# kav-institute/SemanticLiDARUnc

Hardware: AMD Instinct MI355X
Metric: range-image scans/sec (64x2048, T=8 MC) (higher is better)
Workload: dtype f16 (fp16 activations/weights, fp32 accumulate + epilogue, fp32 logits); 1 GPU; SalsaNext MC-dropout T=8 + entropy/MI map + IoU/ECE accumulation, 8 scans of 64x2048x5 per step per GPU (BASELINE configs[2] shape); T=8, parallelism=scan-sharded x1, mc_schedule=every pass fully recomputed

## Files before the change

include/slu.h:

```cpp
#ifndef SLU_H_
#define SLU_H_

#include <stddef.h>
#include <stdint.h>

#ifdef __cplusplus
extern "C" {
#endif

#define SLU_ABI_VERSION 32

#define SLU_OK            0
#define SLU_EINVAL       -1
#define SLU_EUNSUPPORTED -2
#define SLU_ELAUNCH      -3

typedef void* slu_stream_t;

int slu_abi_version(void);
const char* slu_strerror(int code);

#define SLU_MAX_SRC 3

typedef struct slu_conv_src {
  const float* ptr;
  const float* scale;
  int32_t C;
  int32_t pixel_shuffle;
  int32_t nbatch;
  int32_t cuse;
} slu_conv_src;

typedef struct slu_conv_desc {
  slu_conv_src src[SLU_MAX_SRC];
  int32_t nsrc;
  int32_t N, H, W;
  int32_t Cin, Cout;
  int32_t ksize, dil, pad;
  int32_t ck;
  const float* wpack;
  const float* bias;
  int32_t has_act;
  float slope;
  const float* bn_a;
  const float* bn_b;
  const float* resid;
  float* out;
  int32_t precision;
  double* stats;
} slu_conv_desc;

#define SLU_CONV_FP32  0
#define SLU_CONV_F16X3 1

int slu_conv_ck(int ksize);
size_t slu_packed_weight_floats(int cout, int cin, int ksize, int ck);
int slu_pack_conv_weight(const float* w, int cout, int cin, int ksize, int ck, float* out, slu_stream_t stream);
typedef struct slu_pack_job {
  const float* w;
  float* out;
  int32_t cout, cin, ksize, ck;
  int32_t dgrad, reserved;
  uint64_t begin;
// ... 39 lines not shown
int slu_lovasz_fwd(const float* probs, const int64_t* labels, int B, int C, int HW, int64_t ignore_index, unsigned class_mask,
                   void* workspace, size_t workspace_bytes, float* loss, float* n_present, float* grad_probs,
                   slu_stream_t stream);

int slu_bn_stats(const float* y, int N, int C, int HW, double* sum, double* sumsq, slu_stream_t stream);
int slu_bn_bwd_reduce(const float* dz, const float* y, const float* mean, const float* invstd, int N, int C, int HW,
                      double* s1, double* s2, slu_stream_t stream);
int slu_bn_coeffs_fwd(const double* sum, const double* sumsq, double count, const float* gamma, const float* beta, float eps,
                      float momentum, int train, float* running_mean, float* running_var, int C, float* mean, float* invstd,
                      float* a, float* b, slu_stream_t stream);
int slu_bn_coeffs_bwd(const double* s1, const double* s2, double count, const float* gamma, const float* mean, const float* invstd,
                      int train, int C, float* k1, float* k2, float* k3, float* dgamma, float* dbeta, slu_stream_t stream);
int slu_affine_fwd(const float* y, const float* a, const float* b, const float* resid, float* z, int N, int C, int HW,
                   slu_stream_t stream);
int slu_act_affine_bwd(const float* dz, const float* y, const float* k1, const float* k2, const float* k3, float slope,
                       int has_act, int N, int C, int HW, float* da, double* dbias, slu_stream_t stream);
int slu_bn_apply_fwd(const float* y, const double* sum, const double* sumsq, double count, const float* gamma, const float* beta, float eps,
                     float momentum, int train, float* running_mean, float* running_var, const float* resid, float* z, int N, int C, int HW,
                     float* mean, float* invstd, slu_stream_t stream);
int slu_bn_act_bwd(const float* dz, const float* y, const double* s1, const double* s2, double count, const float* gamma, const float* mean,
                   const float* invstd, int has_bn, int train, float slope, int has_act, int N, int C, int HW, float* da, double* acc64,
                   unsigned* ticket, float* dbias, float* dgamma, float* dbeta, slu_stream_t stream);
int slu_nchw_to_nhwc(const float* src, int N, int C, int HW, float* dst, slu_stream_t stream);
int slu_gather_nhwc(const slu_conv_src* src, int nsrc, int N, int H, int W, float* dst, slu_stream_t stream);
int slu_split_grad(const float* dcat, int N, int Ccat, int cbeg, int H, int W, int Csrc, int pixel_shuffle, const float* scale,
                   float* dsrc, slu_stream_t stream);
int slu_avgpool3s2_bwd(const float* dy, const float* scale, float* dx, int N, int C, int H, int W, slu_stream_t stream);
int slu_dgrad_weight(const float* w, int cout, int cin, int ksize, float* wd, slu_stream_t stream);
size_t slu_wgrad_packed_floats(int cout, int cin, int ksize);
int slu_conv2d_wgrad(const float* da_t, const float* in_t, int N, int H, int W, int Cout, int Cin, int ksize, int dil, int pad,
                     float* dWp, float* dW, slu_stream_t stream);
int slu_conv1x1_wgrad_nchw(const float* da, const slu_conv_src* src, int nsrc, int N, int HW, int Cout, float* dW, int prezeroed, slu_stream_t stream);
int slu_conv2d_wgrad_nchw(const float* da, const slu_conv_src* src, int nsrc, int N, int H, int W, int Cout, int ksize, int dil, int pad,
                          float* dWp, float* dW, int prezeroed, slu_stream_t stream);

int slu_maxpool3s2_fwd(const float* x, float* y, int N, int C, int H, int W, slu_stream_t stream);
int slu_nearest_down(const float* x, float* y, int N, int C, int H, int W, int factor, slu_stream_t stream);
int slu_space_to_depth2(const float* x, float* y, int N, int C, int H, int W, slu_stream_t stream);
int slu_space_to_depth2_cat(const float* a, int Ca, int ca, const float* b, int Cb, float* y, int N, int H, int W, slu_stream_t stream);
int slu_depth_to_space(const float* x, float* y, int N, int Cout, int H, int W, int r, int elu_plus_one, int c_off, int Ctot,
                       slu_stream_t stream);
int slu_row_softmax_mul(const float* score, const float* value, float* out, int N, int C, int H, int W, slu_stream_t stream);

int slu_bilinear_upsample(const float* x, float* y, int N, int C, int H, int W, int scale, slu_stream_t stream);
int slu_groupnorm_fwd(const float* x, const float* gamma, const float* beta, int N, int C, int HW, int groups, float eps, int relu, float* mean,
                      float* rstd, float* y, slu_stream_t stream);
int slu_spatial_softmax_gate(const float* x, const float* score, float* stats, float* out, int N, int C, int HW, slu_stream_t stream);

typedef struct slu_h8_src {
  const void* ptr;
  const float* scale;
  int32_t G;
  int32_t nbatch;
} slu_h8_src;

typedef struct slu_conv_h8_desc {
  slu_h8_src src[SLU_MAX_SRC];
  int32_t nsrc;
  int32_t N, H, W, Cout, ksize, dil, pad;
  const void* wpack;
  const float* bias;
  int32_t has_act;
  float slope;
  const float* bn_a;
  const float* bn_b;
  const void* resid;
  void* out;
  int32_t out_f32_nchw;
} slu_conv_h8_desc;

size_t slu_packed_weight_bytes_h8(int cout, int cin, int ksize);
int slu_pack_conv_weight_h8(const float* w, int cout, int cin, int ksize, void* out, slu_stream_t stream);
int slu_conv2d_h8_fwd(const slu_conv_h8_desc* desc, slu_stream_t stream);
int slu_conv2d_h8_kernel_name(const slu_conv_h8_desc* desc, char* buf, size_t n);
int slu_nchw_to_h8(const float* x, const float* scale, void* y, int N, int C, int H, int W, slu_stream_t stream);
int slu_h8_to_nchw(const void* x, float* y, int N, int C, int H, int W, slu_stream_t stream);
int slu_avgpool3s2_h8(const void* x, const float* scale, void* y, int N, int in_batch, int G, int H, int W, slu_stream_t stream);
int slu_pixel_shuffle_h8(const void* x, const float* scale_in, const float* scale_out, void* y, int N, int Gin, int H, int W,
                         slu_stream_t stream);

typedef struct slu_conv_tail_h8_desc {
  const void *a1, *a2;
  int32_t N, H, W, C;
  const void *w2x2, *w1x1;
  const float *biasA, *bnA_a, *bnA_b;
  int32_t hasactA;
  float slopeA;
  const float *biasB, *bnB_a, *bnB_b;
  int32_t hasactB;
  float slopeB;
  const void* resid;
  void* out;
  const void *sc_x, *sc_w;
  const float* sc_bias;
  int32_t sc_cin, sc_hasact;
  float sc_slope;
} slu_conv_tail_h8_desc;
int slu_conv_tail_h8_supported(int C, int H, int W);
int slu_conv_tail_h8_shortcut_supported(int C, int sc_cin);
int slu_conv_tail_h8_fwd(const slu_conv_tail_h8_desc* desc, slu_stream_t stream);
int slu_conv_tail_h8_kernel_name(const slu_conv_tail_h8_desc* desc, char* buf, size_t n);

typedef struct slu_ctx_block_h8_desc {
  const void* x;
  int32_t N, H, W, Cin, C;
  const void *w1, *w2, *w3;
  const float* bias1;
  const float *bias2, *bn1_a, *bn1_b;
  const float *bias3, *bn2_a, *bn2_b;
  float slope;
  void* out;
} slu_ctx_block_h8_desc;
int slu_ctx_block_h8_supported(int Cin, int C, int H, int W);
int slu_ctx_block_h8_fwd(const slu_ctx_block_h8_desc* desc, slu_stream_t stream);

int slu_head_mc_h8(const void* x, int T, int B, int G, int HW, const void* wpack, const float* bias, int C, float eps, float* p_bar,
                   float* h_norm, float* mi_norm, int64_t* preds, slu_stream_t stream);

int slu_dirichlet_head(const float* shape_logits, long long shape_batch_stride, const float* scale_logits, long long scale_batch_stride,
                       int B, int C, int HW, float temperature, float eps, float* alpha, float* p_hat, float* entropy, float* aleatoric,
                       int64_t* preds, slu_stream_t stream);
int slu_dirichlet_uncertainty(const float* alpha, int B, int C, int HW, float eps, float* p_hat, float* entropy, float* aleatoric,
                              int64_t* preds, slu_stream_t stream);

int slu_auroc_scores(const float* preds, const int64_t* labels, const float* score_override, int B, int C, int HW, int mode, int score_kind,
                     int has_ignore, int64_t ignore_index, float eps, float* scores, uint8_t* flags, slu_stream_t stream);
size_t slu_auroc_workspace_bytes(long long n);
int slu_auroc_compute(const float* scores, const uint8_t* is_error, long long n, void* workspace, size_t workspace_bytes, double* out3,
                      float* sorted_scores, uint8_t* sorted_is_error, slu_stream_t stream);

int slu_ua_samples(const int64_t* labels, const int64_t* preds, const float* uncertainty, long long n, const int64_t* ignore_ids, int n_ignore,
                   float* u_out, uint8_t* flags, slu_stream_t stream);
int slu_binned_counts(const float* u, const uint8_t* correct, long long n, const float* edges, int n_bins, int64_t* count, int64_t* n_correct,
                      slu_stream_t stream);

int slu_ece_samples(const float* preds, const int64_t* labels, int B, int C, int HW, int mode, int has_ignore, int64_t ignore_index, float eps,
                    float* conf, uint8_t* flags, slu_stream_t stream);
int slu_binned_stats(const float* u, const uint8_t* correct, long long n, const float* edges, int n_bins, int64_t* count, int64_t* n_correct,
                     double* sum_u, slu_stream_t stream);

size_t slu_group_by_class_workspace_bytes(long long n);
int slu_group_by_class(const int64_t* labels, const float* values, long long n, int C, float* out_values, int64_t* counts, void* workspace,
                       size_t workspace_bytes, slu_stream_t stream);

int slu_tversky_fwd(const float* x, const int64_t* labels, int B, int C, int HW, int model_act, int has_ignore, int64_t ignore_index, float alpha,
                    float beta, float smooth, int reduction, double* sums, float* coef, float* loss, float* any_valid, slu_stream_t stream);
int slu_tversky_bwd(const float* x, const int64_t* labels, int B, int C, int HW, int model_act, int has_ignore, int64_t ignore_index, float alpha,
                    float beta, const float* coef, const float* grad_out, int grad_out_per_class, float* grad_x, slu_stream_t stream);

int slu_dirichlet_loss_fwd(const float* alpha, const int64_t* labels, int B, int C, int HW, int kind, float param, float eps, int has_ignore,
                           int64_t ignore_index, double* sum, int64_t* count, slu_stream_t stream);
int slu_dirichlet_loss_bwd(const float* alpha, const int64_t* labels, int B, int C, int HW, int kind, float param, float eps, int has_ignore,
                           int64_t ignore_index, const float* gscale, float* grad_alpha, slu_stream_t stream);

int slu_dirichlet_loss_fwd_ex(const float* alpha, const int64_t* labels, int B, int C, int HW, int kind, const float* params, int nparams, float eps,
                              int has_ignore, int64_t ignore_index, double* sums2, int64_t* count, slu_stream_t stream);
int slu_dirichlet_loss_bwd_ex(const float* alpha, const int64_t* labels, int B, int C, int HW, int kind, const float* params, int nparams, float eps,
                              int has_ignore, int64_t ignore_index, const float* gscale, float* grad_alpha, slu_stream_t stream);

size_t slu_spherical_projection_workspace_bytes(int N, int H, int W);
int slu_spherical_projection(const double* pc, int N, int C, int H, int W, int use_data_theta_range, double theta_min, double theta_max,
                             void* workspace, size_t workspace_bytes, float* img, double* theta_range_out, slu_stream_t stream);
int slu_spherical_projection_ex(const double* pc, int N, int C, int H, int W, int use_data_theta_range, double theta_min, double theta_max,
                                const double* bins_h, int bins_increasing, int keep_farthest, int flip, void* workspace, size_t workspace_bytes,
// ... 49 lines not shown
```

semanticlidarunc_amd/_lib.py:

```python
from __future__ import annotations

import ctypes as C
import os

ABI_VERSION = 32
MAX_SRC = 3
_HERE = os.path.dirname(os.path.abspath(__file__))
LIB_PATH = os.path.join(_HERE, "libslu_hip.so")

c_f32p = C.c_void_p
c_i64p = C.c_void_p
c_f64p = C.c_void_p
c_stream = C.c_void_p


class ConvSrc(C.Structure):
    _fields_ = [("ptr", C.c_void_p), ("scale", C.c_void_p), ("C", C.c_int32), ("pixel_shuffle", C.c_int32),
                ("nbatch", C.c_int32), ("cuse", C.c_int32)]


class ConvDesc(C.Structure):
    _fields_ = [
        ("src", ConvSrc * MAX_SRC),
        ("nsrc", C.c_int32),
        ("N", C.c_int32), ("H", C.c_int32), ("W", C.c_int32),
        ("Cin", C.c_int32), ("Cout", C.c_int32),
        ("ksize", C.c_int32), ("dil", C.c_int32), ("pad", C.c_int32),
        ("ck", C.c_int32),
        ("wpack", C.c_void_p), ("bias", C.c_void_p),
        ("has_act", C.c_int32), ("slope", C.c_float),
        ("bn_a", C.c_void_p), ("bn_b", C.c_void_p),
        ("resid", C.c_void_p), ("out", C.c_void_p),
        ("precision", C.c_int32),
        ("stats", C.c_void_p),
    ]


class H8Src(C.Structure):
    _fields_ = [("ptr", C.c_void_p), ("scale", C.c_void_p), ("G", C.c_int32), ("nbatch", C.c_int32)]


class ConvH8Desc(C.Structure):
    _fields_ = [
        ("src", H8Src * MAX_SRC),
        ("nsrc", C.c_int32),
        ("N", C.c_int32), ("H", C.c_int32), ("W", C.c_int32), ("Cout", C.c_int32),
        ("ksize", C.c_int32), ("dil", C.c_int32), ("pad", C.c_int32),
        ("wpack", C.c_void_p), ("bias", C.c_void_p),
        ("has_act", C.c_int32), ("slope", C.c_float),
        ("bn_a", C.c_void_p), ("bn_b", C.c_void_p),
        ("resid", C.c_void_p), ("out", C.c_void_p),
        ("out_f32_nchw", C.c_int32),
    ]


class PackJob(C.Structure):
    _fields_ = [("w", C.c_void_p), ("out", C.c_void_p), ("cout", C.c_int32), ("cin", C.c_int32), ("ksize", C.c_int32), ("ck", C.c_int32),
                ("dgrad", C.c_int32), ("reserved", C.c_int32), ("begin", C.c_uint64)]


class ConvTailH8Desc(C.Structure):
    _fields_ = [
        ("a1", C.c_void_p), ("a2", C.c_void_p),
        ("N", C.c_int32), ("H", C.c_int32), ("W", C.c_int32), ("C", C.c_int32),
        ("w2x2", C.c_void_p), ("w1x1", C.c_void_p),
        ("biasA", C.c_void_p), ("bnA_a", C.c_void_p), ("bnA_b", C.c_void_p),
        ("hasactA", C.c_int32), ("slopeA", C.c_float),
        ("biasB", C.c_void_p), ("bnB_a", C.c_void_p), ("bnB_b", C.c_void_p),
        ("hasactB", C.c_int32), ("slopeB", C.c_float),
        ("resid", C.c_void_p), ("out", C.c_void_p),
        ("sc_x", C.c_void_p), ("sc_w", C.c_void_p), ("sc_bias", C.c_void_p),
        ("sc_cin", C.c_int32), ("sc_hasact", C.c_int32), ("sc_slope", C.c_float),
    ]


class CtxBlockH8Desc(C.Structure):
    _fields_ = [
        ("x", C.c_void_p),
        ("N", C.c_int32), ("H", C.c_int32), ("W", C.c_int32), ("Cin", C.c_int32), ("C", C.c_int32),
        ("w1", C.c_void_p), ("w2", C.c_void_p), ("w3", C.c_void_p),
        ("bias1", C.c_void_p),
        ("bias2", C.c_void_p), ("bn1_a", C.c_void_p), ("bn1_b", C.c_void_p),
        ("bias3", C.c_void_p), ("bn2_a", C.c_void_p), ("bn2_b", C.c_void_p),
        ("slope", C.c_float),
        ("out", C.c_void_p),
    ]


SIGNATURES = {
    "slu_abi_version": (C.c_int, []),
    "slu_strerror": (C.c_char_p, [C.c_int]),
    "slu_conv_ck": (C.c_int, [C.c_int]),
    "slu_packed_weight_floats": (C.c_size_t, [C.c_int, C.c_int, C.c_int, C.c_int]),
    "slu_pack_conv_weight": (C.c_int, [c_f32p, C.c_int, C.c_int, C.c_int, C.c_int, c_f32p, c_stream]),
    "slu_pack_conv_weights_multi": (C.c_int, [C.c_void_p, C.c_int, C.c_size_t, c_stream]),
    "slu_conv2d_fwd": (C.c_int, [C.POINTER(ConvDesc), c_stream]),
    "slu_packed_weight_bytes_f16x3": (C.c_size_t, [C.c_int, C.c_int, C.c_int]),
    "slu_pack_conv_weight_f16x3": (C.c_int, [c_f32p, C.c_int, C.c_int, C.c_int, C.c_void_p, c_stream]),
    "slu_conv2d_kernel_name": (C.c_int, [C.POINTER(ConvDesc), C.c_char_p, C.c_size_t]),
    "slu_bn_fold": (C.c_int, [c_f32p, c_f32p, c_f32p, c_f32p, C.c_float, C.c_int, c_f32p, c_f32p, c_stream]),
    "slu_avgpool3s2_fwd": (C.c_int, [c_f32p, c_f32p, c_f32p, C.c_int, C.c_int, C.c_int, C.c_int, c_stream]),
    "slu_avgpool3s2_bcast_fwd": (C.c_int, [c_f32p, c_f32p, c_f32p, C.c_int, C.c_int, C.c_int, C.c_int, C.c_int, c_stream]),
    "slu_mc_reduce": (C.c_int, [c_f32p, C.c_int, C.c_int, C.c_int, C.c_int, C.c_float, c_f32p, c_f32p, c_f32p,
                                c_i64p, c_stream]),
    "slu_softmax_entropy": (C.c_int, [c_f32p, C.c_int, C.c_int, C.c_int, C.c_float, c_f32p, c_f32p, c_i64p,
                                      c_stream]),
    "slu_confusion_update": (C.c_int, [c_i64p, c_i64p, C.c_int64, C.c_int, c_i64p, c_stream]),
    "slu_ece_update": (C.c_int, [c_f32p, c_i64p, C.c_int, C.c_int, C.c_int, C.c_int64, C.c_int, c_i64p, c_f64p,
                                 c_f64p, c_stream]),
    "slu_softmax_nll_fwd": (C.c_int, [c_f32p, c_i64p, C.c_int, C.c_int, C.c_int, C.c_float, c_f32p, c_f64p,
                                      c_stream]),
    "slu_nll_fwd": (C.c_int, [c_f32p, c_i64p, C.c_int, C.c_int, C.c_int, C.c_int, C.c_float, C.c_int64, c_f64p, c_i64p,
                              c_stream]),
    "slu_nll_bwd": (C.c_int, [c_f32p, c_i64p, C.c_int, C.c_int, C.c_int, C.c_int, C.c_float, C.c_int64, c_f32p, c_f32p,
                              c_stream]),
    "slu_softmax_loss_bwd": (C.c_int, [c_f32p, c_i64p, c_f32p, C.c_float, C.c_float, C.c_float, c_f32p, C.c_int, C.c_int,
                                       C.c_int, c_f32p, c_stream]),
    "slu_bn_stats": (C.c_int, [c_f32p, C.c_int, C.c_int, C.c_int, c_f64p, c_f64p, c_stream]),
    "slu_bn_bwd_reduce": (C.c_int, [c_f32p, c_f32p, c_f32p, c_f32p, C.c_int, C.c_int, C.c_int, c_f64p, c_f64p, c_stream]),
    "slu_bn_coeffs_fwd": (C.c_int, [c_f64p, c_f64p, C.c_double, c_f32p, c_f32p, C.c_float, C.c_float, C.c_int, c_f32p, c_f32p, C.c_int,
                                    c_f32p, c_f32p, c_f32p, c_f32p, c_stream]),
    "slu_bn_coeffs_bwd": (C.c_int, [c_f64p, c_f64p, C.c_double, c_f32p, c_f32p, c_f32p, C.c_int, C.c_int, c_f32p, c_f32p, c_f32p,
                                    c_f32p, c_f32p, c_stream]),
    "slu_affine_fwd": (C.c_int, [c_f32p, c_f32p, c_f32p, c_f32p, c_f32p, C.c_int, C.c_int, C.c_int, c_stream]),
    "slu_bn_apply_fwd": (C.c_int, [c_f32p, c_f64p, c_f64p, C.c_double, c_f32p, c_f32p, C.c_float, C.c_float, C.c_int, c_f32p, c_f32p, c_f32p, c_f32p,
                                   C.c_int, C.c_int, C.c_int, c_f32p, c_f32p, c_stream]),
    "slu_bn_act_bwd": (C.c_int, [c_f32p, c_f32p, c_f64p, c_f64p, C.c_double, c_f32p, c_f32p, c_f32p, C.c_int, C.c_int, C.c_float, C.c_int, C.c_int,
                                 C.c_int, C.c_int, c_f32p, c_f64p, C.c_void_p, c_f32p, c_f32p, c_f32p, c_stream]),
    "slu_act_affine_bwd": (C.c_int, [c_f32p, c_f32p, c_f32p, c_f32p, c_f32p, C.c_float, C.c_int, C.c_int, C.c_int, C.c_int,
                                     c_f32p, c_f64p, c_stream]),
    "slu_nchw_to_nhwc": (C.c_int, [c_f32p, C.c_int, C.c_int, C.c_int, c_f32p, c_stream]),
    "slu_gather_nhwc": (C.c_int, [C.POINTER(ConvSrc), C.c_int, C.c_int, C.c_int, C.c_int, c_f32p, c_stream]),
    "slu_split_grad": (C.c_int, [c_f32p, C.c_int, C.c_int, C.c_int, C.c_int, C.c_int, C.c_int, C.c_int, c_f32p, c_f32p,
                                 c_stream]),
    "slu_avgpool3s2_bwd": (C.c_int, [c_f32p, c_f32p, c_f32p, C.c_int, C.c_int, C.c_int, C.c_int, c_stream]),
    "slu_dgrad_weight": (C.c_int, [c_f32p, C.c_int, C.c_int, C.c_int, c_f32p, c_stream]),
    "slu_wgrad_packed_floats": (C.c_size_t, [C.c_int, C.c_int, C.c_int]),
    "slu_conv2d_wgrad": (C.c_int, [c_f32p, c_f32p, C.c_int, C.c_int, C.c_int, C.c_int, C.c_int, C.c_int, C.c_int, C.c_int,
# ... 116 lines not shown
```

semanticlidarunc_amd/csrc/conv2d_h8.hip:

```cpp
#include <stdio.h>
#include "slu_common.h"
#include <cstdlib>
#include <utility>

typedef _Float16 half8 __attribute__((ext_vector_type(8)));
typedef _Float16 half2v __attribute__((ext_vector_type(2)));
typedef float f32x16 __attribute__((ext_vector_type(16)));
typedef float float2v __attribute__((ext_vector_type(2)));

#ifndef H8_M128_OPT_3X3
#define H8_M128_OPT_3X3 15
#endif
#ifndef H8_M128_OPT_2X2
#define H8_M128_OPT_2X2 15
#endif
#ifndef H8_M128_KPC2_DEFAULT
#define H8_M128_KPC2_DEFAULT 0
#endif

namespace {

struct H8Src {
  const uint4* ptr;
  const float* scale;
  int G;
  int gbeg;
  int nb;
};

struct H8Args {
  H8Src src[SLU_MAX_SRC];
  int nsrc;
  int N, H, W, Gin, Cout, Gout, nmblk, nks;
  const uint4* wpack;
  const float *bias, *bn_a, *bn_b;
  int has_act;
  float slope;
  int out_f32;
  int tiles_x, tiles_y;
  int order;
#ifdef SLU_H8_AB
  int dbg;
#endif
};

struct SrcSel {
  const uint4* ptr;
  const float* scale;
  int G, gl, ns;
};

__device__ __forceinline__ SrcSel select_src(const H8Args& a, const int (&img)[SLU_MAX_SRC], int g) {
  SrcSel p{a.src[0].ptr, a.src[0].scale, a.src[0].G, g, img[0]};
#pragma unroll
  for (int s = 1; s < SLU_MAX_SRC; ++s)
    if (s < a.nsrc && g >= a.src[s].gbeg) p = SrcSel{a.src[s].ptr, a.src[s].scale, a.src[s].G, g - a.src[s].gbeg, img[s]};
  return p;
}

__device__ __forceinline__ uint4 scale_record(uint4 v, const float* sp) {
  const float4 s0 = *reinterpret_cast<const float4*>(sp);
  const float4 s1 = *reinterpret_cast<const float4*>(sp + 4);
  half8 h = __builtin_bit_cast(half8, v);
  h[0] *= (_Float16)s0.x; h[1] *= (_Float16)s0.y; h[2] *= (_Float16)s0.z; h[3] *= (_Float16)s0.w;
  h[4] *= (_Float16)s1.x; h[5] *= (_Float16)s1.y; h[6] *= (_Float16)s1.z; h[7] *= (_Float16)s1.w;
  return __builtin_bit_cast(uint4, h);
}

__device__ __forceinline__ unsigned pack2(float x, float y) {
  half2v h;
  h[0] = (_Float16)x;
  h[1] = (_Float16)y;
  return __builtin_bit_cast(unsigned, h);
}

template <int STRIDE>
__device__ __forceinline__ void store_tile(const H8Args& a, const f32x16& acc, const float* se, int cl0, int co0, int hh, bool pix_ok,
                                           size_t n, size_t pix, size_t HW, const void* __restrict__ resid, void* __restrict__ out,
                                           float slope_pre) {
#pragma unroll
// ... 84 lines not shown
      if (resid) {
        const bool okq = pix_ok && go0 + q < a.Gout;
        const uint2 r = *(okq ? resid + (((n * a.Gout + go0 + q) * HW + pix) * 2 + hh) : reinterpret_cast<const uint2*>(zero_addr));
        t0 += __builtin_convertvector(__builtin_bit_cast(half2v, r.x), float2v);
        t1 += __builtin_convertvector(__builtin_bit_cast(half2v, r.y), float2v);
      }
      hw[2 * q2] = __builtin_bit_cast(unsigned, __builtin_convertvector(t0, half2v));
      hw[2 * q2 + 1] = __builtin_bit_cast(unsigned, __builtin_convertvector(t1, half2v));
    }
    const auto s0 = __builtin_amdgcn_permlane32_swap(hw[0], hw[2], false, false);
    const auto s1 = __builtin_amdgcn_permlane32_swap(hw[1], hw[3], false, false);
    const int go = go0 + 2 * pr + hh;
    uint4* dst = (pix_ok && go < a.Gout) ? out + ((n * a.Gout + go) * HW + pix) : reinterpret_cast<uint4*>(trash_addr);
    *dst = make_uint4(s0[0], s1[0], s0[1], s1[1]);
  }
}

#ifdef SLU_H8_PROF
__device__ unsigned long long g_h8_prof[8];
#define H8_PROF_MARK(i)                                         \
  {                                                             \
    const unsigned long long t_now = __builtin_amdgcn_s_memtime(); \
    asm volatile("" ::: "memory");                              \
    prof_acc[i] += t_now - prof_t;                              \
    prof_t = t_now;                                             \
  }
#else
#define H8_PROF_MARK(i)
#endif

#define SLU_GLDS16(gsrc, ldst_wave_base)                                                                  \
  __builtin_amdgcn_global_load_lds((const __attribute__((address_space(1))) void*)(gsrc),                 \
                                   (__attribute__((address_space(3))) void*)(ldst_wave_base), 16, 0, 0)

constexpr int h8_waves_per_simd(int mb, int nwave, int rpw) { return (mb * rpw >= 8) ? 1 : ((nwave >= 8 || mb >= 2 || rpw >= 2) ? 2 : 3); }

template <int KS, int DIL, int PAD, int MB, int WM, int WN, int RPW, bool SCALED, bool WRES, bool F32OUT, int KPC = 1, int OPT = 0, bool ONE = false>
__global__ __launch_bounds__(64 * WM * WN, h8_waves_per_simd(MB, WM * WN, RPW)) void conv_h8_kernel(const H8Args a, const void* __restrict__ resid,
                                                                                                       void* __restrict__ out) {
  constexpr int NWAVE = WM * WN;
  constexpr int T = KS * KS, TS = KPC * T;
  constexpr int TW = 64, TH = WN * RPW, NB = 2 * RPW;
  constexpr int LW = TW + 2 * PAD, LH = TH + 2 * PAD;
  constexpr int REC = LH * LW;
  constexpr int MBLK = WM * MB;
  constexpr int NREC_B = KPC * 2 * REC, NBLK_B = (NREC_B + 63) / 64;
  constexpr int NB_ALLOC = NBLK_B * 64;
  constexpr int NREC_A = MBLK * TS * 64, NBLK_A = MBLK * TS;
  constexpr int NIB = (NBLK_B + NWAVE - 1) / NWAVE, NIA = (NBLK_A + NWAVE - 1) / NWAVE;
  static_assert(KPC == 1 || (!WRES && !SCALED && MB == 2 && WM == 2 && WN == 4), "multi-K-step chunks: the 8-wave 128-channel configuration only");
  static_assert(OPT == 0 || (MB == 2 && WM == 2 && WN == 4 && !F32OUT), "OPT: the 8-wave 128-channel configuration only");
  static_assert(KPC <= 2, "pc_rc carries 2 bits of channel block");
  static_assert(KPC == 1 || ONE, "multi-K-step chunks: single-source layers only");

  extern __shared__ __attribute__((aligned(16))) char smem[];
  float* s_epi = reinterpret_cast<float*>(smem);
  uint4* s_scale = reinterpret_cast<uint4*>(s_epi + 3 * MBLK * 32);
  uint4* s_b = s_scale + (SCALED ? 128 : 0);
  uint4* s_a = s_b + 2 * NB_ALLOC;

  const int tid = threadIdx.x, lane = tid & 63, wave = __builtin_amdgcn_readfirstlane(tid >> 6);
  const int wm = wave / WN, wn = wave % WN;
  const bool late_half = wave >= NWAVE / 2;
  const int mblk0 = blockIdx.y * MBLK;
  int t_beg, t_end, t_step = 1;
  {
    const int nwg = gridDim.x, b = blockIdx.x, xcd = b & 7, qq = nwg >> 3, rr = nwg & 7;
    const int w = (xcd < rr ? xcd * (qq + 1) : rr * (qq + 1) + (xcd - rr) * qq) + (b >> 3);
    const long long nt = (long long)a.tiles_x * a.tiles_y * a.N;
    if (a.order) {
      t_step = nwg;
      t_beg = w;
      t_end = w < nt ? w + (int)((nt - w + nwg - 1) / nwg) * nwg : w;
    } else {
      t_beg = (int)(nt * w / nwg);
      t_end = (int)(nt * (w + 1) / nwg);
    }
  }
  t_beg = __builtin_amdgcn_readfirstlane(t_beg);
  t_end = __builtin_amdgcn_readfirstlane(t_end);
  t_step = __builtin_amdgcn_readfirstlane(t_step);
  if (t_beg >= t_end) return;

  if (tid < MBLK * 32) {
    const int co = mblk0 * 32 + tid;
    const bool ok = co < a.Cout;
    s_epi[tid] = (ok && a.bias) ? a.bias[co] : 0.0f;
    s_epi[MBLK * 32 + tid] = (ok && a.bn_a) ? a.bn_a[co] : 1.0f;
    s_epi[2 * MBLK * 32 + tid] = (ok && a.bn_a) ? a.bn_b[co] : 0.0f;
  }

  const int hh = lane >> 5, jj = lane & 31;
  const size_t HW = (size_t)a.H * a.W;
  const float slope_pre = (a.has_act & 3) == 1 ? a.slope : 1.0f;
  const int nks = a.nks;
  const int nchunk = (nks + KPC - 1) / KPC;
  const int a_stride = WRES ? nks * T * 64 : TS * 64;
  const int abase = (wm * MB) * a_stride + lane;
  const int bbase = hh * REC + (wn * RPW) * LW + jj;

  struct TilePos { int tx, ty, x0, y0, n, i0, i1, i2; };
  auto rfl = [](int v) __attribute__((always_inline)) { return __builtin_amdgcn_readfirstlane(v); };
  const int step_tx = rfl(t_step % a.tiles_x), step_ty = rfl((t_step / a.tiles_x) % a.tiles_y), step_n = rfl(t_step / (a.tiles_x * a.tiles_y));
  auto finish = [&](TilePos& p) __attribute__((always_inline)) {
    p.x0 = p.tx * TW;
    p.y0 = p.ty * TH;
    p.i0 = p.i1 = p.i2 = p.n;
    if constexpr (!ONE) {
      if (a.src[0].nb) p.i0 = rfl(p.n % a.src[0].nb);
      if (a.nsrc > 1 && a.src[1].nb) p.i1 = rfl(p.n % a.src[1].nb);
      if (a.nsrc > 2 && a.src[2].nb) p.i2 = rfl(p.n % a.src[2].nb);
    }
  };
  auto decode = [&](int t) __attribute__((always_inline)) {
    TilePos p;
    p.tx = rfl(t % a.tiles_x);
    t /= a.tiles_x;
    p.ty = rfl(t % a.tiles_y);
    p.n = rfl(t / a.tiles_y);
    finish(p);
    return p;
  };
  auto advance = [&](TilePos p) __attribute__((always_inline)) {
    p.tx += step_tx;
    if (p.tx >= a.tiles_x) p.tx -= a.tiles_x, p.ty += 1;
    p.ty += step_ty;
    if (p.ty >= a.tiles_y) p.ty -= a.tiles_y, p.n += 1;
    p.n += step_n;
    finish(p);
    return p;
  };
  static_assert(SLU_MAX_SRC == 3, "TilePos carries one image index per source");
  uintptr_t zero_addr = reinterpret_cast<uintptr_t>(&g_zero_rec);
  asm volatile("" : "+s"(zero_addr));
  uintptr_t trash_addr = reinterpret_cast<uintptr_t>(&g_trash_rec);
  asm volatile("" : "+s"(trash_addr));
  int pc_rc[NIB], pc_off[NIB];
#pragma unroll
  for (int i = 0; i < NIB; ++i) {
    const int e = (i * NWAVE + wave) * 64 + lane;
    const int g2 = e / REC;
    const int rem = e - g2 * REC;
    const int r = rem / LW;
    const int c = rem - r * LW;
    pc_rc[i] = r | (c << 8) | ((g2 & (2 * KPC - 1)) << 16) | ((e < NREC_B ? 1 : 0) << 20);
    pc_off[i] = r * a.W + c + (g2 & (2 * KPC - 1)) * (int)HW;
  }
  constexpr int NPIECE = NIB + (WRES ? 0 : NIA);
  constexpr int PPT = (NPIECE + TS - 1) / TS;
  uintptr_t st_b0 = 0, st_b1 = 0;
  int st_g0 = 0;
  bool st_on = false;
  int st_x0 = 0, st_y0 = 0, st_q = 0, st_wave = wave;
  uint4 *st_db = s_b, *st_da = s_a;
  auto stage_begin = [&](const TilePos& tp, int q, int buf) __attribute__((always_inline)) {
    const int img[SLU_MAX_SRC] = {tp.i0, tp.i1, tp.i2};
    const long long org = (long long)(tp.y0 - PAD) * a.W + (tp.x0 - PAD);
    st_g0 = 2 * KPC * q;
    if constexpr (ONE) {
      st_b0 = reinterpret_cast<uintptr_t>(a.src[0].ptr) + 16 * ((long long)(((size_t)tp.n * a.src[0].G + st_g0) * HW) + org);
      st_b1 = st_b0;
    } else {
      const SrcSel p0 = select_src(a, img, st_g0 < a.Gin ? st_g0 : 0), p1 = select_src(a, img, st_g0 + 1 < a.Gin ? st_g0 + 1 : 0);
      st_b0 = reinterpret_cast<uintptr_t>(p0.ptr) + 16 * ((long long)(((size_t)p0.ns * p0.G + p0.gl) * HW) + org);
      st_b1 = reinterpret_cast<uintptr_t>(p1.ptr) + 16 * ((long long)(((size_t)p1.ns * p1.G + p1.gl) * HW) + org - (long long)HW);
    }
    st_x0 = tp.x0 - PAD;
    st_y0 = tp.y0 - PAD;
    st_q = q;
    st_db = s_b + buf * NB_ALLOC;
    st_da = s_a + buf * NREC_A;
    st_on = true;
    st_wave = wave;
    asm volatile("" : "+s"(st_wave));
  };
  auto stage_piece = [&](int i) __attribute__((always_inline)) {
    if (i < NIB) {
      const int blk = i * NWAVE + st_wave;
      if (NBLK_B % NWAVE == 0 || blk < NBLK_B) {
        const int rc = pc_rc[i];
        const int gy = st_y0 + (rc & 255), gx = st_x0 + ((rc >> 8) & 255);
        const int gsel = (rc >> 16) & 3;
        const uintptr_t gb = (!ONE && gsel == 1) ? st_b1 : st_b0;
        const bool ok = (rc >> 20) && st_g0 + gsel < a.Gin && (unsigned)gy < (unsigned)a.H && (unsigned)gx < (unsigned)a.W;
        const uintptr_t src = ok ? gb + 16 * (long long)pc_off[i] : zero_addr;
        SLU_GLDS16(reinterpret_cast<const uint4*>(src), st_db + blk * 64);
      }
    } else if constexpr (!WRES) {
      const int blk = (i - NIB) * NWAVE + st_wave;
      if (NBLK_A % NWAVE == 0 || blk < NBLK_A) {
        const int m = blk / TS, r = blk - m * TS;
        const bool live = mblk0 + m < a.nmblk && (KPC == 1 || KPC * st_q + r / T < nks);
        const uint4* src = live ? a.wpack + (((size_t)(mblk0 + m) * nks + KPC * st_q) * T + r) * 64 + lane : reinterpret_cast<const uint4*>(zero_addr);
        SLU_GLDS16(src, st_da + blk * 64);
      }
    }
  };
  auto stage_after_tap = [&](int tap) __attribute__((always_inline)) {
    if (st_on) {
#pragma unroll
      for (int k = 0; k < PPT; ++k)
        if (tap * PPT + k < NPIECE) stage_piece(tap * PPT + k);
    }
  };
  auto stage_scales = [&](int n, int par) __attribute__((always_inline)) {
    if (tid < 64) {
      half8 h;
#pragma unroll
      for (int k = 0; k < 8; ++k) h[k] = (_Float16)1.0f;
      if (tid < a.Gin) {
        int img[SLU_MAX_SRC] = {0, 0, 0};
        const SrcSel p = select_src(a, img, tid);
        if (p.scale) {
          const float* sp = p.scale + ((size_t)n * p.G + p.gl) * 8;
          const float4 s0 = *reinterpret_cast<const float4*>(sp), s1 = *reinterpret_cast<const float4*>(sp + 4);
          h[0] = (_Float16)s0.x; h[1] = (_Float16)s0.y; h[2] = (_Float16)s0.z; h[3] = (_Float16)s0.w;
          h[4] = (_Float16)s1.x; h[5] = (_Float16)s1.y; h[6] = (_Float16)s1.z; h[7] = (_Float16)s1.w;
        }
      }
      s_scale[par * 64 + tid] = __builtin_bit_cast(uint4, h);
    }
  };

  if constexpr (WRES) {
    const int per_m = nks * T;
    for (int blk = wave; blk < MBLK * per_m; blk += NWAVE) {
      const int m = blk / per_m;
      const uint4* src = mblk0 + m < a.nmblk ? a.wpack + ((size_t)(mblk0 + m) * per_m + (blk - m * per_m)) * 64 + lane : &g_zero_rec;
      SLU_GLDS16(src, s_a + blk * 64);
    }
  }
  TilePos cur = decode(t_beg), nxt = cur;
  stage_begin(cur, 0, 0);
#pragma unroll
  for (int i = 0; i < NPIECE; ++i) stage_piece(i);
  int buf = 0;
  constexpr bool SWAP16 = (OPT & 8) != 0;
  constexpr int NST = MB * NB * (SWAP16 ? 2 : 4);
  constexpr bool PRE = MB == 1 && !F32OUT;
  const uint2* resid2 = reinterpret_cast<const uint2*>(resid);
  uint2 rv[PRE ? NB : 1][4];
  auto setup_next = [&](int tile, int q) __attribute__((always_inline)) {
    st_on = false;
    if (q + 1 < nchunk) {
      stage_begin(cur, q + 1, buf ^ 1);
    } else if (tile + t_step < t_end) {
      nxt = advance(cur);
      stage_begin(nxt, 0, buf ^ 1);
    }
  };

#ifdef SLU_H8_PROF
  unsigned long long prof_acc[6] = {0, 0, 0, 0, 0, 0}, prof_t = __builtin_amdgcn_s_memtime();
#endif
  int tile_no = 0;
  for (int tile = t_beg; tile < t_end; tile += t_step, ++tile_no) {
    f32x16 acc[MB][NB];
#pragma unroll
    for (int i = 0; i < MB; ++i)
#pragma unroll
      for (int b = 0; b < NB; ++b)
#pragma unroll
        for (int r = 0; r < 16; ++r) acc[i][b][r] = 0.0f;
    const int spar = tile_no & 1;
    if constexpr (SCALED) stage_scales(cur.n, spar);
    for (int q = 0; q < nchunk; ++q) {
      if constexpr ((OPT & 4) != 0) setup_next(tile, q);
      if (!F32OUT && q == 0 && tile != t_beg) asm volatile("s_waitcnt vmcnt(%0)" ::"n"(NST < 63 ? NST : 63) : "memory");
      else asm volatile("s_waitcnt vmcnt(0)" ::: "memory");
      asm volatile("s_waitcnt lgkmcnt(0)" ::: "memory");
      H8_PROF_MARK(0)
      __builtin_amdgcn_s_barrier();
      asm volatile("" ::: "memory");
      H8_PROF_MARK(1)
      if constexpr ((OPT & 4) == 0) setup_next(tile, q);
      if constexpr (PRE) {
        if (resid && q == nchunk - 1) {
#pragma unroll
          for (int b = 0; b < NB; ++b) {
            const int gy = cur.y0 + wn * RPW + (b >> 1), gx = cur.x0 + (b & 1) * 32 + jj;
            const bool pix_ok = gy < a.H && gx < a.W;
            const size_t pix = (size_t)gy * a.W + gx;
#pragma unroll
            for (int k = 0; k < 4; ++k) {
              const int go = (mblk0 + wm) * 4 + k;
              rv[b][k] = *((pix_ok && go < a.Gout) ? resid2 + (((size_t)cur.n * a.Gout + go) * HW + pix) * 2 + hh
                                                   : reinterpret_cast<const uint2*>(zero_addr));
            }
          }
        }
      }
      H8_PROF_MARK(2)
      const uint4* sb = s_b + buf * NB_ALLOC + bbase;
      const uint4* sa = s_a + abase + (WRES ? q * T * 64 : buf * NREC_A);
      half8 sc;
      if constexpr (SCALED) sc = __builtin_bit_cast(half8, s_scale[spar * 64 + 2 * q + hh]);
      {
        if constexpr (MB == 2 && WM == 2 && WN == 4) {
          half8 af[2][MB], bf[2][NB];
          auto read_frags = [&](int set, int ts) __attribute__((always_inline)) {
            const int j = ts / T, tap = ts % T;
            const int dy = (tap / KS) * DIL, dx = (tap % KS) * DIL;
#pragma unroll
            for (int i = 0; i < MB; ++i) af[set][i] = __builtin_bit_cast(half8, sa[i * a_stride + ts * 64]);
#pragma unroll
            for (int b = 0; b < NB; ++b) {
              bf[set][b] = __builtin_bit_cast(half8, sb[j * 2 * REC + ((b >> 1) + dy) * LW + (b & 1) * 32 + dx]);
              if constexpr (SCALED) bf[set][b] *= sc;
            }
          };
          read_frags(0, 0);
#pragma unroll
          for (int ts = 0; ts < TS; ++ts) {
            if (ts + 1 < TS) read_frags((ts + 1) & 1, ts + 1);
            __builtin_amdgcn_sched_barrier(0);
            if constexpr ((OPT & 1) != 0) {
              if (late_half) stage_after_tap(ts);
              __builtin_amdgcn_sched_barrier(0);
            }
            if constexpr ((OPT & 2) != 0) __builtin_amdgcn_s_setprio(1);
#pragma unroll
            for (int b = 0; b < NB; ++b)
#pragma unroll
              for (int i = 0; i < MB; ++i) acc[i][b] = __builtin_amdgcn_mfma_f32_32x32x16_f16(af[ts & 1][i], bf[ts & 1][b], acc[i][b], 0, 0, 0);
            if constexpr ((OPT & 2) != 0) __builtin_amdgcn_s_setprio(0);
            __builtin_amdgcn_sched_barrier(0);
            if constexpr ((OPT & 1) != 0) {
              if (!late_half) stage_after_tap(ts);
            } else {
              stage_after_tap(ts);
            }
          }
        } else if constexpr (MB == 1) {
          half8 af[2][MB], bf[2][NB];
          auto read_frags = [&](int set, int tap) __attribute__((always_inline)) {
            const int dy = (tap / KS) * DIL, dx = (tap % KS) * DIL;
#pragma unroll
            for (int i = 0; i < MB; ++i) af[set][i] = __builtin_bit_cast(half8, sa[i * a_stride + tap * 64]);
#pragma unroll
            for (int b = 0; b < NB; ++b) {
              bf[set][b] = __builtin_bit_cast(half8, sb[((b >> 1) + dy) * LW + (b & 1) * 32 + dx]);
              if constexpr (SCALED) bf[set][b] *= sc;
            }
          };
          read_frags(0, 0);
#pragma unroll
          for (int tap = 0; tap < T; ++tap) {
            if (tap + 1 < T) read_frags((tap + 1) & 1, tap + 1);
#pragma unroll
            for (int b = 0; b < NB; ++b)
#pragma unroll
              for (int i = 0; i < MB; ++i) acc[i][b] = __builtin_amdgcn_mfma_f32_32x32x16_f16(af[tap & 1][i], bf[tap & 1][b], acc[i][b], 0, 0, 0);
            if (tap + 1 < T) {
#pragma unroll
              for (int k = 0; k < MB * NB; ++k) {
                __builtin_amdgcn_sched_group_barrier(0x008, 1, 0);
                __builtin_amdgcn_sched_group_barrier(0x100, (MB + NB + MB * NB - 1) / (MB * NB), 0);
              }
            }
            stage_after_tap(tap);
          }
        } else {
#pragma unroll
          for (int tap = 0; tap < T; ++tap) {
            const int dy = (tap / KS) * DIL, dx = (tap % KS) * DIL;
            half8 af[MB];
#pragma unroll
            for (int i = 0; i < MB; ++i) af[i] = __builtin_bit_cast(half8, sa[i * a_stride + tap * 64]);
#pragma unroll
            for (int b = 0; b < NB; ++b) {
              half8 bf = __builtin_bit_cast(half8, sb[((b >> 1) + dy) * LW + (b & 1) * 32 + dx]);
              if constexpr (SCALED) bf *= sc;
#pragma unroll
              for (int i = 0; i < MB; ++i) acc[i][b] = __builtin_amdgcn_mfma_f32_32x32x16_f16(af[i], bf, acc[i][b], 0, 0, 0);
            }
#pragma unroll
            for (int k = 0; k < MB * NB; ++k) {
              __builtin_amdgcn_sched_group_barrier(0x008, 1, 0);
              __builtin_amdgcn_sched_group_barrier(0x100, (MB + NB + MB * NB - 1) / (MB * NB), 0);
            }
            stage_after_tap(tap);
          }
        }
      }
      buf ^= 1;
      H8_PROF_MARK(3)
    }
    {
#pragma unroll
      for (int i = 0; i < MB; ++i) {
        const int ml = wm * MB + i;
#pragma unroll
        for (int b = 0; b < NB; ++b) {
          const int gy = cur.y0 + wn * RPW + (b >> 1), gx = cur.x0 + (b & 1) * 32 + jj;
          const bool pix_ok = gy < a.H && gx < a.W;
          const size_t pix = pix_ok ? (size_t)gy * a.W + gx : 0;
          if constexpr (F32OUT)
            store_tile<MBLK * 32>(a, acc[i][b], s_epi, ml * 32, (mblk0 + ml) * 32, hh, pix_ok, (size_t)cur.n, pix, HW, resid, out, slope_pre);
          else if constexpr (SWAP16)
            store_tile_swap16<MBLK * 32>(a, acc[i][b], s_epi, ml * 32, (mblk0 + ml) * 4, hh, pix_ok, (size_t)cur.n, pix, HW, resid2,
                                         reinterpret_cast<uint4*>(out), slope_pre, zero_addr, trash_addr);
          else
            store_tile_full<MBLK * 32, PRE>(a, acc[i][b], s_epi, ml * 32, (mblk0 + ml) * 4, hh, pix_ok, (size_t)cur.n, pix, HW, resid2,
                                            rv[PRE ? b : 0], reinterpret_cast<uint2*>(out), slope_pre, zero_addr, trash_addr);
          __builtin_amdgcn_sched_barrier(0);
        }
      }
    }
    H8_PROF_MARK(4)
    cur = nxt;
  }
#ifdef SLU_H8_PROF
  if (tid == 0) {
    for (int i = 0; i < 5; ++i) atomicAdd(&g_h8_prof[i], prof_acc[i]);
    atomicAdd(&g_h8_prof[5], 1ull);
  }
#endif
}

template <int MB, int NBW>
__global__ __launch_bounds__(256, (MB * NBW >= 8) ? 2 : ((MB * NBW >= 4) ? 3 : 4)) void conv1x1_h8_kernel(const H8Args a, const void* __restrict__ resid,
                                                                                                         void* __restrict__ out) {
  constexpr int KSPC = 4;
  constexpr int NWV = MB * KSPC * 64, NW = (NWV + 255) / 256;
  extern __shared__ __attribute__((aligned(16))) char smem[];
// ... 440 lines not shown
  const size_t HWi = (size_t)H * W;
  const int OW = 2 * W;
  for (size_t e = (size_t)blockIdx.x * blockDim.x + threadIdx.x; e < total; e += (size_t)gridDim.x * blockDim.x) {
    const int w = (int)(e % W);
    size_t r = e / W;
    const int h = (int)(r % H);
    r /= H;
    const int go = (int)(r % Go);
    const size_t n = r / Go;
    float v[4][8];
#pragma unroll
    for (int q = 0; q < 4; ++q) {
      const int gi = 4 * go + q;
      const bool ok = gi < Gi;
      const half8 rec = __builtin_bit_cast(half8, ok ? x[(n * Gi + gi) * HWi + (size_t)h * W + w] : make_uint4(0u, 0u, 0u, 0u));
#pragma unroll
      for (int slot = 0; slot < 8; ++slot) {
        float t = (float)rec[slot];
        if (ok && s_in) t *= s_in[n * Gi * 8 + gi * 8 + slot];
        v[slot & 3][2 * q + (slot >> 2)] = t;
      }
    }
    if (s_out) {
#pragma unroll
      for (int k = 0; k < 8; ++k) {
        const int co = 8 * go + k;
        const float so = co < 2 * Gi ? s_out[n * (Gi * 2) + co] : 0.0f;
#pragma unroll
        for (int sub = 0; sub < 4; ++sub) v[sub][k] *= so;
      }
    }
#pragma unroll
    for (int sub = 0; sub < 4; ++sub) {
      const size_t o = ((n * Go + go) * (size_t)(2 * H) + (2 * h + (sub >> 1))) * OW + 2 * w + (sub & 1);
      y[o] = make_uint4(pack2(v[sub][0], v[sub][1]), pack2(v[sub][2], v[sub][3]), pack2(v[sub][4], v[sub][5]), pack2(v[sub][6], v[sub][7]));
    }
  }
}

inline unsigned grid_for(size_t total) {
  const size_t nb = (total + 255) / 256;
  return (unsigned)(nb > 32768 ? 32768 : (nb ? nb : 1));
}

int fill_h8(const slu_conv_h8_desc* d, H8Args& a) {
  if (!d || !d->out || !d->wpack || d->nsrc < 1 || d->nsrc > SLU_MAX_SRC) return SLU_EINVAL;
  if (d->N <= 0 || d->H <= 0 || d->W <= 0 || d->Cout <= 0) return SLU_EINVAL;
  if (d->bn_a && !d->bn_b) return SLU_EINVAL;
  if (d->has_act != 0 && d->has_act != 1) return SLU_EINVAL;
  if (d->has_act && !(d->slope >= 0.0f && d->slope <= 1.0f)) return SLU_EINVAL;
  int g = 0;
  for (int s = 0; s < d->nsrc; ++s) {
    const slu_h8_src& S = d->src[s];
    if (!S.ptr || S.G <= 0 || S.nbatch < 0) return SLU_EINVAL;
    if (((uintptr_t)S.ptr & 15) || ((uintptr_t)S.scale & 15)) return SLU_EINVAL;
    a.src[s] = H8Src{reinterpret_cast<const uint4*>(S.ptr), S.scale, S.G, g, S.nbatch};
    g += S.G;
  }
  for (int s = d->nsrc; s < SLU_MAX_SRC; ++s) a.src[s] = H8Src{nullptr, nullptr, 0, 0x7fffffff, 0};
  if (((uintptr_t)d->out & 15) || ((uintptr_t)d->resid & 15) || ((uintptr_t)d->wpack & 15)) return SLU_EINVAL;
  if (d->resid && d->out_f32_nchw) return SLU_EINVAL;
  a.nsrc = d->nsrc;
  a.N = d->N; a.H = d->H; a.W = d->W;
  a.Gin = g;
  a.Cout = d->Cout;
  a.Gout = (d->Cout + 7) / 8;
  a.nmblk = (d->Cout + 31) / 32;
  a.nks = (g + 1) / 2;
  a.wpack = reinterpret_cast<const uint4*>(d->wpack);
  a.bias = d->bias; a.bn_a = d->bn_a; a.bn_b = d->bn_b;
  a.has_act = d->has_act; a.slope = d->slope;
  a.out_f32 = d->out_f32_nchw ? 1 : 0;
  a.tiles_x = a.tiles_y = 0;
#ifdef SLU_H8_AB
  static const int dbg = [] { const char* e = getenv("SLU_GEMM_DBG"); return e ? atoi(e) : 0; }();
  a.dbg = dbg;
#endif
  return SLU_OK;
}

template <int KS, int DIL, int PAD, int MB, int WM, int WN, int RPW, bool SCALED, bool WRES, bool F32OUT = false, int KPC = 1, int OPT = 0, bool ONE = false>
int launch_h8_k(H8Args& a, const slu_conv_h8_desc* d, const SluEmit& e) {
  constexpr int TH = WN * RPW, MBLK = WM * MB, T = KS * KS, NWAVE = WM * WN;
  constexpr size_t nb_alloc = (size_t)((KPC * 2 * (TH + 2 * PAD) * (64 + 2 * PAD) + 63) / 64) * 64;
  const size_t lds = (size_t)3 * MBLK * 32 * 4 + (SCALED ? 2048 : 0) + 2 * nb_alloc * 16 + (size_t)MBLK * (WRES ? a.nks : 2 * KPC) * T * 64 * 16;
  if (lds > 160 * 1024) return SLU_EUNSUPPORTED;
  if (SCALED && a.Gin > 64) return SLU_EUNSUPPORTED;
  a.tiles_x = (a.W + 63) / 64;
  a.tiles_y = (a.H + TH - 1) / TH;
  static const int order = [] { const char* e = getenv("SLU_H8_ORDER"); return e ? atoi(e) : 1; }();
  a.order = order;
  const long long nt = (long long)a.tiles_x * a.tiles_y * a.N;
  const int gy = (a.nmblk + MBLK - 1) / MBLK;
  if (nt <= 0 || nt > 0x7fffffffLL || gy > 65535) return SLU_EUNSUPPORTED;
  if (e.name)
    return slu_emit_name(e, "conv_h8_kernel<%d, %d, %d, %d, %d, %d, %d, %s, %s, %s, %d, %d, %s>", KS, DIL, PAD, MB, WM, WN, RPW, slu_tf(SCALED),
                         slu_tf(WRES), slu_tf(F32OUT), KPC, OPT, slu_tf(ONE));
  long long per_cu = h8_waves_per_simd(MB, NWAVE, RPW) * 4 / NWAVE;
  const long long by_lds = (long long)(160 * 1024 / lds);
  if (by_lds < per_cu) per_cu = by_lds;
  if (per_cu < 1) per_cu = 1;
  long long gx = (256 * per_cu + gy - 1) / gy;
  if (gx < 8) gx = 8;
  if (gx > nt) gx = nt;
  auto kern = conv_h8_kernel<KS, DIL, PAD, MB, WM, WN, RPW, SCALED, WRES, F32OUT, KPC, OPT, ONE>;
  static SluLdsGrant grant;
  if (slu_grant_dynamic_lds(reinterpret_cast<const void*>(kern), lds, grant) != SLU_OK) return SLU_ELAUNCH;
  hipLaunchKernelGGL(kern, dim3((unsigned)gx, (unsigned)gy), dim3(64 * NWAVE), lds, e.st, a, d->resid, d->out);
  SLU_CHECK_LAUNCH();
}

typedef float f32x4v __attribute__((ext_vector_type(4)));

struct RingArgs {
  const uint4 *x, *x1;
  int G0, G1;
  const uint4* wpack;
  const float *bias, *bn_a, *bn_b;
  float slope;
  uint4* out;
  int N, H, W, tiles_x, tiles_y;
};

template <int NKS, int NIB, int P, int NST>
constexpr int ring3_younger(int c) {
  const int s0 = ((c - P) % NKS + NKS) % NKS;
  int n = s0 == NKS - 1 ? NST : 0;
  for (int d = 1; d < P; ++d) n += NIB + ((s0 + d) % NKS == NKS - 1 ? NST : 0);
  return n;
}
template <class F, int... Cs>
__device__ __forceinline__ void ring3_static_for(F&& f, std::integer_sequence<int, Cs...>) {
  (f(std::integral_constant<int, Cs>{}), ...);
}

template <int DIL, int MB, int NKS, int RPW, int D>
__global__ __launch_bounds__(512, 2) void ring3_h8_kernel(const RingArgs a) {
  constexpr int NWAVE = 8, KS = 3, T = 9, PAD = DIL, P = D - 1;
  constexpr int C = 32 * MB, GO = 4 * MB;
  constexpr int TW = 64, TH = NWAVE * RPW, NB = 2 * RPW;
  constexpr int LW = TW + 2 * PAD, LH = TH + 2 * PAD, REC = LH * LW;
  constexpr int NBLK_B = (2 * REC + 63) / 64, NIB = (NBLK_B + NWAVE - 1) / NWAVE;
  constexpr int BUFREC = NBLK_B * 64;
  constexpr int NST = MB * NB * 2;
  static_assert(P >= 1 && P <= NKS, "ring depth");

  __shared__ __attribute__((aligned(16))) float s_epi[3 * C];
  extern __shared__ __attribute__((aligned(16))) char smem[];
  uint4* s_w = reinterpret_cast<uint4*>(smem);
  uint4* s_ring = s_w + MB * NKS * T * 64;
  uint4* s_trash = s_ring + D * BUFREC;

  const int tid = threadIdx.x, lane = tid & 63, wave = __builtin_amdgcn_readfirstlane(tid >> 6), wn = wave;
  const int hh = lane >> 5, jj = lane & 31;
  const size_t HW = (size_t)a.H * a.W;

  int t_beg, t_end, t_step;
  {
    const int nwg = gridDim.x, b = blockIdx.x, xcd = b & 7, qq = nwg >> 3, rr = nwg & 7;
    const int w = (xcd < rr ? xcd * (qq + 1) : rr * (qq + 1) + (xcd - rr) * qq) + (b >> 3);
    const long long nt = (long long)a.tiles_x * a.tiles_y * a.N;
    t_step = nwg;
    t_beg = w;
    t_end = w < nt ? w + (int)((nt - w + nwg - 1) / nwg) * nwg : w;
  }
  if (t_beg >= t_end) return;

  if (tid < C) {
    s_epi[tid] = a.bias ? a.bias[tid] : 0.0f;
    s_epi[C + tid] = a.bn_a ? a.bn_a[tid] : 1.0f;
    s_epi[2 * C + tid] = a.bn_a ? a.bn_b[tid] : 0.0f;
  }
  for (int blk = wave; blk < MB * NKS * T; blk += NWAVE) SLU_GLDS16(a.wpack + (size_t)blk * 64 + lane, s_w + blk * 64);

  struct TilePos { int x0, y0, n; };
  auto decode = [&](int t) {
    TilePos p;
    const int tx = t % a.tiles_x;
    t /= a.tiles_x;
    p.x0 = tx * TW;
    p.y0 = (t % a.tiles_y) * TH;
    p.n = t / a.tiles_y;
    return p;
  };
  int pc_rc[NIB], pc_off[NIB];
#pragma unroll
  for (int i = 0; i < NIB; ++i) {
    const int e = (i * NWAVE + wave) * 64 + lane;
    const int g2 = e / REC, rem = e - g2 * REC, r = rem / LW, c = rem - r * LW;
    pc_rc[i] = r | (c << 8) | ((g2 & 1) << 16) | ((e < 2 * REC ? 1 : 0) << 17);
    pc_off[i] = (r * a.W + c) * 16;
  }
  auto stage = [&](const TilePos& tp, int c, int slot, bool valid) {
    uint4* db = s_ring + slot * BUFREC;
    const uintptr_t zero = reinterpret_cast<uintptr_t>(&g_zero_rec);
    const bool second = 2 * c >= a.G0;
    const uint4* src = second ? a.x1 : a.x;
    const int gs = second ? a.G1 : a.G0, g = second ? 2 * c - a.G0 : 2 * c;
    const uintptr_t base0 = reinterpret_cast<uintptr_t>(src) +
                            16 * ((long long)(((size_t)tp.n * gs + g) * HW) + (long long)(tp.y0 - PAD) * a.W + (tp.x0 - PAD));
    const uintptr_t base1 = base0 + 16 * (long long)HW;
#pragma unroll
    for (int i = 0; i < NIB; ++i) {
      const int blk = i * NWAVE + wave;
      const int rc = pc_rc[i];
      const int gy = tp.y0 - PAD + (rc & 255), gx = tp.x0 - PAD + ((rc >> 8) & 255);
      const bool ok = valid && (rc >> 17) && (unsigned)gy < (unsigned)a.H && (unsigned)gx < (unsigned)a.W;
      const uintptr_t p = ok ? (((rc >> 16) & 1) ? base1 : base0) + (long long)pc_off[i] : zero;
      SLU_GLDS16(reinterpret_cast<const uint4*>(p), (NBLK_B % NWAVE == 0 || blk < NBLK_B) ? db + blk * 64 : s_trash);
    }
    asm volatile("" ::: "memory");
  };

  const int bbase = hh * REC + (wn * RPW) * LW + jj;
  TilePos cur = decode(t_beg), nxt = cur;
  bool has_next = t_beg + t_step < t_end;
  if (has_next) nxt = decode(t_beg + t_step);
#pragma unroll
  for (int c = 0; c < P; ++c) stage(cur, c, c, true);
  int rslot = 0, wslot = P % D;
  bool first = true;
  const float2v sl = {a.slope, a.slope};
  const f32x4v* se4p = reinterpret_cast<const f32x4v*>(s_epi) + hh;

  for (int tile = t_beg; tile < t_end; tile += t_step) {
    f32x16 acc[MB][NB];
#pragma unroll
    for (int i = 0; i < MB; ++i)
#pragma unroll
      for (int b = 0; b < NB; ++b)
#pragma unroll
        for (int r = 0; r < 16; ++r) acc[i][b][r] = 0.0f;

    auto position = [&](auto cc) {
      constexpr int c = decltype(cc)::value;
      constexpr int YOUNG = ring3_younger<NKS, NIB, P, NST>(c);
      static_assert(YOUNG <= 63, "vmcnt is a 6-bit counter");
      if (first && c < P) asm volatile("s_waitcnt vmcnt(0)" ::: "memory");
      else asm volatile("s_waitcnt vmcnt(%0)" ::"n"(YOUNG) : "memory");
      asm volatile("s_waitcnt lgkmcnt(0)" ::: "memory");
      __builtin_amdgcn_s_barrier();
      asm volatile("" ::: "memory");
      {
        constexpr int cn = (c + P) % NKS;
        if (c + P < NKS) stage(cur, cn, wslot, true);
        else stage(nxt, cn, wslot, has_next);
        wslot = wslot + 1 == D ? 0 : wslot + 1;
      }
      const uint4* sb = s_ring + rslot * BUFREC + bbase;
      rslot = rslot + 1 == D ? 0 : rslot + 1;
      half8 fa[2][MB], fb[2][NB];
      auto rd = [&](int tap, int buf) {
        const int dy = (tap / KS) * DIL, dx = (tap % KS) * DIL;
#pragma unroll
        for (int i = 0; i < MB; ++i) fa[buf][i] = __builtin_bit_cast(half8, s_w[((i * NKS + c) * T + tap) * 64 + lane]);
#pragma unroll
        for (int b = 0; b < NB; ++b) fb[buf][b] = __builtin_bit_cast(half8, sb[((b >> 1) + dy) * LW + (b & 1) * 32 + dx]);
      };
      rd(0, 0);
#pragma unroll
      for (int tap = 0; tap < T; ++tap) {
        if (tap + 1 < T) rd(tap + 1, (tap + 1) & 1);
        __builtin_amdgcn_sched_barrier(0);
#pragma unroll
        for (int b = 0; b < NB; ++b)
#pragma unroll
          for (int i = 0; i < MB; ++i) acc[i][b] = __builtin_amdgcn_mfma_f32_32x32x16_f16(fa[tap & 1][i], fb[tap & 1][b], acc[i][b], 0, 0, 0);
        __builtin_amdgcn_sched_barrier(0);
      }
    };
    ring3_static_for(position, std::make_integer_sequence<int, NKS>{});
    first = false;

#pragma unroll
    for (int i = 0; i < MB; ++i)
#pragma unroll
      for (int b = 0; b < NB; ++b) {
        const int gy = cur.y0 + wn * RPW + (b >> 1), gx = cur.x0 + (b & 1) * 32 + jj;
        const bool ok = gy < a.H && gx < a.W;
        const size_t idx0 = ok ? ((size_t)cur.n * GO + i * 4 + hh) * HW + (size_t)gy * a.W + gx : 0;
#pragma unroll
        for (int pr = 0; pr < 2; ++pr) {
          unsigned hw[4];
#pragma unroll
          for (int q2 = 0; q2 < 2; ++q2) {
            const int q = 2 * pr + q2;
            const int c4 = (i * 32 + 8 * q) / 4;
            const f32x4v bi = se4p[c4], ba = se4p[C / 4 + c4], bb = se4p[2 * C / 4 + c4];
            float2v t0 = {acc[i][b][4 * q], acc[i][b][4 * q + 1]}, t1 = {acc[i][b][4 * q + 2], acc[i][b][4 * q + 3]};
            t0 += float2v{bi.x, bi.y};
            t1 += float2v{bi.z, bi.w};
            t0 = __builtin_elementwise_max(t0, t0 * sl);
            t1 = __builtin_elementwise_max(t1, t1 * sl);
            t0 = t0 * float2v{ba.x, ba.y} + float2v{bb.x, bb.y};
            t1 = t1 * float2v{ba.z, ba.w} + float2v{bb.z, bb.w};
            hw[2 * q2] = __builtin_bit_cast(unsigned, __builtin_convertvector(t0, half2v));
            hw[2 * q2 + 1] = __builtin_bit_cast(unsigned, __builtin_convertvector(t1, half2v));
          }
          const auto s0 = __builtin_amdgcn_permlane32_swap(hw[0], hw[2], false, false);
          const auto s1 = __builtin_amdgcn_permlane32_swap(hw[1], hw[3], false, false);
          uint4* dst = ok ? a.out + idx0 + (size_t)(2 * pr) * HW : &g_trash_rec;
          *dst = make_uint4(s0[0], s1[0], s0[1], s1[1]);
        }
      }
    asm volatile("" ::: "memory");
    cur = nxt;
    has_next = tile + 2 * t_step < t_end;
    if (has_next) nxt = decode(tile + 2 * t_step);
  }
  asm volatile("s_waitcnt vmcnt(0)" ::: "memory");
}

template <int DIL, int MB, int NKS, int RPW, int D>
int launch_ring3(const H8Args& h, const slu_conv_h8_desc* d, const SluEmit& e) {
  constexpr int TH = 8 * RPW, PAD = DIL;
  constexpr size_t nblk_b = (size_t)(2 * (TH + 2 * PAD) * (64 + 2 * PAD) + 63) / 64;
  constexpr size_t lds = ((size_t)MB * NKS * 9 * 64 + (size_t)D * nblk_b * 64 + 64) * 16;
  static_assert(lds + 3 * 32 * MB * 4 <= 160 * 1024, "ring does not fit in LDS");
  RingArgs a{};
  a.x = h.src[0].ptr; a.G0 = h.src[0].G;
  a.x1 = h.nsrc > 1 ? h.src[1].ptr : h.src[0].ptr; a.G1 = h.nsrc > 1 ? h.src[1].G : 0;
  a.wpack = h.wpack; a.bias = h.bias; a.bn_a = h.bn_a; a.bn_b = h.bn_b;
  a.slope = (h.has_act & 3) == 1 ? h.slope : 1.0f;
  a.out = reinterpret_cast<uint4*>(d->out);
  a.N = h.N; a.H = h.H; a.W = h.W;
  a.tiles_x = (a.W + 63) / 64;
  a.tiles_y = (a.H + TH - 1) / TH;
  const long long nt = (long long)a.tiles_x * a.tiles_y * a.N;
  if (nt < 256) return -1;
  if (nt > 0x7fffffffLL) return SLU_EUNSUPPORTED;
  if (e.name) return slu_emit_name(e, "ring3_h8_kernel<%d, %d, %d, %d, %d>", DIL, MB, NKS, RPW, D);
  auto kern = ring3_h8_kernel<DIL, MB, NKS, RPW, D>;
  static SluLdsGrant grant;
  if (slu_grant_dynamic_lds(reinterpret_cast<const void*>(kern), lds, grant) != SLU_OK) return SLU_ELAUNCH;
  hipLaunchKernelGGL(kern, dim3(256), dim3(512), lds, e.st, a);
  SLU_CHECK_LAUNCH();
}

bool ring3_ok(const slu_conv_h8_desc* d, const H8Args& a) {
  static const bool off = [] { const char* e = getenv("SLU_H8_RING3"); return e && e[0] == '0'; }();
  if (off || d->ksize != 3 || d->pad != d->dil || (d->dil != 1 && d->dil != 2) || a.nsrc < 1 || a.nsrc > 2) return false;
  int gsum = 0;
  for (int s = 0; s < a.nsrc; ++s) {
    if (a.src[s].scale || a.src[s].nb) return false;
    gsum += a.src[s].G;
  }
  if (gsum != a.Gin || (a.nsrc == 2 && (a.src[0].G & 1)) || a.out_f32 || d->resid || (a.has_act & ~1)) return false;
  if ((a.has_act & 1) && !(a.slope >= 0.0f && a.slope <= 1.0f)) return false;
  return (a.Cout == 32 || a.Cout == 64) && ((a.Gin == 4 || a.Gin == 8) || (a.Gin == 10 && a.Cout == 32 && d->dil == 1));
}

int launch_ring3_any(const H8Args& a, const slu_conv_h8_desc* d, const SluEmit& e) {
  const int mb = a.Cout / 32, nks = a.Gin / 2;
  if (nks == 5) return launch_ring3<1, 1, 5, 1, 4>(a, d, e);
  if (mb == 2 && nks == 4) return d->dil == 1 ? launch_ring3<1, 2, 4, 1, 3>(a, d, e) : launch_ring3<2, 2, 4, 1, 3>(a, d, e);
  if (mb == 2 && nks == 2) return d->dil == 1 ? launch_ring3<1, 2, 2, 2, 3>(a, d, e) : launch_ring3<2, 2, 2, 1, 3>(a, d, e);
  if (mb == 1 && nks == 4) return d->dil == 1 ? launch_ring3<1, 1, 4, 2, 3>(a, d, e) : launch_ring3<2, 1, 4, 1, 3>(a, d, e);
  return d->dil == 1 ? launch_ring3<1, 1, 2, 2, 3>(a, d, e) : launch_ring3<2, 1, 2, 2, 3>(a, d, e);
}

constexpr size_t WRES_MAX_BYTES = 24 * 1024;

template <int KS, int DIL, int PAD, int MB, int WM, int WN, int RPW, bool SCALED>
int launch_h8(H8Args& a, const slu_conv_h8_desc* d, const SluEmit& e) {
  const size_t wbytes = (size_t)WM * MB * a.nks * KS * KS * 64 * 16;
  if (wbytes <= WRES_MAX_BYTES) return launch_h8_k<KS, DIL, PAD, MB, WM, WN, RPW, SCALED, true>(a, d, e);
  return launch_h8_k<KS, DIL, PAD, MB, WM, WN, RPW, SCALED, false>(a, d, e);
}

inline long long wg_count(const H8Args& a, int th, int mblk) {
  return (long long)a.N * ((a.H + th - 1) / th) * ((a.W + 63) / 64) * ((a.nmblk + mblk - 1) / mblk);
}

enum { CFG_M32_TH16 = 0, CFG_M64_TH16, CFG_M128_TH8, CFG_M32_TH8, CFG_M64_TH8, CFG_M128_TH4, CFG_M32_TH4, CFG_M64_TH4, CFG_COUNT };

int choose_h8(const H8Args& a) {
  const long long want = 256;
  static const int forced = [] { const char* e = getenv("SLU_H8_CFG"); return e ? atoi(e) : -1; }();
  if (forced >= 0 && forced < CFG_COUNT) return forced;
  if (a.nmblk >= 4) {
    if (a.H >= 8 && wg_count(a, 8, 4) >= want) return CFG_M128_TH8;
    if (wg_count(a, 4, 4) >= want) return CFG_M128_TH4;
    if (wg_count(a, 4, 2) >= want) return CFG_M64_TH4;
    return CFG_M32_TH4;
  }
  if (a.nmblk >= 2) {
    if (a.H >= 16 && wg_count(a, 16, 2) >= want) return CFG_M64_TH16;
    if (a.H >= 8 && wg_count(a, 8, 2) >= want) return CFG_M64_TH8;
    if (wg_count(a, 4, 2) >= want) return CFG_M64_TH4;
    return CFG_M32_TH4;
  }
  if (a.H >= 16 && wg_count(a, 16, 1) >= want) return CFG_M32_TH16;
  if (a.H >= 8 && wg_count(a, 8, 1) >= want) return CFG_M32_TH8;
  return CFG_M32_TH4;
}

int g_h8_opt = [] { const char* e = getenv("SLU_H8_OPT"); return e ? atoi(e) : -1; }();
int g_h8_kpc2 = [] { const char* e = getenv("SLU_H8_KPC2"); return e ? atoi(e) : H8_M128_KPC2_DEFAULT; }();

// ... 73 lines not shown

template <int MB>
int launch_h8_1x1_res_nks(H8Args& a, const slu_conv_h8_desc* d, const SluEmit& e) {
  switch (a.nks) {
    case 1:  return launch_h8_1x1_res<MB, 1>(a, d, e);
    case 2:  return launch_h8_1x1_res<MB, 2>(a, d, e);
    case 5: case 6:   return launch_h8_1x1_res<MB, 6>(a, d, e);
    case 10: case 12: return launch_h8_1x1_res<MB, 12>(a, d, e);
  }
  return -1;
}

constexpr int GEMM1X1_KC = 4, GEMM1X1_D256 = 2, GEMM1X1_D128 = 3;
bool gemm1x1_ok(const slu_conv_h8_desc* d, const H8Args& a) {
  static const bool off = [] { const char* e = getenv("SLU_H8_GEMM1X1"); return e && e[0] == '0'; }();
  static const bool all = [] { const char* e = getenv("SLU_H8_GEMM1X1"); return e && e[0] == '2'; }();
  if (off || d->ksize != 1 || d->pad != 0 || a.out_f32 || (a.Cout != 256 && !(all && a.Cout == 128))) return false;
  if (((long long)a.H * a.W) % 256 || a.nks % GEMM1X1_KC || a.Gin != 2 * a.nks) return false;
  if ((a.has_act & ~1) || ((a.has_act & 1) && !(a.slope >= 0.0f && a.slope <= 1.0f))) return false;
  for (int s = 0; s < a.nsrc; ++s)
    if (a.src[s].scale || a.src[s].nb || a.src[s].G % (2 * GEMM1X1_KC)) return false;
  return (long long)a.N * a.H * a.W / 256 <= 0x7fffffffLL;
}

template <int MB, int D>
int launch_gemm1x1(H8Args& a, const slu_conv_h8_desc* d, const SluEmit& e) {
  constexpr int KC = GEMM1X1_KC, MBLK = 2 * MB;
  constexpr size_t lds = (size_t)3 * MBLK * 32 * 4 + (size_t)D * (2 * KC * 256) * 16 + (size_t)D * (MBLK * KC * 64) * 16;
  static_assert(lds <= 160 * 1024, "gemm1x1 LDS");
  const long long nt = (long long)a.N * a.H * a.W / 256;
  const long long gx = nt < 256 ? nt : 256;
  if (e.name) return slu_emit_name(e, "gemm1x1_h8_kernel<%d, %d, %d>", MB, KC, D);
  auto kern = gemm1x1_h8_kernel<MB, KC, D>;
  static SluLdsGrant grant;
  if (slu_grant_dynamic_lds(reinterpret_cast<const void*>(kern), lds, grant) != SLU_OK) return SLU_ELAUNCH;
  hipLaunchKernelGGL(kern, dim3((unsigned)gx), dim3(512), lds, e.st, a, d->resid, d->out);
  SLU_CHECK_LAUNCH();
}

bool any_scale(const slu_conv_h8_desc* d) {
  for (int s = 0; s < d->nsrc; ++s)
    if (d->src[s].scale) return true;
  return false;
}

bool stream_ok(const slu_conv_h8_desc* d, const H8Args& a) {
  return d->ksize == 1 && d->pad == 0 && a.nmblk <= 8 && ((long long)a.H * a.W) % 32 == 0 && !any_scale(d);
}

int conv_h8_dispatch(const slu_conv_h8_desc* d, const SluEmit& e) {
  H8Args a{};
  const int rc = fill_h8(d, a);
  if (rc != SLU_OK) return rc;
  if (gemm1x1_ok(d, a)) return a.Cout == 128 ? launch_gemm1x1<2, GEMM1X1_D128>(a, d, e) : launch_gemm1x1<4, GEMM1X1_D256>(a, d, e);
  if (stream_ok(d, a)) {
    if (a.nmblk <= 2) {
      const int rc2 = a.nmblk == 1 ? launch_h8_1x1_res_nks<1>(a, d, e) : launch_h8_1x1_res_nks<2>(a, d, e);
      if (rc2 != -1) return rc2;
    }
    if (a.nmblk == 1) return launch_h8_1x1<1, 2>(a, d, e);
    if (a.nmblk == 2) return launch_h8_1x1<2, 2>(a, d, e);
    if (a.nmblk <= 4) return launch_h8_1x1<4, 1>(a, d, e);
    return launch_h8_1x1<8, 1>(a, d, e);
  }
  if (ring3_ok(d, a)) {
    const int rc2 = launch_ring3_any(a, d, e);
    if (rc2 != -1) return rc2;
  }
  const bool sc = any_scale(d);
  if (a.out_f32) {
    if (d->ksize != 1 || d->dil != 1 || d->pad != 0 || sc) return SLU_EUNSUPPORTED;
    return launch_h8_k<1, 1, 0, 1, 1, 4, 1, false, false, true>(a, d, e);
  }
  const int cfg = choose_h8(a);
  if (d->ksize == 1 && d->dil == 1 && d->pad == 0) return launch_h8_family<1, 1, 0>(a, d, cfg, sc, e);
  if (d->ksize == 3 && d->dil == 1 && d->pad == 1) return launch_h8_family<3, 1, 1>(a, d, cfg, sc, e);
  if (d->ksize == 3 && d->dil == 2 && d->pad == 2) return launch_h8_family<3, 2, 2>(a, d, cfg, sc, e);
  if (d->ksize == 2 && d->dil == 2 && d->pad == 1) return launch_h8_family<2, 2, 1>(a, d, cfg, sc, e);
  return SLU_EUNSUPPORTED;
}

}

extern "C" size_t slu_packed_weight_bytes_h8(int cout, int cin, int ksize) {
  if (cout <= 0 || cin <= 0 || ksize <= 0) return 0;
  const size_t nmblk = (cout + 31) / 32, nks = (cin + 15) / 16;
  return nmblk * nks * (size_t)(ksize * ksize) * 64 * 16;
}

extern "C" int slu_pack_conv_weight_h8(const float* w, int cout, int cin, int ksize, void* out, slu_stream_t stream) {
  if (!w || !out) return SLU_EINVAL;
  const size_t bytes = slu_packed_weight_bytes_h8(cout, cin, ksize);
  if (bytes == 0) return SLU_EINVAL;
  const size_t total = bytes / 16;
  hipLaunchKernelGGL(pack_h8_kernel, dim3(grid_for(total)), dim3(256), 0, slu_stream(stream), w, cout, cin, ksize, (cin + 15) / 16, total,
                     reinterpret_cast<uint4*>(out));
  SLU_CHECK_LAUNCH();
}

extern "C" int slu_conv2d_h8_fwd(const slu_conv_h8_desc* d, slu_stream_t stream) { return conv_h8_dispatch(d, SluEmit{slu_stream(stream), nullptr, 0}); }

extern "C" int slu_conv2d_h8_kernel_name(const slu_conv_h8_desc* d, char* buf, size_t n) {
  return buf ? conv_h8_dispatch(d, SluEmit{nullptr, buf, n}) : SLU_EINVAL;
}

#ifdef SLU_H8_AB
// ... 48 lines not shown
```

semanticlidarunc_amd/csrc/ctx_block_h8.hip:

```cpp
#include <algorithm>
#include <type_traits>
#include "slu_common.h"

typedef _Float16 half8 __attribute__((ext_vector_type(8)));
typedef _Float16 half2v __attribute__((ext_vector_type(2)));
typedef float f32x16 __attribute__((ext_vector_type(16)));
typedef float float2v __attribute__((ext_vector_type(2)));

namespace {

struct CtxArgs {
  const uint4* x;
  const uint4 *w1, *w2, *w3;
  const float *b1, *b2, *bn1_a, *bn1_b, *b3, *bn2_a, *bn2_b;
  float slope;
  uint2* out;
  int N, H, W, Gin;
  int strips_x, nseg, seg_rows;
};

constexpr int R = 8, TW = 64;
constexpr int SW = TW + 6, SROWS = R + 6;
constexpr int AW = TW + 4, AROWS = R + 4;
constexpr int SRING = SROWS * SW + 32, ARING = AROWS * AW + 32;
constexpr int NB1F = (SROWS * SW + 31) / 32, NB1 = (R * SW + 31) / 32;
constexpr int NB2F = (AROWS * AW + 31) / 32, NB2 = (R * AW + 31) / 32;
constexpr int NWAVE = 8;
#ifndef SLU_CTX_RING
#define SLU_CTX_RING 4
#endif
constexpr int RING = SLU_CTX_RING;
constexpr int PW1 = (NB1F + NWAVE - 1) / NWAVE, PW2 = (NB2F + NWAVE - 1) / NWAVE, PW3 = 2;
constexpr int OFF_S = 0, OFF_A = OFF_S + 4 * SRING, OFF_W1 = OFF_A + 4 * ARING;
template <int NKS1> constexpr int off_w2() { return OFF_W1 + NKS1 * 64; }
template <int NKS1> constexpr int off_w3() { return off_w2<NKS1>() + 18 * 64; }
template <int NKS1> constexpr int off_epi() { return off_w3<NKS1>() + 18 * 64; }
template <int NKS1> constexpr size_t lds_bytes() { return (size_t)(off_epi<NKS1>() + 56) * 16; }

#ifdef SLU_CTX_PROF
__device__ unsigned long long g_ctx_prof[8];
#define CTX_PROF_MARK(i)                                             \
  {                                                                  \
    const unsigned long long t_now = __builtin_amdgcn_s_memtime();  \
    asm volatile("" ::: "memory");                                   \
    prof_acc[i] += t_now - prof_t;                                   \
    prof_t = t_now;                                                  \
  }
#else
#define CTX_PROF_MARK(i)
#endif

__device__ uint4 g_trash_rec_c;
__device__ uint4 g_zero_rec_c;

__device__ __forceinline__ int opaque(int v) {
  asm volatile("" : "+v"(v));
  return v;
}

__device__ __forceinline__ float2v leaky2(float2v t, float2v sl) {
  const float2v m = t * sl;
  float2v r;
  asm("v_max_f32 %0, %1, %2" : "=v"(r[0]) : "v"(t[0]), "v"(m[0]));
  asm("v_max_f32 %0, %1, %2" : "=v"(r[1]) : "v"(t[1]), "v"(m[1]));
  return r;
}

__device__ __forceinline__ unsigned pack2h(float2v t) { return __builtin_bit_cast(unsigned, __builtin_convertvector(t, half2v)); }

__device__ __forceinline__ int wrap(int v, int n) { return v >= n ? v - n : v; }
// ... 3 lines not shown
  extern __shared__ __attribute__((aligned(16))) char smem[];
  uint4* lds = reinterpret_cast<uint4*>(smem);
  uint2* lds2 = reinterpret_cast<uint2*>(smem);
  float4* lds4 = reinterpret_cast<float4*>(smem);
  constexpr int OFF_W2 = off_w2<NKS1>(), OFF_W3 = off_w3<NKS1>(), OFF_EPI = off_epi<NKS1>();

  const int tid = threadIdx.x, lane = tid & 63, wave = tid >> 6;
  const int hh = lane >> 5, jj = lane & 31;
  const size_t HW = (size_t)a.H * a.W;

  int t_beg, t_end, t_step;
  {
    const int nwg = gridDim.x, b = blockIdx.x, xcd = b & 7, qq = nwg >> 3, rr = nwg & 7;
    const int w = (xcd < rr ? xcd * (qq + 1) : rr * (qq + 1) + (xcd - rr) * qq) + (b >> 3);
    const long long nt = (long long)a.strips_x * a.nseg * a.N;
    t_step = nwg;
    t_beg = w;
    t_end = w < nt ? w + (int)((nt - w + nwg - 1) / nwg) * nwg : w;
  }
  if (t_beg >= t_end) return;

  {
    float* s_epi = reinterpret_cast<float*>(lds + OFF_EPI);
    if (tid < 32) {
      s_epi[tid] = a.b1 ? a.b1[tid] : 0.0f;
      s_epi[32 + tid] = a.b2 ? a.b2[tid] : 0.0f;
      s_epi[64 + tid] = a.bn1_a ? a.bn1_a[tid] : 1.0f;
      s_epi[96 + tid] = a.bn1_a ? a.bn1_b[tid] : 0.0f;
      s_epi[128 + tid] = a.b3 ? a.b3[tid] : 0.0f;
      s_epi[160 + tid] = a.bn2_a ? a.bn2_a[tid] : 1.0f;
      s_epi[192 + tid] = a.bn2_a ? a.bn2_b[tid] : 0.0f;
    }
    for (int e = tid; e < NKS1 * 64; e += 64 * NWAVE) lds[OFF_W1 + e] = a.w1[e];
    for (int e = tid; e < 18 * 64; e += 64 * NWAVE) {
      lds[OFF_W2 + e] = a.w2[e];
      lds[OFF_W3 + e] = a.w3[e];
    }
  }

  int p1_rc[PW1], p1_goff[PW1], p2_rc[PW2];
#pragma unroll
  for (int i = 0; i < PW1; ++i) {
    const int e = 32 * (wave + NWAVE * i) + jj, r = e / SW, c = e - r * SW;
    p1_rc[i] = r | (c << 8);
    p1_goff[i] = r * a.W + c;
  }
#pragma unroll
  for (int i = 0; i < PW2; ++i) {
    const int e = 32 * (wave + NWAVE * i) + jj, r = e / AW, c = e - r * AW;
    p2_rc[i] = r | (c << 8);
  }
  const int i_w1 = opaque(OFF_W1 + lane), i_w2 = opaque(OFF_W2 + lane), i_w3 = opaque(OFF_W3 + lane), i_epi = opaque(OFF_EPI + hh);

  struct Band { int x0, y0, n, j, r1; };
  auto decode = [&](int t) {
    Band p;
    const int tx = t % a.strips_x;
    t /= a.strips_x;
    p.x0 = tx * TW;
    p.y0 = (t % a.nseg) * a.seg_rows;
    p.n = t / a.nseg;
    p.j = 0;
    p.r1 = min(a.H, p.y0 + a.seg_rows);
    return p;
  };
  uint4 xr[PW1][NKS1];
  auto load_x = [&](const Band& bd) {
    const bool first = bd.j == 0;
    const int ys = first ? bd.y0 - 3 : bd.y0 + 3, nr = first ? SROWS : R;
    const long long org = (long long)ys * a.W + (bd.x0 - 3);
#pragma unroll
    for (int i = 0; i < PW1; ++i) {
      const int rc = p1_rc[i];
      const int gy = ys + (rc & 255), gx = bd.x0 - 3 + (rc >> 8);
      const bool in = (rc & 255) < nr && (unsigned)gy < (unsigned)a.H && (unsigned)gx < (unsigned)a.W;
#pragma unroll
      for (int k = 0; k < NKS1; ++k) {
        const int g = 2 * k + hh;
        const bool ok = in && g < a.Gin;
        xr[i][k] = *(ok ? a.x + (long long)(((size_t)bd.n * a.Gin + g) * HW) + org + p1_goff[i] : &g_zero_rec_c);
      }
    }
  };

  const float2v sl = {a.slope, a.slope};
  auto lane_bias = [&](int first_f4) {
    f32x16 v;
#pragma unroll
    for (int q = 0; q < 4; ++q) {
      const float4 t = lds4[i_epi + first_f4 + 2 * q];
      v[4 * q] = t.x; v[4 * q + 1] = t.y; v[4 * q + 2] = t.z; v[4 * q + 3] = t.w;
    }
    return v;
  };

  auto run_p1 = [&](const Band& bd) {
    const bool first = bd.j == 0;
    const int jr = R * bd.j;
    {
      const int ys = first ? bd.y0 - 3 : bd.y0 + 3, nr = first ? SROWS : R, u0 = first ? 0 : (jr + 6) % SROWS;
      auto phase1 = [&](auto nl_c) {
        constexpr int NL = decltype(nl_c)::value;
        const f32x16 biasv = lane_bias(0);
        half8 af[NKS1];
#pragma unroll
        for (int k = 0; k < NKS1; ++k) af[k] = __builtin_bit_cast(half8, lds[i_w1 + k * 64]);
        f32x16 acc[NL];
#pragma unroll
        for (int i = 0; i < NL; ++i)
#pragma unroll
          for (int k = 0; k < NKS1; ++k)
            acc[i] = __builtin_amdgcn_mfma_f32_32x32x16_f16(af[k], __builtin_bit_cast(half8, xr[i][k]), k == 0 ? biasv : acc[i], 0, 0, 0);
#pragma unroll
        for (int i = 0; i < NL; ++i) {
          const int r = p1_rc[i] & 255, c = p1_rc[i] >> 8;
          const int gy = ys + r, gx = bd.x0 - 3 + c;
          const bool in = (unsigned)gy < (unsigned)a.H && (unsigned)gx < (unsigned)a.W;
          const int wi = opaque(((OFF_S + (r < nr ? wrap(u0 + r, SROWS) * SW + c : SROWS * SW + jj)) << 1) + hh);
#pragma unroll
          for (int q = 0; q < 4; ++q) {
            const float2v t0 = leaky2(float2v{acc[i][4 * q], acc[i][4 * q + 1]}, sl), t1 = leaky2(float2v{acc[i][4 * q + 2], acc[i][4 * q + 3]}, sl);
            lds2[wi + q * SRING * 2] = in ? make_uint2(pack2h(t0), pack2h(t1)) : make_uint2(0u, 0u);
          }
        }
      };
      static_assert(NB1F > (PW1 - 1) * NWAVE && NB1 > (PW1 - 2) * NWAVE && NB1 <= (PW1 - 1) * NWAVE, "P1 block counts per wave: 4 / 3 / 2");
      const int nl = (first ? NB1F - wave + NWAVE - 1 : NB1 - wave + NWAVE - 1) / NWAVE;
      if (nl == PW1) phase1(std::integral_constant<int, PW1>{});
      else if (nl == PW1 - 1) phase1(std::integral_constant<int, PW1 - 1>{});
      else phase1(std::integral_constant<int, PW1 - 2>{});
    }
  };

// ... 178 lines not shown
#ifdef SLU_CTX_PROF
  if (tid == 0) {
    for (int i = 0; i < 6; ++i) atomicAdd(&g_ctx_prof[i], prof_acc[i]);
    atomicAdd(&g_ctx_prof[6], 1ull);
  }
#endif
}

template <int NKS1>
int launch_ctx(CtxArgs& a, hipStream_t st) {
  constexpr size_t lds = lds_bytes<NKS1>();
  static_assert(lds <= 160 * 1024, "rings do not fit in LDS");
  constexpr long long NCU = 256;
  const long long strips = (long long)((a.W + TW - 1) / TW) * a.N;
  const int bands = (a.H + R - 1) / R;
  int per = bands;
  if (strips < NCU) {
    const int nseg = (int)std::min<long long>(bands, (NCU + strips - 1) / strips);
    per = (bands + nseg - 1) / nseg;
  }
  a.strips_x = (a.W + TW - 1) / TW;
  a.nseg = (bands + per - 1) / per;
  a.seg_rows = per * R;
  const long long nt = strips * a.nseg;
  if (nt <= 0 || nt > 0x7fffffffLL || (long long)bands * R + 2 * R > 0x7fffffffLL) return SLU_EUNSUPPORTED;
  long long gx = NCU;
  if (gx > nt) gx = nt;
  auto kern = ctx_h8_kernel<NKS1>;
  static SluLdsGrant grant;
  if (slu_grant_dynamic_lds(reinterpret_cast<const void*>(kern), lds, grant) != SLU_OK) return SLU_ELAUNCH;
  hipLaunchKernelGGL(kern, dim3((unsigned)gx), dim3(64 * NWAVE), lds, st, a);
  SLU_CHECK_LAUNCH();
}

}

#ifdef SLU_CTX_PROF
extern "C" int slu_ctx_prof_read(unsigned long long* out8) {
  if (hipMemcpyFromSymbol(out8, HIP_SYMBOL(g_ctx_prof), sizeof(unsigned long long) * 8) != hipSuccess) return SLU_ELAUNCH;
  unsigned long long z[8] = {};
  return hipMemcpyToSymbol(HIP_SYMBOL(g_ctx_prof), z, sizeof(z)) == hipSuccess ? SLU_OK : SLU_ELAUNCH;
}
#endif

extern "C" int slu_ctx_block_h8_supported(int Cin, int C, int H, int W) { return (Cin >= 1 && Cin <= 32 && C == 32 && H > 0 && W > 0 && W < (1 << 20)) ? 1 : 0; }

extern "C" int slu_ctx_block_h8_fwd(const slu_ctx_block_h8_desc* d, slu_stream_t stream) {
  if (!d || !d->x || !d->w1 || !d->w2 || !d->w3 || !d->out || d->N <= 0 || d->H <= 0 || d->W <= 0) return SLU_EINVAL;
  if (((uintptr_t)d->x | (uintptr_t)d->out | (uintptr_t)d->w1 | (uintptr_t)d->w2 | (uintptr_t)d->w3) & 15) return SLU_EINVAL;
  if ((d->bn1_a == nullptr) != (d->bn1_b == nullptr) || (d->bn2_a == nullptr) != (d->bn2_b == nullptr)) return SLU_EINVAL;
  if (!slu_ctx_block_h8_supported(d->Cin, d->C, d->H, d->W)) return SLU_EUNSUPPORTED;
  if (!(d->slope >= 0.0f && d->slope <= 1.0f)) return SLU_EINVAL;
  if (d->x == d->out) return SLU_EINVAL;
  CtxArgs a{};
  a.x = reinterpret_cast<const uint4*>(d->x);
  a.w1 = reinterpret_cast<const uint4*>(d->w1);
  a.w2 = reinterpret_cast<const uint4*>(d->w2);
  a.w3 = reinterpret_cast<const uint4*>(d->w3);
  a.b1 = d->bias1; a.b2 = d->bias2; a.bn1_a = d->bn1_a; a.bn1_b = d->bn1_b; a.b3 = d->bias3; a.bn2_a = d->bn2_a; a.bn2_b = d->bn2_b;
  a.slope = d->slope;
  a.out = reinterpret_cast<uint2*>(d->out);
  a.N = d->N; a.H = d->H; a.W = d->W; a.Gin = (d->Cin + 7) / 8;
  hipStream_t st = slu_stream(stream);
  return d->Cin <= 16 ? launch_ctx<1>(a, st) : launch_ctx<2>(a, st);
}
```

semanticlidarunc_amd/csrc/dropout_draw.hip:

```cpp
#include "slu_common.h"

namespace {

struct uint4x { unsigned x, y, z, w; };

__device__ __forceinline__ uint4x philox4x32_10(unsigned long long seed, unsigned long long counter, unsigned long long subseq) {
  unsigned k0 = (unsigned)seed, k1 = (unsigned)(seed >> 32);
  unsigned c0 = (unsigned)counter, c1 = (unsigned)(counter >> 32), c2 = (unsigned)subseq, c3 = (unsigned)(subseq >> 32);
#pragma unroll
  for (int r = 0; r < 10; ++r) {
    const unsigned long long p0 = 0xD2511F53ull * c0, p1 = 0xCD9E8D57ull * c2;
    const unsigned n0 = (unsigned)(p1 >> 32) ^ c1 ^ k0, n1 = (unsigned)p1, n2 = (unsigned)(p0 >> 32) ^ c3 ^ k1, n3 = (unsigned)p0;
    c0 = n0; c1 = n1; c2 = n2; c3 = n3;
    k0 += 0x9E3779B9u;
    k1 += 0xBB67AE85u;
  }
  return uint4x{c0, c1, c2, c3};
}

__device__ __forceinline__ float site_mult(const slu_dropout_site* sites, int site, long long e, unsigned long long seed, unsigned long long offset) {
  const slu_dropout_site s = sites[site];
  if (!s.active) return 1.0f;
  const long long g = s.begin + e;
  const uint4x r = philox4x32_10(seed, offset + (unsigned long long)(g >> 2), 0ull);
  const unsigned bits = (g & 3) == 0 ? r.x : ((g & 3) == 1 ? r.y : ((g & 3) == 2 ? r.z : r.w));
  const float u = (float)(bits >> 8) * (1.0f / 16777216.0f);
  return u < s.p ? 0.0f : 1.0f / (1.0f - s.p);
}

__global__ __launch_bounds__(256) void dropout_draw_kernel(const slu_dropout_site* __restrict__ sites, const slu_dropout_out* __restrict__ outs, int nout,
                                                           int N, unsigned long long seed, unsigned long long offset, float* __restrict__ buf,
                                                           long long total) {
  for (long long e = (long long)blockIdx.x * blockDim.x + threadIdx.x; e < total; e += (long long)gridDim.x * blockDim.x) {
    int o = 0;
    while (o + 1 < nout && e >= outs[o + 1].begin) ++o;
    const slu_dropout_out d = outs[o];
    const long long r = e - d.begin;
    const int c = (int)(r % d.C);
    const long long n = r / d.C;
    float v = 1.0f;
    if (d.site_a >= 0) v *= site_mult(sites, d.site_a, n * sites[d.site_a].C + d.off_a + c, seed, offset);
    if (d.site_b >= 0) v *= site_mult(sites, d.site_b, n * sites[d.site_b].C + d.off_b + (d.shuffled ? c / 4 : c), seed, offset);
    if (d.site_c >= 0) v *= site_mult(sites, d.site_c, n * sites[d.site_c].C + d.off_c + (d.shuffled ? c / 4 : c), seed, offset);
    buf[e] = v;
  }
}

}

extern "C" int slu_dropout_draw(const slu_dropout_site* sites, int nsites, const slu_dropout_out* outs, int nout, int N, unsigned long long seed,
                                unsigned long long offset, float* buf, long long total, slu_stream_t stream) {
  if (!sites || !outs || !buf || nsites <= 0 || nout <= 0 || N <= 0 || total <= 0) return SLU_EINVAL;
  const long long nb = (total + 255) / 256;
  hipLaunchKernelGGL(dropout_draw_kernel, dim3((unsigned)(nb > 4096 ? 4096 : nb)), dim3(256), 0, slu_stream(stream), sites, outs, nout, N, seed, offset,
                     buf, total);
  SLU_CHECK_LAUNCH();
}
```

semanticlidarunc_amd/graph_infer.py:

```python
from __future__ import annotations

import torch

from semanticlidarunc_amd.utils.mc_dropout import dropout_sampling


class GraphedMCPredict:
    def __init__(self, model: torch.nn.Module, example: torch.Tensor, T: int = 8, eps: float = 1e-12, warmup: int = 2):
        if not example.is_cuda or example.dim() != 4:
            raise RuntimeError("GraphedMCPredict: a [B, C, H, W] example tensor on the GPU is needed")
        model.eval()
        with torch.no_grad():
            ok = hasattr(model, "mc_fused_ok") and model.mc_fused_ok(example, T)
        if not ok:
            raise RuntimeError("GraphedMCPredict covers the fused half-precision MC path of SalsaNext (set_conv_precision('f16'), eval BatchNorm)")
        self.model, self.T, self.eps = model, int(T), float(eps)
        self._x = example.clone()
        n = self.T * example.shape[0]
        with dropout_sampling(model, enable=True):
            side = torch.cuda.Stream()
            side.wait_stream(torch.cuda.current_stream())
            with torch.cuda.stream(side), torch.no_grad():
                for _ in range(max(1, warmup)):
                    model.mc_predict_fused(self._x, self.T, self.eps, False)
            torch.cuda.current_stream().wait_stream(side)
            self._scales = None
            self._plan = None
            drawn = model._predraw_dropout(n, example.device)
            if drawn is not None:
                plan = model.__dict__.get("_drop_plan")
                if plan is None:
                    raise RuntimeError("GraphedMCPredict needs the one-launch dropout draw (SLU_DROPOUT_KERNEL=1)")
                self._plan, flags = plan[1], plan[2]
                self._buf = torch.empty(self._plan.total, dtype=torch.float32, device=example.device)
                self._scales = self._plan.run(out=self._buf)
                for k in flags:
                    self._scales[k] = True
            self.graph = torch.cuda.CUDAGraph()
            with torch.cuda.graph(self.graph), torch.no_grad():
                self._out = model.mc_predict_fused(self._x, self.T, self.eps, False, scales=self._scales if self._scales is not None else {})

    @torch.no_grad()
    def __call__(self, x: torch.Tensor):
        if x.shape != self._x.shape:
            raise RuntimeError(f"GraphedMCPredict: captured for {tuple(self._x.shape)}, got {tuple(x.shape)}")
        self._x.copy_(x)
        if self._plan is not None:
            self._plan.run(out=self._buf)
        self.graph.replay()
        return self._out
```

semanticlidarunc_amd/h8.py:

```python
from __future__ import annotations


import ctypes as C
from typing import NamedTuple, Optional, Sequence

import torch

from . import _lib, ops
from ._lib import ConvH8Desc, check
from .ops import _ptr, _req, _stream


class H8Source(NamedTuple):
    tensor: torch.Tensor
    scale: Optional[torch.Tensor] = None
    nbatch: int = 0


def _req_h8(t: torch.Tensor, name: str) -> torch.Tensor:
    _req(t, name, torch.float16)
    if t.dim() != 5 or t.shape[4] != 8:
        raise RuntimeError(f"{name}: expected an h8 tensor [N, G, H, W, 8], got {tuple(t.shape)}")
    return t


def to_h8(x: torch.Tensor, scale: Optional[torch.Tensor] = None) -> torch.Tensor:
    _req(x, "x")
    if x.dim() != 4:
        raise RuntimeError(f"x: expected NCHW, got {tuple(x.shape)}")
    n, c, h, w = x.shape
    if scale is not None:
        _req(scale, "scale")
        if tuple(scale.shape) != (n, c):
            raise RuntimeError(f"scale: expected {(n, c)}, got {tuple(scale.shape)}")
    y = torch.empty((n, (c + 7) // 8, h, w, 8), dtype=torch.float16, device=x.device)
    check(_lib.load().slu_nchw_to_h8(x.data_ptr(), _ptr(scale), y.data_ptr(), n, c, h, w, _stream()), "slu_nchw_to_h8")
    return y


def from_h8(x: torch.Tensor, channels: Optional[int] = None) -> torch.Tensor:
    _req_h8(x, "x")
    n, g, h, w, _ = x.shape
    c = 8 * g if channels is None else int(channels)
    if not 8 * (g - 1) < c <= 8 * g:
        raise RuntimeError(f"from_h8: {c} channels do not fit {g} blocks")
    y = torch.empty((n, c, h, w), dtype=torch.float32, device=x.device)
    check(_lib.load().slu_h8_to_nchw(x.data_ptr(), y.data_ptr(), n, c, h, w, _stream()), "slu_h8_to_nchw")
    return y


def pack_conv_weight_h8(weight: torch.Tensor) -> torch.Tensor:
    _req(weight, "weight")
    if weight.dim() != 4 or weight.shape[2] != weight.shape[3]:
        raise RuntimeError(f"weight: expected [Cout,Cin,k,k], got {tuple(weight.shape)}")
    lib = _lib.load()
    cout, cin, ks, _ = weight.shape
    nbytes = lib.slu_packed_weight_bytes_h8(cout, cin, ks)
    if nbytes == 0:
        raise RuntimeError("pack_conv_weight_h8: unsupported weight shape")
    out = torch.empty(nbytes, dtype=torch.uint8, device=weight.device)
    check(lib.slu_pack_conv_weight_h8(weight.data_ptr(), cout, cin, ks, out.data_ptr(), _stream()), "slu_pack_conv_weight_h8")
    return out


def conv2d_h8(srcs: Sequence[H8Source], wpack: torch.Tensor, cin: int, cout: int, ksize: int, dil: int, pad: int,
              bias: Optional[torch.Tensor] = None, slope: Optional[float] = None,
              bn_a: Optional[torch.Tensor] = None, bn_b: Optional[torch.Tensor] = None,
              resid: Optional[torch.Tensor] = None, out_f32_nchw: bool = False) -> torch.Tensor:
    lib = _lib.load()
    if not 1 <= len(srcs) <= _lib.MAX_SRC:
        raise RuntimeError(f"conv2d_h8: 1..{_lib.MAX_SRC} sources supported, got {len(srcs)}")
    d = ConvH8Desc()
    n = h = w = None
    gin = 0
    keep = []
    for i, s in enumerate(srcs):
        t = _req_h8(s.tensor, f"src[{i}]")
        sn, sg, sh, sw, _ = t.shape
        if s.nbatch:
            if i == 0 or sn != s.nbatch or n % sn:
                raise RuntimeError(f"src[{i}]: a batch-broadcast source must follow a full-batch source and divide N")
            sn = n
        if n is None:
            n, h, w = sn, sh, sw
        elif (sn, sh, sw) != (n, h, w):
            raise RuntimeError(f"src[{i}]: spatial/batch size {(sn, sh, sw)} != {(n, h, w)}")
        if s.scale is not None:
            _req(s.scale, f"src[{i}].scale")
            if tuple(s.scale.shape) != (n, 8 * sg):
                raise RuntimeError(f"src[{i}].scale: expected {(n, 8 * sg)}, got {tuple(s.scale.shape)}")
        d.src[i].ptr, d.src[i].scale, d.src[i].G, d.src[i].nbatch = t.data_ptr(), _ptr(s.scale), sg, int(s.nbatch)
        gin += sg
        keep.append(t)
    if not 8 * (gin - 1) < cin <= 8 * gin:
        raise RuntimeError(f"conv2d_h8: cin={cin} does not match {gin} input blocks")
    _req(wpack, "wpack", torch.uint8)
    if wpack.numel() != lib.slu_packed_weight_bytes_h8(cout, cin, ksize):
        raise RuntimeError(f"wpack: {wpack.numel()} bytes does not match Cout={cout} Cin={cin} k={ksize} (h8)")
    for t, nme in ((bias, "bias"), (bn_a, "bn_a"), (bn_b, "bn_b")):
        if t is not None:
            _req(t, nme)
            if t.numel() != cout:
                raise RuntimeError(f"{nme}: expected {cout} elements, got {t.numel()}")
    if (bn_a is None) != (bn_b is None):
        raise RuntimeError("bn_a and bn_b must be given together")
    gout = (cout + 7) // 8
    if out_f32_nchw:
        if resid is not None:
            raise RuntimeError("conv2d_h8: no residual on the fp32 NCHW output form")
        out = torch.empty((n, cout, h, w), dtype=torch.float32, device=keep[0].device)
    else:
        out = torch.empty((n, gout, h, w, 8), dtype=torch.float16, device=keep[0].device)
    if resid is not None:
        _req_h8(resid, "resid")
        if tuple(resid.shape) != (n, gout, h, w, 8):
            raise RuntimeError(f"resid: expected {(n, gout, h, w, 8)}, got {tuple(resid.shape)}")
    d.nsrc = len(srcs)
    d.N, d.H, d.W, d.Cout = n, h, w, cout
    d.ksize, d.dil, d.pad = ksize, dil, pad
    d.wpack, d.bias = wpack.data_ptr(), _ptr(bias)
    d.has_act, d.slope = (0, 0.0) if slope is None else (1, float(slope))
    d.bn_a, d.bn_b, d.resid, d.out = _ptr(bn_a), _ptr(bn_b), _ptr(resid), out.data_ptr()
    d.out_f32_nchw = 1 if out_f32_nchw else 0
    if ops.TIMING is None:
        check(lib.slu_conv2d_h8_fwd(C.byref(d), _stream()), "slu_conv2d_h8_fwd")
        return out
    buf = C.create_string_buffer(96)
    check(lib.slu_conv2d_h8_kernel_name(C.byref(d), buf, 96), "slu_conv2d_h8_kernel_name")
    e0, e1 = torch.cuda.Event(enable_timing=True), torch.cuda.Event(enable_timing=True)
    e0.record()
    check(lib.slu_conv2d_h8_fwd(C.byref(d), _stream()), "slu_conv2d_h8_fwd")
    e1.record()
    flops = 2.0 * cin * cout * ksize * ksize * n * h * w
    nbytes = n * h * w * (2.0 * cin + (4.0 if out_f32_nchw else 2.0) * cout) + 2.0 * cout * cin * ksize * ksize
    ops.TIMING.append((buf.value.decode(), flops, nbytes, e0, e1, nbytes + (n * h * w * 2.0 * cout if resid is not None else 0.0)))
    ops.TIMING_TAGS.append(f"N{n} {cin}->{cout} k{ksize}d{dil} {h}x{w}")
    return out


def conv_tail_supported(channels: int, h: int, w: int) -> bool:
    return bool(_lib.load().slu_conv_tail_h8_supported(int(channels), int(h), int(w)))


def conv_tail_shortcut_supported(channels: int, cin: int) -> bool:
# ... 27 lines not shown
    if resid is not None:
        _req_h8(resid, "resid")
        if resid.shape != a1.shape:
            raise RuntimeError(f"resid: expected {tuple(a1.shape)}, got {tuple(resid.shape)}")
    if shortcut is not None:
        sx, sw, sb, sslope, scin = shortcut
        if resid is not None:
            raise RuntimeError("conv_tail_h8: resid and shortcut are exclusive")
        if not conv_tail_shortcut_supported(c, scin):
            raise RuntimeError(f"conv_tail_h8: shortcut {scin} -> {c} is not covered (run the 1x1 conv and pass resid)")
        _req_h8(sx, "shortcut.x")
        _req(sw, "shortcut.w", torch.uint8)
        if tuple(sx.shape) != (n, scin // 8, h, w, 8) or sw.numel() != lib.slu_packed_weight_bytes_h8(c, scin, 1):
            raise RuntimeError("conv_tail_h8: shortcut operand sizes do not match")
        if sb is not None:
            _req(sb, "shortcut.bias")
            if sb.numel() != c:
                raise RuntimeError(f"shortcut.bias: expected {c} elements, got {sb.numel()}")
    out = torch.empty_like(a1)
    d.a1, d.a2, d.N, d.H, d.W, d.C = a1.data_ptr(), a2.data_ptr(), n, h, w, c
    if shortcut is not None:
        d.sc_x, d.sc_w, d.sc_bias, d.sc_cin = sx.data_ptr(), sw.data_ptr(), _ptr(sb), int(scin)
        d.sc_hasact, d.sc_slope = (0, 0.0) if sslope is None else (1, float(sslope))
    d.w2x2, d.w1x1 = w2x2.data_ptr(), w1x1.data_ptr()
    d.biasA, d.bnA_a, d.bnA_b = _ptr(bias_a), _ptr(None if bn_a is None else bn_a[0]), _ptr(None if bn_a is None else bn_a[1])
    d.biasB, d.bnB_a, d.bnB_b = _ptr(bias_b), _ptr(None if bn_b is None else bn_b[0]), _ptr(None if bn_b is None else bn_b[1])
    d.hasactA, d.slopeA = (0, 0.0) if slope_a is None else (1, float(slope_a))
    d.hasactB, d.slopeB = (0, 0.0) if slope_b is None else (1, float(slope_b))
    d.resid, d.out = _ptr(resid), out.data_ptr()
    if ops.TIMING is None:
        check(lib.slu_conv_tail_h8_fwd(C.byref(d), _stream()), "slu_conv_tail_h8_fwd")
        return out
    buf = C.create_string_buffer(96)
    check(lib.slu_conv_tail_h8_kernel_name(C.byref(d), buf, 96), "slu_conv_tail_h8_kernel_name")
    e0, e1 = torch.cuda.Event(enable_timing=True), torch.cuda.Event(enable_timing=True)
    e0.record()
    check(lib.slu_conv_tail_h8_fwd(C.byref(d), _stream()), "slu_conv_tail_h8_fwd")
    e1.record()
    scin = shortcut[4] if shortcut is not None else 0
    flops = 2.0 * c * (c * (4 + 3) + scin) * n * h * w
    nbytes = n * h * w * 2.0 * (c + c + 3 * c + c + (scin + c if shortcut is not None else 0)) + 2.0 * c * (c * (4 + 3) + scin)
    min_bytes = n * h * w * 2.0 * (c * 3 + (c if resid is not None else 0) + scin) + 2.0 * c * (c * (4 + 3) + scin)
    ops.TIMING.append((buf.value.decode(), flops, nbytes, e0, e1, min_bytes))
    ops.TIMING_TAGS.append(f"N{n} {c}->{c} k2d2 + {3 * c}->{c} k1" + (f" + {scin}->{c} k1 shortcut" if shortcut is not None else "") + f" fused {h}x{w}")
    return out


def ctx_block_supported(cin: int, c: int, h: int, w: int) -> bool:
    return bool(_lib.load().slu_ctx_block_h8_supported(int(cin), int(c), int(h), int(w)))


def ctx_block_h8(x: torch.Tensor, cin: int, w1: torch.Tensor, w2: torch.Tensor, w3: torch.Tensor, bias1: Optional[torch.Tensor],
                 bias2: Optional[torch.Tensor], bn1: Optional[tuple], bias3: Optional[torch.Tensor], bn2: Optional[tuple],
                 slope: float) -> torch.Tensor:
    lib = _lib.load()
    _req_h8(x, "x")
    n, g, h, w, _ = x.shape
    if not 8 * (g - 1) < cin <= 8 * g or not ctx_block_supported(cin, 32, h, w):
        raise RuntimeError(f"ctx_block_h8: cin={cin} with {g} input blocks is not covered by the fused kernel")
    for t, nme, shape in ((w1, "w1", (32, cin, 1)), (w2, "w2", (32, 32, 3)), (w3, "w3", (32, 32, 3))):
        _req(t, nme, torch.uint8)
        if t.numel() != lib.slu_packed_weight_bytes_h8(*shape):
            raise RuntimeError(f"{nme}: packed weight size does not match {shape}")
    vecs = (("bias1", bias1), ("bias2", bias2), ("bias3", bias3)) + tuple((f"bn{k}[{i}]", v) for k, pair in ((1, bn1), (2, bn2)) if pair is not None
                                                                           for i, v in enumerate(pair))
    for name, t in vecs:
        if t is not None:
            _req(t, name)
            if t.numel() != 32:
                raise RuntimeError(f"{name}: expected 32 elements, got {t.numel()}")
    out = torch.empty((n, 4, h, w, 8), dtype=torch.float16, device=x.device)
    d = _lib.CtxBlockH8Desc()
    d.x, d.N, d.H, d.W, d.Cin, d.C = x.data_ptr(), n, h, w, int(cin), 32
    d.w1, d.w2, d.w3 = w1.data_ptr(), w2.data_ptr(), w3.data_ptr()
    d.bias1, d.bias2, d.bias3 = _ptr(bias1), _ptr(bias2), _ptr(bias3)
    d.bn1_a, d.bn1_b = _ptr(None if bn1 is None else bn1[0]), _ptr(None if bn1 is None else bn1[1])
    d.bn2_a, d.bn2_b = _ptr(None if bn2 is None else bn2[0]), _ptr(None if bn2 is None else bn2[1])
    d.slope, d.out = float(slope), out.data_ptr()
    if ops.TIMING is None:
        check(lib.slu_ctx_block_h8_fwd(C.byref(d), _stream()), "slu_ctx_block_h8_fwd")
        return out
    e0, e1 = torch.cuda.Event(enable_timing=True), torch.cuda.Event(enable_timing=True)
    e0.record()
    check(lib.slu_ctx_block_h8_fwd(C.byref(d), _stream()), "slu_ctx_block_h8_fwd")
    e1.record()
    px = float(n * h * w)
    flops = 2.0 * (cin * 32 + 2 * 9 * 32 * 32) * px
    nbytes = px * 2.0 * ((8 * g + 32) + (32 + 32) + (32 + 32)) + 2.0 * (32 * cin + 2 * 9 * 32 * 32)
    min_bytes = px * 2.0 * (8 * g + 32) + 2.0 * (32 * cin + 2 * 9 * 32 * 32)
    ops.TIMING.append((f"ctx_h8_kernel<{1 if cin <= 16 else 2}>", flops, nbytes, e0, e1, min_bytes))
    ops.TIMING_TAGS.append(f"N{n} {cin}->32 k1 + 32->32 k3d1 + 32->32 k3d2 fused {h}x{w}")
    return out


def head_mc_h8(x: torch.Tensor, wpack: torch.Tensor, bias: Optional[torch.Tensor], classes: int, passes: int, batch: int, eps: float = 1e-12):
    _req_h8(x, "x")
    n, g, h, w, _ = x.shape
    if n != passes * batch:
        raise RuntimeError(f"head_mc_h8: {n} images != T * B = {passes} * {batch}")
    lib = _lib.load()
    _req(wpack, "wpack", torch.uint8)
    if wpack.numel() != lib.slu_packed_weight_bytes_h8(classes, 8 * g, 1):
        raise RuntimeError("head_mc_h8: packed weight size does not match the head")
    if bias is not None:
        _req(bias, "bias")
        if bias.numel() != classes:
            raise RuntimeError(f"bias: expected {classes} elements, got {bias.numel()}")
    dev = x.device
    p_bar = torch.empty((batch, classes, h, w), dtype=torch.float32, device=dev)
    hn = torch.empty((batch, h, w), dtype=torch.float32, device=dev)
    mi = torch.empty((batch, h, w), dtype=torch.float32, device=dev)
    preds = torch.empty((batch, h, w), dtype=torch.int64, device=dev)
    args = (x.data_ptr(), passes, batch, g, h * w, wpack.data_ptr(), _ptr(bias), classes, float(eps), p_bar.data_ptr(), hn.data_ptr(),
            mi.data_ptr(), preds.data_ptr(), _stream())
    if ops.TIMING is None:
        check(lib.slu_head_mc_h8(*args), "slu_head_mc_h8")
        return p_bar, hn, mi, preds
    e0, e1 = torch.cuda.Event(enable_timing=True), torch.cuda.Event(enable_timing=True)
    e0.record()
    check(lib.slu_head_mc_h8(*args), "slu_head_mc_h8")
    e1.record()
    flops = 2.0 * 8 * g * classes * n * h * w
    nbytes = n * h * w * (2.0 * 8 * g + 4.0 * classes) + 2.0 * classes * 8 * g
    min_bytes = n * h * w * 2.0 * 8 * g + batch * h * w * (4.0 * classes + 16.0) + 2.0 * classes * 8 * g
    ops.TIMING.append((f"head_mc_h8_kernel<{g // 2}>", flops, nbytes, e0, e1, min_bytes))
    ops.TIMING_TAGS.append(f"N{n} {8 * g}->{classes} k1 head + MC reduce T={passes} {h}x{w}")
    return p_bar, hn, mi, preds


def avgpool3s2_h8(x: torch.Tensor, scale: Optional[torch.Tensor] = None, n_out: Optional[int] = None) -> torch.Tensor:
    _req_h8(x, "x")
    b, g, h, w, _ = x.shape
    n = b if n_out is None else int(n_out)
    if n % b:
        raise RuntimeError("avgpool3s2_h8: n_out must be a multiple of the input batch")
    if scale is not None:
        _req(scale, "scale")
        if tuple(scale.shape) != (n, 8 * g):
            raise RuntimeError(f"scale: expected {(n, 8 * g)}, got {tuple(scale.shape)}")
    y = torch.empty((n, g, (h + 1) // 2, (w + 1) // 2, 8), dtype=torch.float16, device=x.device)
    check(_lib.load().slu_avgpool3s2_h8(x.data_ptr(), _ptr(scale), y.data_ptr(), n, 0 if n == b else b, g, h, w, _stream()),
          "slu_avgpool3s2_h8")
# ... 16 lines not shown
```

semanticlidarunc_amd/ops.py:

```python
from __future__ import annotations

import ctypes as C
from typing import NamedTuple, Optional, Sequence

import torch

from . import _lib
from ._lib import ConvDesc, check

INT64_MIN = -(2 ** 63)

TIMING = None
TIMING_TAGS = []


def _stream() -> int:
    return torch.cuda.current_stream().cuda_stream


def _req(t: torch.Tensor, name: str, dtype=torch.float32) -> torch.Tensor:
    if not isinstance(t, torch.Tensor):
        raise TypeError(f"{name}: expected a torch.Tensor, got {type(t).__name__}")
    if not t.is_cuda:
        raise RuntimeError(f"{name}: tensor is on '{t.device}'; the HIP path only runs on a GPU (no CPU fallback)")
# ... 1194 lines not shown
    _req(label, "label", torch.int32)
    _req(lut, "lut", torch.int32)
    _req(bad_count, "bad_count", torch.int32)
    if xyzi.dim() != 2 or xyzi.shape[1] != 4 or label.dim() != 1 or label.numel() != xyzi.shape[0] or xyzi.shape[0] == 0:
        raise RuntimeError(f"kitti_decode: xyzi [N, 4] / label [N] expected, got {tuple(xyzi.shape)} / {tuple(label.shape)}")
    n = xyzi.shape[0]
    pc = torch.empty((n, 5), dtype=torch.float64, device=xyzi.device)
    ang = 0.0 if rotate_deg is None else math.radians(float(rotate_deg))
    if rotate_deg is not None:
        import numpy as np
        ang = float(np.radians(float(rotate_deg)))
        ca, sa = float(np.cos(ang)), float(np.sin(ang))
    else:
        ca, sa = 1.0, 0.0
    check(_lib.load().slu_kitti_decode(xyzi.data_ptr(), label.data_ptr(), n, lut.data_ptr(), lut.numel(), 0 if rotate_deg is None else 1, ca, sa,
                                       pc.data_ptr(), bad_count.data_ptr(), _stream()), "slu_kitti_decode")
    return pc


def range_image_split(img: torch.Tensor, normals: Optional[torch.Tensor], range_out, refl_out, xyz_out, normals_out, labels_out) -> None:
    _req(img, "img")
    h, w, c = img.shape
    for t, nme, shape, dt in ((range_out, "range_out", (1, h, w), torch.float32), (refl_out, "refl_out", (1, h, w), torch.float32),
                              (xyz_out, "xyz_out", (3, h, w), torch.float32), (labels_out, "labels_out", (1, h, w), torch.int64)):
        _req(t, nme, dt)
        if tuple(t.shape) != shape:
            raise RuntimeError(f"{nme}: expected {shape}, got {tuple(t.shape)}")
    if normals is not None:
        _req(normals, "normals")
        _req(normals_out, "normals_out")
        if tuple(normals.shape) != (h, w, 3) or tuple(normals_out.shape) != (3, h, w):
            raise RuntimeError("normals: expected [H, W, 3] in and [3, H, W] out")
    check(_lib.load().slu_range_image_split(img.data_ptr(), _ptr(normals), h, w, c, range_out.data_ptr(), refl_out.data_ptr(), xyz_out.data_ptr(),
                                            _ptr(normals_out) if normals is not None else None, labels_out.data_ptr(), _stream()), "slu_range_image_split")


class DropoutPlan:

    def __init__(self, n: int, sites, outs, device):
        import numpy as np
        self.n, self.device = int(n), device
        st = np.zeros(len(sites), dtype=np.dtype([("begin", "<i8"), ("C", "<i4"), ("active", "<i4"), ("p", "<f4"), ("reserved", "<i4")]))
        g = 0
        for i, (c, p, active) in enumerate(sites):
            st[i] = (g, c, 1 if active else 0, p, 0)
            if active:
                g += self.n * c
        self.draws = g
        ot = np.zeros(len(outs), dtype=np.dtype([("begin", "<i8"), ("C", "<i4"), ("site_a", "<i4"), ("off_a", "<i4"), ("site_b", "<i4"), ("off_b", "<i4"),
                                                 ("site_c", "<i4"), ("off_c", "<i4"), ("shuffled", "<i4")]))
        e, self.slices = 0, []
        for i, (key, c, refs, shuffled) in enumerate(outs):
            refs = list(refs) + [(-1, 0)] * (3 - len(refs))
            ot[i] = (e, c, refs[0][0], refs[0][1], refs[1][0], refs[1][1], refs[2][0], refs[2][1], 1 if shuffled else 0)
            self.slices.append((key, e, c))
            e += self.n * c
        self.total = e
        assert st.dtype.itemsize == 24 and ot.dtype.itemsize == 40
        self.sites = torch.from_numpy(st.view(np.uint8).copy()).to(device)
        self.outs = torch.from_numpy(ot.view(np.uint8).copy()).to(device)
        self.nsites, self.nout = len(sites), len(outs)

    def run(self, out: Optional[torch.Tensor] = None):
        gen = torch.cuda.default_generators[self.device.index if self.device.index is not None else torch.cuda.current_device()]
        seed, off = int(gen.initial_seed()), int(gen.get_offset())
        adv = ((self.draws + 3) // 4 + 3) // 4 * 4
        gen.set_offset(off + adv)
        if out is None:
            buf = torch.empty(self.total, dtype=torch.float32, device=self.device)
        else:
            buf = _req(out, "out")
            if buf.numel() != self.total:
                raise RuntimeError(f"DropoutPlan.run: out holds {buf.numel()} elements, the plan needs {self.total}")
        check(_lib.load().slu_dropout_draw(self.sites.data_ptr(), self.nsites, self.outs.data_ptr(), self.nout, self.n, seed & (2 ** 64 - 1), off, buf.data_ptr(),
                                           self.total, _stream()), "slu_dropout_draw")
        return {key: buf[b:b + self.n * c].view(self.n, c) for key, b, c in self.slices}


def dwconv3x3(x: torch.Tensor, w: torch.Tensor, bias: Optional[torch.Tensor], stride: int = 1, act: str = "none") -> torch.Tensor:
    _req(x, "x")
    _req(w, "w")
    n, c, h, wd = x.shape
    if tuple(w.shape) != (c, 9) or (bias is not None and bias.numel() != c):
        raise RuntimeError(f"dwconv3x3: weight {tuple(w.shape)} / bias do not match {c} channels")
    if bias is not None:
        _req(bias, "bias")
    oh, ow = (h + stride - 1) // stride, (wd + stride - 1) // stride
    y = torch.empty((n, c, oh, ow), dtype=torch.float32, device=x.device)
    check(_lib.load().slu_dwconv3x3_fwd(x.data_ptr(), w.data_ptr(), _ptr(bias), y.data_ptr(), n, c, h, wd, int(stride), {"none": 0, "silu": 3}[act],
                                        _stream()), "slu_dwconv3x3_fwd")
    return y


def dwconv3x3_wgrad(x: torch.Tensor, dy: torch.Tensor) -> torch.Tensor:
    _req(x, "x")
    _req(dy, "dy")
    if x.shape != dy.shape:
        raise RuntimeError("dwconv3x3_wgrad: x / dy shape mismatch")
    n, c, h, w = x.shape
    dw = torch.empty((c, 9), dtype=torch.float32, device=x.device)
    check(_lib.load().slu_dwconv3x3_wgrad(x.data_ptr(), dy.data_ptr(), dw.data_ptr(), n, c, h, w, _stream()), "slu_dwconv3x3_wgrad")
    return dw


def global_avgpool(x: torch.Tensor) -> torch.Tensor:
    _req(x, "x")
    n, c, h, w = x.shape
# ... 20 lines not shown
```

semanticlidarunc_amd/salsanext.py:

```python
from __future__ import annotations

import os
from typing import Dict, Optional

import torch
import torch.nn as nn

from . import autograd as _autograd
from . import h8, ops
from .autograd import AvgPoolFn, ConvLayerFn, LayerCfg
from .ops import ConvSource

_SLOPE = 0.01

CONV_PRECISIONS = ("fp32", "f16x3", "f16")
_CONV_PRECISION = os.environ.get("SLU_CONV_PRECISION", "fp32")
_TRAIN_CONV_PRECISION = os.environ.get("SLU_TRAIN_CONV_PRECISION", "fp32")
_FUSE_TAIL = os.environ.get("SLU_FUSE_TAIL", "1") != "0"
_FUSE_TAIL_MAX_C = int(os.environ.get("SLU_FUSE_TAIL_MAX_C", "64"))
_FUSE_SHORTCUT = os.environ.get("SLU_FUSE_SHORTCUT", "1") != "0"
_FUSE_CTX = os.environ.get("SLU_FUSE_CTX", "1") != "0"
_PACK_MULTI = os.environ.get("SLU_PACK_MULTI", "1") != "0"
_FUSE_HEAD_MC = os.environ.get("SLU_FUSE_HEAD_MC", "1") != "0"


def set_train_conv_precision(precision: str) -> None:
    global _TRAIN_CONV_PRECISION
    if precision not in ("fp32", "f16x3"):
        raise ValueError(f"unknown training conv precision {precision!r}; choose 'fp32' or 'f16x3'")
    _TRAIN_CONV_PRECISION = precision



def set_conv_precision(precision: str) -> None:
    global _CONV_PRECISION
    if precision not in CONV_PRECISIONS:
        raise ValueError(f"unknown conv precision {precision!r}; choose from {CONV_PRECISIONS}")
    _CONV_PRECISION = precision


def get_conv_precision() -> str:
    return _CONV_PRECISION


class _Prepared:

    __slots__ = ("key", "wpack", "bn_key", "bn_a", "bn_b", "dgrad", "key16", "wpack16", "key8", "wpack8")

    def __init__(self):
        self.key = self.bn_key = None
        self.wpack = self.bn_a = self.bn_b = None
        self.key16 = self.wpack16 = None
        self.key8 = self.wpack8 = None
        self.dgrad = {}


def _tkey(*ts):
    return tuple((t.data_ptr(), t._version, t.device) for t in ts)


class _FusedBlock(nn.Module):

    def __call__(self, *args, **kwargs):
        _autograd.nbt_scope_enter()
        try:
            return super().__call__(*args, **kwargs)
        finally:
            _autograd.nbt_scope_exit()

    def _folded_bn(self, p: _Prepared, bn: Optional[nn.BatchNorm2d]):
        if bn is None:
            return None, None
        bkey = _tkey(bn.weight, bn.bias, bn.running_mean, bn.running_var)
        if p.bn_key != bkey:
            p.bn_a, p.bn_b = ops.bn_fold(bn.weight.detach(), bn.bias.detach(), bn.running_mean, bn.running_var, bn.eps)
            p.bn_key = bkey
        return p.bn_a, p.bn_b

    def _run_h8(self, p: _Prepared, conv: nn.Conv2d, bn, srcs, resid, act, out_f32):
        wkey = _tkey(conv.weight)
        if p.key8 != wkey:
            p.wpack8 = h8.pack_conv_weight_h8(conv.weight.detach().contiguous())
            p.key8 = wkey
        bn_a, bn_b = self._folded_bn(p, bn)
        return h8.conv2d_h8([h8.H8Source(s.tensor, s.scale, s.nbatch) for s in srcs], p.wpack8, conv.in_channels,
                            conv.out_channels, conv.kernel_size[0], conv.dilation[0], conv.padding[0],
                            bias=None if conv.bias is None else conv.bias.detach(), slope=_SLOPE if act else None,
                            bn_a=bn_a, bn_b=bn_b, resid=resid, out_f32_nchw=out_f32)

    def _prepared(self, conv: nn.Conv2d) -> _Prepared:
        cache: Dict[str, _Prepared] = self.__dict__.setdefault("_prep", {})
        p = cache.get(str(id(conv)))
        if p is None:
            p = cache[str(id(conv))] = _Prepared()
        return p

    def _tail_is_fused(self, conv_a: nn.Conv2d, conv_b: nn.Conv2d, a1) -> bool:
        c = conv_a.out_channels
        return bool(_FUSE_TAIL and a1.dtype == torch.float16 and a1.dim() == 5 and conv_a.kernel_size == (2, 2) and conv_a.dilation == (2, 2)
                    and conv_b.kernel_size == (1, 1) and conv_b.in_channels == 3 * c and conv_b.out_channels == c
                    and c <= _FUSE_TAIL_MAX_C and h8.conv_tail_supported(c, a1.shape[2], a1.shape[3]))

    def _run_tail(self, conv_a: nn.Conv2d, bn_a, conv_b: nn.Conv2d, bn_b, a1, a2, resid=None, shortcut=None):
        if self._tail_is_fused(conv_a, conv_b, a1):
            packs, folded = [], []
            for conv, bn in ((conv_a, bn_a), (conv_b, bn_b)):
                p = self._prepared(conv)
                wkey = _tkey(conv.weight)
                if p.key8 != wkey:
                    p.wpack8 = h8.pack_conv_weight_h8(conv.weight.detach().contiguous())
                    p.key8 = wkey
                packs.append(p.wpack8)
                fa, fb = self._folded_bn(p, bn)
                folded.append(None if fa is None else (fa, fb))
            sc = None
            if shortcut is not None:
                sx, sconv = shortcut
                p = self._prepared(sconv)
                wkey = _tkey(sconv.weight)
                if p.key8 != wkey:
                    p.wpack8 = h8.pack_conv_weight_h8(sconv.weight.detach().contiguous())
                    p.key8 = wkey
                sc = (sx, p.wpack8, None if sconv.bias is None else sconv.bias.detach(), _SLOPE, sconv.in_channels)
            return h8.conv_tail_h8(a1, a2, packs[0], packs[1], None if conv_a.bias is None else conv_a.bias.detach(), _SLOPE, folded[0],
                                   None if conv_b.bias is None else conv_b.bias.detach(), _SLOPE, folded[1], resid=resid, shortcut=sc)
        if shortcut is not None:
            resid = self._run(shortcut[1], None, [ConvSource(shortcut[0])])
        a3 = self._run(conv_a, bn_a, [ConvSource(a2)])
        return self._run(conv_b, bn_b, [ConvSource(a1), ConvSource(a2), ConvSource(a3)], resid=resid)

    def _run(self, conv: nn.Conv2d, bn: Optional[nn.BatchNorm2d], srcs, resid=None, act=True, out_f32=False):
        cache: Dict[str, _Prepared] = self.__dict__.setdefault("_prep", {})
        name = str(id(conv))
        p = cache.get(name)
        if p is None:
            p = cache[name] = _Prepared()
        if srcs[0].tensor.dtype == torch.float16:
            return self._run_h8(p, conv, bn, srcs, resid, act, out_f32)
        wkey = _tkey(conv.weight)
        if p.key != wkey:
            p.wpack = ops.pack_conv_weight(conv.weight.detach().contiguous())
            p.key = wkey
        k = conv.kernel_size[0]
        slope = _SLOPE if act else None
        wants_grad = torch.is_grad_enabled() and (
            conv.weight.requires_grad or any(s.tensor.requires_grad for s in srcs)
            or (resid is not None and resid.requires_grad) or (bn is not None and bn.weight.requires_grad))
        if wants_grad or (bn is not None and bn.training):
            wp = p.wpack
            if _TRAIN_CONV_PRECISION == "f16x3":
                if p.key16 != wkey:
                    p.wpack16 = ops.pack_conv_weight_f16x3(conv.weight.detach().contiguous())
                    p.key16 = wkey
                wp = p.wpack16
            cfg = LayerCfg(k, conv.dilation[0], conv.padding[0], slope, [s.scale for s in srcs],
                           [s.pixel_shuffle for s in srcs], bn, conv.out_channels, wp, p.dgrad, _TRAIN_CONV_PRECISION)
            return ConvLayerFn.apply(cfg, conv.weight, conv.bias, None if bn is None else bn.weight,
                                     None if bn is None else bn.bias, resid, *[s.tensor for s in srcs])
        bn_a, bn_b = self._folded_bn(p, bn)
        wpack, precision = p.wpack, "fp32"
        if _CONV_PRECISION == "f16x3":
            precision = "f16x3"
            if p.key16 != wkey:
                p.wpack16 = ops.pack_conv_weight_f16x3(conv.weight.detach().contiguous())
                p.key16 = wkey
            wpack = p.wpack16
        return ops.conv2d_fused(srcs, wpack, conv.out_channels, k, conv.dilation[0], conv.padding[0],
                                bias=None if conv.bias is None else conv.bias.detach(),
                                slope=slope, bn_a=bn_a, bn_b=bn_b, resid=resid, precision=precision)


_DROPOUT_KERNEL = os.environ.get("SLU_DROPOUT_KERNEL", "1") != "0"


def _draw(drop: nn.Dropout2d, n: int, c: int, device, override: Optional[Dict[str, torch.Tensor]], name: str):
    if override is not None:
        s = override.get(name)
        return None if s is None else s.reshape(n, c).to(device=device, dtype=torch.float32).contiguous()
    if not drop.training or drop.p == 0.0:
        return None
    return drop(torch.ones((n, c, 1, 1), dtype=torch.float32, device=device)).reshape(n, c)


def _mul(a, b):
    if a is None:
        return b
    if b is None:
        return a
    return a * b


class ResContextBlock(_FusedBlock):
    def __init__(self, in_filters, out_filters):
        super().__init__()
        self.conv1 = nn.Conv2d(in_filters, out_filters, 1)
        self.conv2 = nn.Conv2d(out_filters, out_filters, 3, padding=1)
        self.bn1 = nn.BatchNorm2d(out_filters)
        self.conv3 = nn.Conv2d(out_filters, out_filters, 3, dilation=2, padding=2)
        self.bn2 = nn.BatchNorm2d(out_filters)

    def forward(self, x):
        if (_FUSE_CTX and x.dtype == torch.float16 and x.dim() == 5 and self.conv1.out_channels == 32
                and h8.ctx_block_supported(self.conv1.in_channels, 32, x.shape[2], x.shape[3])):
            packs, folded = [], []
            for conv, bn in ((self.conv1, None), (self.conv2, self.bn1), (self.conv3, self.bn2)):
                p = self._prepared(conv)
                wkey = _tkey(conv.weight)
                if p.key8 != wkey:
                    p.wpack8 = h8.pack_conv_weight_h8(conv.weight.detach().contiguous())
                    p.key8 = wkey
                packs.append(p.wpack8)
                fa, fb = self._folded_bn(p, bn)
                folded.append(None if fa is None else (fa, fb))
            b = [None if c.bias is None else c.bias.detach() for c in (self.conv1, self.conv2, self.conv3)]
            return h8.ctx_block_h8(x, self.conv1.in_channels, packs[0], packs[1], packs[2], b[0], b[1], folded[1], b[2], folded[2], _SLOPE)
        shortcut = self._run(self.conv1, None, [ConvSource(x)])
        a1 = self._run(self.conv2, self.bn1, [ConvSource(shortcut)])
        return self._run(self.conv3, self.bn2, [ConvSource(a1)], resid=shortcut)


class ResBlock(_FusedBlock):
    def __init__(self, in_filters, out_filters, dropout_rate, kernel_size=(3, 3), stride=1, pooling=True, drop_out=True):
        super().__init__()
        if stride != 1 or tuple(kernel_size) != (3, 3):
            raise ValueError("only the stride-1 / 3x3-pool configuration of the reference is implemented")
        self.pooling, self.drop_out = pooling, drop_out
        self.conv1 = nn.Conv2d(in_filters, out_filters, 1)
        self.conv2 = nn.Conv2d(in_filters, out_filters, 3, padding=1)
        self.bn1 = nn.BatchNorm2d(out_filters)
        self.conv3 = nn.Conv2d(out_filters, out_filters, 3, dilation=2, padding=2)
        self.bn2 = nn.BatchNorm2d(out_filters)
        self.conv4 = nn.Conv2d(out_filters, out_filters, 2, dilation=2, padding=1)
        self.bn3 = nn.BatchNorm2d(out_filters)
        self.conv5 = nn.Conv2d(out_filters * 3, out_filters, 1)
        self.bn4 = nn.BatchNorm2d(out_filters)
        self.dropout = nn.Dropout2d(p=dropout_rate)

    def features(self, x):
        src = [ConvSource(x)]
        fuse_sc = (_FUSE_SHORTCUT and x.dtype == torch.float16 and x.dim() == 5 and x.shape[1] * 8 == self.conv1.in_channels
                   and h8.conv_tail_shortcut_supported(self.conv1.out_channels, self.conv1.in_channels))
        shortcut = None if fuse_sc else self._run(self.conv1, None, src)
        a1 = self._run(self.conv2, self.bn1, src)
        a2 = self._run(self.conv3, self.bn2, [ConvSource(a1)])
        if fuse_sc and self._tail_is_fused(self.conv4, self.conv5, a1):
            return self._run_tail(self.conv4, self.bn3, self.conv5, self.bn4, a1, a2, shortcut=(x, self.conv1))
        if shortcut is None:
            shortcut = self._run(self.conv1, None, src)
        return self._run_tail(self.conv4, self.bn3, self.conv5, self.bn4, a1, a2, resid=shortcut)

    def forward(self, x, _scales=None, _name=""):
        full = self.features(x)
        s = None
        if self.drop_out:
            s = _draw(self.dropout, full.shape[0], self.conv5.out_channels, full.device, _scales, _name + ".dropout")
        if self.pooling:
            if full.dtype == torch.float16:
                return h8.avgpool3s2_h8(full, s), full
            pooled = AvgPoolFn.apply(full, s) if (torch.is_grad_enabled() and full.requires_grad) else ops.avgpool3s2(full, s)
            return pooled, full
        return full, s


class UpBlock(_FusedBlock):
    def __init__(self, in_filters, out_filters, dropout_rate, drop_out=True):
        super().__init__()
        self.drop_out, self.in_filters, self.out_filters = drop_out, in_filters, out_filters
        self.dropout1 = nn.Dropout2d(p=dropout_rate)
        self.dropout2 = nn.Dropout2d(p=dropout_rate)
        self.conv1 = nn.Conv2d(in_filters // 4 + 2 * out_filters, out_filters, 3, padding=1)
        self.bn1 = nn.BatchNorm2d(out_filters)
        self.conv2 = nn.Conv2d(out_filters, out_filters, 3, dilation=2, padding=2)
        self.bn2 = nn.BatchNorm2d(out_filters)
        self.conv3 = nn.Conv2d(out_filters, out_filters, 2, dilation=2, padding=1)
        self.bn3 = nn.BatchNorm2d(out_filters)
        self.conv4 = nn.Conv2d(out_filters * 3, out_filters, 1)
        self.bn4 = nn.BatchNorm2d(out_filters)
        self.dropout3 = nn.Dropout2d(p=dropout_rate)

    def _compose_scales(self, x_scale, d1, d2):
        cu = self.in_filters // 4
        sx, ss = x_scale, None
        up = d1
        if d2 is not None:
            up = _mul(up, d2[:, :cu])
            ss = d2[:, cu:].contiguous()
        if up is not None:
            sx = _mul(sx, up.repeat_interleave(4, dim=1))
        return sx, ss

    def forward(self, x, skip, x_scale=None, _scales=None, _name="", skip_nbatch=0):
        n, cx, dev = x.shape[0], self.in_filters, x.device
        cu, cs = cx // 4, self.conv1.in_channels - cx // 4
        if _scales is not None and _scales.get(_name + "._composed"):
            sx, ss = _scales.get(_name + "._sx"), _scales.get(_name + "._ss")
        elif self.drop_out:
            sx, ss = self._compose_scales(x_scale, _draw(self.dropout1, n, cu, dev, _scales, _name + ".dropout1"),
                                          _draw(self.dropout2, n, cu + cs, dev, _scales, _name + ".dropout2"))
        else:
            sx, ss = x_scale, None
        if x.dtype == torch.float16:
            xs = h8.pixel_shuffle_h8(x, None if sx is None else sx.contiguous())
            e1 = self._run(self.conv1, self.bn1, [ConvSource(xs), ConvSource(skip, ss, False, skip_nbatch)])
        else:
            if sx is not None:
                sx = sx.contiguous()
            e1 = self._run(self.conv1, self.bn1, [ConvSource(x, sx, True), ConvSource(skip, ss, False, skip_nbatch)])
        e2 = self._run(self.conv2, self.bn2, [ConvSource(e1)])
        out = self._run_tail(self.conv3, self.bn3, self.conv4, self.bn4, e1, e2)
        s3 = None
        if self.drop_out:
            s3 = _draw(self.dropout3, n, self.out_filters, dev, _scales, _name + ".dropout3")
        return out, s3


class SalsaNext(_FusedBlock):
    def __init__(self, nclasses, nchannels=5):
        super().__init__()
        self.nclasses = nclasses
        self.downCntx = ResContextBlock(nchannels, 32)
        self.downCntx2 = ResContextBlock(32, 32)
        self.downCntx3 = ResContextBlock(32, 32)
        self.resBlock1 = ResBlock(32, 64, 0.2, pooling=True, drop_out=False)
        self.resBlock2 = ResBlock(64, 128, 0.2, pooling=True)
        self.resBlock3 = ResBlock(128, 256, 0.2, pooling=True)
        self.resBlock4 = ResBlock(256, 256, 0.2, pooling=True)
        self.resBlock5 = ResBlock(256, 256, 0.2, pooling=False)
        self.upBlock1 = UpBlock(256, 128, 0.2)
        self.upBlock2 = UpBlock(128, 128, 0.2)
        self.upBlock3 = UpBlock(128, 64, 0.2)
        self.upBlock4 = UpBlock(64, 32, 0.2, drop_out=False)
        self.logits = nn.Conv2d(32, nclasses, 1)
        self.tail_act = nn.Softmax(dim=1)

    def forward(self, x):
        return self._forward(x, None)

    def forward_with_dropout_scales(self, x, scales: Dict[str, torch.Tensor]):
        return self._forward(x, scales)

    def _head(self, u1):
        if self.__dict__.get("_features_only", False):
            return u1
        return self._run(self.logits, None, [ConvSource(u1)], act=False, out_f32=True)

    def mc_fused_ok(self, x, T: int) -> bool:
        return (_FUSE_HEAD_MC and _CONV_PRECISION == "f16" and isinstance(x, torch.Tensor) and x.dim() == 4 and x.is_cuda
                and (x.shape[2] * x.shape[3]) % 32 == 0 and self.logits.out_channels <= 32 and self._inference_only())

    @torch.no_grad()
    def mc_predict_fused(self, x, T: int, eps: float = 1e-12, share_prefix: bool = False, scales=None):
        b = x.shape[0]
        self.__dict__["_features_only"] = True
        try:
            u1 = self.forward_mc(x, T, scales) if share_prefix else self._forward(x.repeat(int(T), 1, 1, 1), scales)
        finally:
            self.__dict__["_features_only"] = False
        p = self._prepared(self.logits)
        wkey = _tkey(self.logits.weight)
        if p.key8 != wkey:
            p.wpack8 = h8.pack_conv_weight_h8(self.logits.weight.detach().contiguous())
            p.key8 = wkey
        return h8.head_mc_h8(u1, p.wpack8, None if self.logits.bias is None else self.logits.bias.detach(), self.logits.out_channels,
                             int(T), b, eps)

    @torch.no_grad()
    def forward_mc(self, x, T: int, scales: Optional[Dict[str, torch.Tensor]] = None):
        if self.training or any(m.training for m in self.modules() if isinstance(m, nn.BatchNorm2d)):
            raise RuntimeError("forward_mc needs eval-mode BatchNorm (use utils.mc_dropout.mc_forward)")
        if not isinstance(x, torch.Tensor) or x.dim() != 4 or not x.is_cuda:
            raise RuntimeError("forward_mc expects a [B, C, H, W] tensor on the GPU")
        if x.shape[2] % 16 or x.shape[3] % 16:
            raise RuntimeError("SalsaNext needs H and W divisible by 16")
        b = x.shape[0]
        n = int(T) * b
        x = x.contiguous().float()
        half = _CONV_PRECISION == "f16"
        if scales is None and not torch.cuda.is_current_stream_capturing():
            scales = self._predraw_dropout(n, x.device)
        if half:
            x = h8.to_h8(x)
        d = self.downCntx3(self.downCntx2(self.downCntx(x)))
        d0c, d0b = self.resBlock1(d, scales, "resBlock1")
        full2 = self.resBlock2.features(d0c)
        self._join_dropout()
        s2 = _draw(self.resBlock2.dropout, n, self.resBlock2.conv5.out_channels, x.device, scales, "resBlock2.dropout")
        d1c = h8.avgpool3s2_h8(full2, s2, n) if half else ops.avgpool3s2_bcast(full2, s2, n)
        d2c, d2b = self.resBlock3(d1c, scales, "resBlock3")
        d3c, d3b = self.resBlock4(d2c, scales, "resBlock4")
        d5c, s5 = self.resBlock5(d3c, scales, "resBlock5")
        u4, s = self.upBlock1(d5c, d3b, s5, scales, "upBlock1")
        u3, s = self.upBlock2(u4, d2b, s, scales, "upBlock2")
        u2, s = self.upBlock3(u3, full2, s, scales, "upBlock3", skip_nbatch=b)
        u1, _ = self.upBlock4(u2, d0b, s, scales, "upBlock4", skip_nbatch=b)
        return self._head(u1)

    def _inference_only(self) -> bool:
        if any(m.training for m in self.modules() if isinstance(m, nn.BatchNorm2d)):
            return False
        return not (torch.is_grad_enabled() and any(p.requires_grad for p in self.parameters()))

    _DROPOUT_SITES = (("resBlock2", "dropout", 128), ("resBlock3", "dropout", 256), ("resBlock4", "dropout", 256), ("resBlock5", "dropout", 256),
                      ("upBlock1", "dropout1", 64), ("upBlock1", "dropout2", 320), ("upBlock1", "dropout3", 128),
                      ("upBlock2", "dropout1", 32), ("upBlock2", "dropout2", 288), ("upBlock2", "dropout3", 128),
                      ("upBlock3", "dropout1", 32), ("upBlock3", "dropout2", 160), ("upBlock3", "dropout3", 64))

    def _predraw_dropout(self, n: int, device):
        sites = [(f"{blk}.{name}", getattr(getattr(self, blk), name), c) for blk, name, c in self._DROPOUT_SITES]
        if not any(d.training and d.p > 0.0 for _, d, _ in sites):
            return None
        if _DROPOUT_KERNEL:
            return self._predraw_dropout_kernel(n, device, sites)
        main = torch.cuda.current_stream(device)
        side = self.__dict__.get("_drop_stream")
        if side is None or side.device != device:
            side = self.__dict__["_drop_stream"] = torch.cuda.Stream(device)
        out: Dict[str, torch.Tensor] = {}
        with torch.cuda.stream(side):
            for key, drop, c in sites:
                s = _draw(drop, n, c, device, None, key)
                if s is not None:
                    s.record_stream(main)
                    out[key] = s
            prod = out.get("resBlock5.dropout")
            for blk in ("upBlock1", "upBlock2", "upBlock3", "upBlock4"):
                sx, ss = getattr(self, blk)._compose_scales(prod, out.get(f"{blk}.dropout1"), out.get(f"{blk}.dropout2"))
                for key, t in ((f"{blk}._sx", sx), (f"{blk}._ss", ss)):
                    if t is not None:
                        t.record_stream(main)
                        out[key] = t
                out[f"{blk}._composed"] = True
                prod = out.get(f"{blk}.dropout3")
        self.__dict__["_drop_event"] = side.record_event()
        return out

    def _predraw_dropout_kernel(self, n: int, device, sites):
        sig = (n, str(device), tuple((bool(d.training), float(d.p)) for _, d, _ in sites))
        plan = self.__dict__.get("_drop_plan")
        if plan is None or plan[0] != sig:
            index = {key: i for i, (key, _, _) in enumerate(sites)}
            active = {key: bool(d.training and d.p > 0.0) for key, d, _ in sites}
            chans = {key: c for key, _, c in sites}
            outs = []

            def add(key, c, refs, shuffled=False):
                refs = [(index[k], off) for k, off in refs if k is not None and active.get(k, False)]
                if refs:
                    outs.append((key, c, refs, shuffled))

            for blk in ("resBlock2", "resBlock3", "resBlock4", "resBlock5"):
                add(f"{blk}.dropout", chans[f"{blk}.dropout"], [(f"{blk}.dropout", 0)])
            prod = "resBlock5.dropout"
            for blk in ("upBlock1", "upBlock2", "upBlock3", "upBlock4"):
                m = getattr(self, blk)
                cu, cs = m.in_filters // 4, m.conv1.in_channels - m.in_filters // 4
                d1, d2, d3 = (f"{blk}.dropout{k}" if f"{blk}.dropout{k}" in index else None for k in (1, 2, 3))
                add(f"{blk}._sx", m.in_filters, [(prod, 0), (d1, 0), (d2, 0)], shuffled=True)
                add(f"{blk}._ss", cs, [(d2, cu)])
                if d3 is not None:
                    add(f"{blk}.dropout3", chans[d3], [(d3, 0)])
                prod = d3
            fixed = []
            for key, c, refs, shuffled in outs:
                if shuffled and (len(refs) < 1 or refs[0][0] != index.get(self._sx_producer(key), -2)):
                    refs = [(-1, 0)] + refs
                fixed.append((key, c, refs[:3], shuffled))
            plan = (sig, ops.DropoutPlan(n, [(c, float(d.p), bool(d.training and d.p > 0.0)) for _, d, c in sites], fixed, device),
                    [f"{blk}._composed" for blk in ("upBlock1", "upBlock2", "upBlock3", "upBlock4")])
            self.__dict__["_drop_plan"] = plan
        out = plan[1].run()
        for k in plan[2]:
            out[k] = True
        return out

    @staticmethod
    def _sx_producer(key: str):
        return {"upBlock1._sx": "resBlock5.dropout", "upBlock2._sx": "upBlock1.dropout3", "upBlock3._sx": "upBlock2.dropout3",
                "upBlock4._sx": "upBlock3.dropout3"}.get(key)

    def _pack_training_weights(self):
        if not _PACK_MULTI or _TRAIN_CONV_PRECISION != "fp32":
            return
        owners = [(m, c) for m in self.modules() if isinstance(m, _FusedBlock) for c in m.children() if isinstance(c, nn.Conv2d)]
        weights = [c.weight for _, c in owners]
        if not weights or not all(w.is_cuda and w.dtype == torch.float32 and w.is_contiguous() for w in weights):
            return
        keys = [_tkey(w) for w in weights]
        plan = self.__dict__.get("_pack_plan")
        if plan is None or not plan.matches(weights):
            plan = self.__dict__["_pack_plan"] = ops.WeightPackPlan([w.detach() for w in weights])
            self.__dict__["_pack_keys"] = None
        if self.__dict__.get("_pack_keys") != keys:
            plan.run()
            self.__dict__["_pack_keys"] = keys
        for i, ((m, c), w, k) in enumerate(zip(owners, weights, keys)):
            p = m._prepared(c)
            p.wpack, p.key = plan.fwd[i], k
            p.dgrad["pack"], p.dgrad["key"] = plan.dgrad[i], (w.data_ptr(), w._version)

    def _join_dropout(self):
        ev = self.__dict__.pop("_drop_event", None)
        if ev is not None:
            torch.cuda.current_stream().wait_event(ev)

    def _forward(self, x, scales):
        if not isinstance(x, torch.Tensor) or x.dim() != 4:
            raise RuntimeError("SalsaNext expects a [B, C, H, W] tensor")
        if not x.is_cuda:
            raise RuntimeError("semanticlidarunc_amd.SalsaNext runs on MI355X only: input is on "
                               f"'{x.device}' and there is no CPU fallback")
        if x.shape[2] % 16 or x.shape[3] % 16:
            raise RuntimeError("SalsaNext needs H and W divisible by 16")
        x = x.contiguous().float()
        if not self._inference_only():
            self._pack_training_weights()
        if scales is None and (self._inference_only() or _DROPOUT_KERNEL) and not torch.cuda.is_current_stream_capturing():
            scales = self._predraw_dropout(x.shape[0], x.device)
        if _CONV_PRECISION == "f16" and self._inference_only():
            x = h8.to_h8(x)
        d = self.downCntx(x)
        d = self.downCntx2(d)
        d = self.downCntx3(d)
        d0c, d0b = self.resBlock1(d, scales, "resBlock1")
        self._join_dropout()
        d1c, d1b = self.resBlock2(d0c, scales, "resBlock2")
        d2c, d2b = self.resBlock3(d1c, scales, "resBlock3")
        d3c, d3b = self.resBlock4(d2c, scales, "resBlock4")
        d5c, s5 = self.resBlock5(d3c, scales, "resBlock5")
        u4, s = self.upBlock1(d5c, d3b, s5, scales, "upBlock1")
        u3, s = self.upBlock2(u4, d2b, s, scales, "upBlock2")
        u2, s = self.upBlock3(u3, d1b, s, scales, "upBlock3")
        u1, _ = self.upBlock4(u2, d0b, s, scales, "upBlock4")
        return self._head(u1)
```

Before: 706.0 scans/s.

## Read pixel-shuffled decoder inputs in place and broadcast the shared MC input

Producers now write decoder block outputs in a stored permuted order. The following 3x3 conv then reads the pixel shuffle directly by computing shuffled addresses in its load stage, with dropout multipliers indexed by sub-pixel parity. This removes the separate pixel_shuffle_h8 pass and its extra activation round trip. Separately, the context block can broadcast a single input across T passes through an nbatch modulo instead of materialising x.repeat. Together these add more index arithmetic, LDS for the multipliers and new support constraints.

```diff
diff --git a/include/slu.h b/include/slu.h
--- a/include/slu.h
+++ b/include/slu.h
@@ -8,7 +8,7 @@
 extern "C" {
 #endif
 
-#define SLU_ABI_VERSION 32
+#define SLU_ABI_VERSION 33
 
 #define SLU_OK            0
 #define SLU_EINVAL       -1
@@ -154,6 +154,8 @@
   const float* scale;
   int32_t G;
   int32_t nbatch;
+  int32_t shuffle;
+  int32_t reserved;
 } slu_h8_src;
 
 typedef struct slu_conv_h8_desc {
@@ -212,6 +214,7 @@
   const float *bias3, *bn2_a, *bn2_b;
   float slope;
   void* out;
+  int32_t nbatch;
 } slu_ctx_block_h8_desc;
 int slu_ctx_block_h8_supported(int Cin, int C, int H, int W);
 int slu_ctx_block_h8_fwd(const slu_ctx_block_h8_desc* desc, slu_stream_t stream);
diff --git a/semanticlidarunc_amd/_lib.py b/semanticlidarunc_amd/_lib.py
--- a/semanticlidarunc_amd/_lib.py
+++ b/semanticlidarunc_amd/_lib.py
@@ -3,7 +3,7 @@
 import ctypes as C
 import os
 
-ABI_VERSION = 32
+ABI_VERSION = 33
 MAX_SRC = 3
 _HERE = os.path.dirname(os.path.abspath(__file__))
 LIB_PATH = os.path.join(_HERE, "libslu_hip.so")
@@ -37,7 +37,8 @@
 
 
 class H8Src(C.Structure):
-    _fields_ = [("ptr", C.c_void_p), ("scale", C.c_void_p), ("G", C.c_int32), ("nbatch", C.c_int32)]
+    _fields_ = [("ptr", C.c_void_p), ("scale", C.c_void_p), ("G", C.c_int32), ("nbatch", C.c_int32), ("shuffle", C.c_int32),
+                ("reserved", C.c_int32)]
 
 
 class ConvH8Desc(C.Structure):
@@ -84,6 +85,7 @@
         ("bias3", C.c_void_p), ("bn2_a", C.c_void_p), ("bn2_b", C.c_void_p),
         ("slope", C.c_float),
         ("out", C.c_void_p),
+        ("nbatch", C.c_int32),
     ]
 
 
diff --git a/semanticlidarunc_amd/csrc/conv2d_h8.hip b/semanticlidarunc_amd/csrc/conv2d_h8.hip
--- a/semanticlidarunc_amd/csrc/conv2d_h8.hip
+++ b/semanticlidarunc_amd/csrc/conv2d_h8.hip
@@ -26,6 +26,7 @@
   int G;
   int gbeg;
   int nb;
+  int shuf;
 };
 
 struct H8Args {
@@ -216,6 +217,8 @@
   static_assert(OPT == 0 || (MB == 2 && WM == 2 && WN == 4 && !F32OUT), "OPT: the 8-wave 128-channel configuration only");
   static_assert(KPC <= 2, "pc_rc carries 2 bits of channel block");
   static_assert(KPC == 1 || ONE, "multi-K-step chunks: single-source layers only");
+  constexpr bool SHUF = SCALED && KS == 3 && DIL == 1 && PAD == 1 && !ONE && KPC == 1;
+  static_assert(!SHUF || (WN * RPW) % 2 == 0, "tile rows start on even image rows");
 
   extern __shared__ __attribute__((aligned(16))) char smem[];
   float* s_epi = reinterpret_cast<float*>(smem);
@@ -313,14 +316,20 @@
   constexpr int NPIECE = NIB + (WRES ? 0 : NIA);
   constexpr int PPT = (NPIECE + TS - 1) / TS;
   uintptr_t st_b0 = 0, st_b1 = 0;
+  bool st_sh = false;
+  const int hw4 = (a.H >> 1) * (a.W >> 1), w2 = a.W >> 1;
   int st_g0 = 0;
   bool st_on = false;
   int st_x0 = 0, st_y0 = 0, st_q = 0, st_wave = wave;
   uint4 *st_db = s_b, *st_da = s_a;
   auto stage_begin = [&](const TilePos& tp, int q, int buf) __attribute__((always_inline)) {
     const int img[SLU_MAX_SRC] = {tp.i0, tp.i1, tp.i2};
-    const long long org = (long long)(tp.y0 - PAD) * a.W + (tp.x0 - PAD);
+    long long org = (long long)(tp.y0 - PAD) * a.W + (tp.x0 - PAD);
     st_g0 = 2 * KPC * q;
+    if constexpr (SHUF) {
+      st_sh = a.src[0].shuf && st_g0 < a.src[0].G;
+      if (st_sh) org = 0;
+    }
     if constexpr (ONE) {
       st_b0 = reinterpret_cast<uintptr_t>(a.src[0].ptr) + 16 * ((long long)(((size_t)tp.n * a.src[0].G + st_g0) * HW) + org);
       st_b1 = st_b0;
@@ -347,7 +356,11 @@
         const int gsel = (rc >> 16) & 3;
         const uintptr_t gb = (!ONE && gsel == 1) ? st_b1 : st_b0;
         const bool ok = (rc >> 20) && st_g0 + gsel < a.Gin && (unsigned)gy < (unsigned)a.H && (unsigned)gx < (unsigned)a.W;
-        const uintptr_t src = ok ? gb + 16 * (long long)pc_off[i] : zero_addr;
+        int off = pc_off[i];
+        if constexpr (SHUF) {
+          if (st_sh) off = gsel * (int)HW + (2 * (gy & 1) + (gx & 1)) * hw4 + (gy >> 1) * w2 + (gx >> 1);
+        }
+        const uintptr_t src = ok ? gb + 16 * (long long)off : zero_addr;
         SLU_GLDS16(reinterpret_cast<const uint4*>(src), st_db + blk * 64);
       }
     } else if constexpr (!WRES) {
@@ -372,9 +385,24 @@
       half8 h;
 #pragma unroll
       for (int k = 0; k < 8; ++k) h[k] = (_Float16)1.0f;
-      if (tid < a.Gin) {
+      int g = tid;
+      bool stored0 = false;
+      if constexpr (SHUF) {
+        if (a.src[0].shuf) {
+          stored0 = tid < 4 * a.src[0].G;
+          g = stored0 ? 0 : tid - 3 * a.src[0].G;
+        }
+      }
+      if (stored0) {
+        if (a.src[0].scale) {
+          const float* sp = a.src[0].scale + ((size_t)n * 4 * a.src[0].G + tid) * 8;
+          const float4 s0 = *reinterpret_cast<const float4*>(sp), s1 = *reinterpret_cast<const float4*>(sp + 4);
+          h[0] = (_Float16)s0.x; h[1] = (_Float16)s0.y; h[2] = (_Float16)s0.z; h[3] = (_Float16)s0.w;
+          h[4] = (_Float16)s1.x; h[5] = (_Float16)s1.y; h[6] = (_Float16)s1.z; h[7] = (_Float16)s1.w;
+        }
+      } else if (g < a.Gin) {
         int img[SLU_MAX_SRC] = {0, 0, 0};
-        const SrcSel p = select_src(a, img, tid);
+        const SrcSel p = select_src(a, img, g);
         if (p.scale) {
           const float* sp = p.scale + ((size_t)n * p.G + p.gl) * 8;
           const float4 s0 = *reinterpret_cast<const float4*>(sp), s1 = *reinterpret_cast<const float4*>(sp + 4);
@@ -457,8 +485,23 @@
       H8_PROF_MARK(2)
       const uint4* sb = s_b + buf * NB_ALLOC + bbase;
       const uint4* sa = s_a + abase + (WRES ? q * T * 64 : buf * NREC_A);
-      half8 sc;
-      if constexpr (SCALED) sc = __builtin_bit_cast(half8, s_scale[spar * 64 + 2 * q + hh]);
+      half8 scm[SHUF ? 2 : 1][SHUF ? 2 : 1];
+      if constexpr (SHUF) {
+        const int g0s = a.src[0].shuf ? a.src[0].G : 0;
+        if (2 * q < g0s) {
+#pragma unroll
+          for (int yr = 0; yr < 2; ++yr)
+#pragma unroll
+            for (int xr = 0; xr < 2; ++xr)
+              scm[yr][xr] = __builtin_bit_cast(half8, s_scale[spar * 64 + 4 * (2 * q + hh) + 2 * ((yr + wn * RPW + 1) & 1) + ((jj + xr + 1) & 1)]);
+        } else {
+          scm[0][0] = __builtin_bit_cast(half8, s_scale[spar * 64 + 3 * g0s + 2 * q + hh]);
+          scm[0][1] = scm[1][0] = scm[1][1] = scm[0][0];
+        }
+      } else if constexpr (SCALED) {
+        scm[0][0] = __builtin_bit_cast(half8, s_scale[spar * 64 + 2 * q + hh]);
+      }
+      auto sc_of = [&](int b, int dy, int dx) __attribute__((always_inline)) -> half8 { return SHUF ? scm[((b >> 1) + dy) & 1][dx & 1] : scm[0][0]; };
       {
         if constexpr (MB == 2 && WM == 2 && WN == 4) {
           half8 af[2][MB], bf[2][NB];
@@ -470,7 +513,7 @@
 #pragma unroll
             for (int b = 0; b < NB; ++b) {
               bf[set][b] = __builtin_bit_cast(half8, sb[j * 2 * REC + ((b >> 1) + dy) * LW + (b & 1) * 32 + dx]);
-              if constexpr (SCALED) bf[set][b] *= sc;
+              if constexpr (SCALED) bf[set][b] *= sc_of(b, dy, dx);
             }
           };
           read_frags(0, 0);
@@ -504,7 +547,7 @@
 #pragma unroll
             for (int b = 0; b < NB; ++b) {
               bf[set][b] = __builtin_bit_cast(half8, sb[((b >> 1) + dy) * LW + (b & 1) * 32 + dx]);
-              if constexpr (SCALED) bf[set][b] *= sc;
+              if constexpr (SCALED) bf[set][b] *= sc_of(b, dy, dx);
             }
           };
           read_frags(0, 0);
@@ -534,7 +577,7 @@
 #pragma unroll
             for (int b = 0; b < NB; ++b) {
               half8 bf = __builtin_bit_cast(half8, sb[((b >> 1) + dy) * LW + (b & 1) * 32 + dx]);
-              if constexpr (SCALED) bf *= sc;
+              if constexpr (SCALED) bf *= sc_of(b, dy, dx);
 #pragma unroll
               for (int i = 0; i < MB; ++i) acc[i][b] = __builtin_amdgcn_mfma_f32_32x32x16_f16(af[i], bf, acc[i][b], 0, 0, 0);
             }
@@ -1081,12 +1124,14 @@
   int g = 0;
   for (int s = 0; s < d->nsrc; ++s) {
     const slu_h8_src& S = d->src[s];
-    if (!S.ptr || S.G <= 0 || S.nbatch < 0) return SLU_EINVAL;
+    if (!S.ptr || S.G <= 0 || S.nbatch < 0 || (S.shuffle != 0 && S.shuffle != 1)) return SLU_EINVAL;
     if (((uintptr_t)S.ptr & 15) || ((uintptr_t)S.scale & 15)) return SLU_EINVAL;
-    a.src[s] = H8Src{reinterpret_cast<const uint4*>(S.ptr), S.scale, S.G, g, S.nbatch};
-    g += S.G;
-  }
-  for (int s = d->nsrc; s < SLU_MAX_SRC; ++s) a.src[s] = H8Src{nullptr, nullptr, 0, 0x7fffffff, 0};
+    if (S.shuffle && (s != 0 || S.G % 8 || (d->H & 1) || (d->W & 1) || S.nbatch)) return SLU_EINVAL;
+    const int gc = S.shuffle ? S.G / 4 : S.G;
+    a.src[s] = H8Src{reinterpret_cast<const uint4*>(S.ptr), S.scale, gc, g, S.nbatch, S.shuffle};
+    g += gc;
+  }
+  for (int s = d->nsrc; s < SLU_MAX_SRC; ++s) a.src[s] = H8Src{nullptr, nullptr, 0, 0x7fffffff, 0, 0};
   if (((uintptr_t)d->out & 15) || ((uintptr_t)d->resid & 15) || ((uintptr_t)d->wpack & 15)) return SLU_EINVAL;
   if (d->resid && d->out_f32_nchw) return SLU_EINVAL;
   a.nsrc = d->nsrc;
@@ -1115,6 +1160,10 @@
   const size_t lds = (size_t)3 * MBLK * 32 * 4 + (SCALED ? 2048 : 0) + 2 * nb_alloc * 16 + (size_t)MBLK * (WRES ? a.nks : 2 * KPC) * T * 64 * 16;
   if (lds > 160 * 1024) return SLU_EUNSUPPORTED;
   if (SCALED && a.Gin > 64) return SLU_EUNSUPPORTED;
+  if (a.src[0].shuf) {
+    if (!(SCALED && KS == 3 && DIL == 1 && PAD == 1 && !ONE && KPC == 1 && !F32OUT)) return SLU_EUNSUPPORTED;
+    if (3 * a.src[0].G + a.Gin > 64) return SLU_EUNSUPPORTED;
+  }
   a.tiles_x = (a.W + 63) / 64;
   a.tiles_y = (a.H + TH - 1) / TH;
   static const int order = [] { const char* e = getenv("SLU_H8_ORDER"); return e ? atoi(e) : 1; }();
@@ -1149,6 +1198,8 @@
   float slope;
   uint4* out;
   int N, H, W, tiles_x, tiles_y;
+  int shuf;
+  const float* sc0;
 };
 
 template <int NKS, int NIB, int P, int NST>
@@ -1179,6 +1230,7 @@
   uint4* s_w = reinterpret_cast<uint4*>(smem);
   uint4* s_ring = s_w + MB * NKS * T * 64;
   uint4* s_trash = s_ring + D * BUFREC;
+  uint4* s_mul = s_trash + 64;
 
   const int tid = threadIdx.x, lane = tid & 63, wave = __builtin_amdgcn_readfirstlane(tid >> 6), wn = wave;
   const int hh = lane >> 5, jj = lane & 31;
@@ -1201,6 +1253,19 @@
     s_epi[2 * C + tid] = a.bn_a ? a.bn_b[tid] : 0.0f;
   }
   for (int blk = wave; blk < MB * NKS * T; blk += NWAVE) SLU_GLDS16(a.wpack + (size_t)blk * 64 + lane, s_w + blk * 64);
+  const bool mul0 = NKS == 5 && a.shuf && a.sc0;
+  if constexpr (NKS == 5) {
+    if (mul0) {
+      for (int e = tid; e < a.N * 4 * a.G0; e += 64 * NWAVE) {
+        const float4 s0 = *reinterpret_cast<const float4*>(a.sc0 + (size_t)e * 8), s1 = *reinterpret_cast<const float4*>(a.sc0 + (size_t)e * 8 + 4);
+        half8 h;
+        h[0] = (_Float16)s0.x; h[1] = (_Float16)s0.y; h[2] = (_Float16)s0.z; h[3] = (_Float16)s0.w;
+        h[4] = (_Float16)s1.x; h[5] = (_Float16)s1.y; h[6] = (_Float16)s1.z; h[7] = (_Float16)s1.w;
+        s_mul[e] = __builtin_bit_cast(uint4, h);
+      }
+    }
+  }
+  const int hw4 = (a.H >> 1) * (a.W >> 1), w2 = a.W >> 1;
 
   struct TilePos { int x0, y0, n; };
   auto decode = [&](int t) {
@@ -1226,8 +1291,9 @@
     const bool second = 2 * c >= a.G0;
     const uint4* src = second ? a.x1 : a.x;
     const int gs = second ? a.G1 : a.G0, g = second ? 2 * c - a.G0 : 2 * c;
+    const bool sh = NKS == 5 && a.shuf && !second;
     const uintptr_t base0 = reinterpret_cast<uintptr_t>(src) +
-                            16 * ((long long)(((size_t)tp.n * gs + g) * HW) + (long long)(tp.y0 - PAD) * a.W + (tp.x0 - PAD));
+                            16 * ((long long)(((size_t)tp.n * gs + g) * HW) + (sh ? 0ll : (long long)(tp.y0 - PAD) * a.W + (tp.x0 - PAD)));
     const uintptr_t base1 = base0 + 16 * (long long)HW;
 #pragma unroll
     for (int i = 0; i < NIB; ++i) {
@@ -1235,7 +1301,11 @@
       const int rc = pc_rc[i];
       const int gy = tp.y0 - PAD + (rc & 255), gx = tp.x0 - PAD + ((rc >> 8) & 255);
       const bool ok = valid && (rc >> 17) && (unsigned)gy < (unsigned)a.H && (unsigned)gx < (unsigned)a.W;
-      const uintptr_t p = ok ? (((rc >> 16) & 1) ? base1 : base0) + (long long)pc_off[i] : zero;
+      int off = pc_off[i];
+      if constexpr (NKS == 5) {
+        if (sh) off = 16 * ((2 * (gy & 1) + (gx & 1)) * hw4 + (gy >> 1) * w2 + (gx >> 1));
+      }
+      const uintptr_t p = ok ? (((rc >> 16) & 1) ? base1 : base0) + (long long)off : zero;
       SLU_GLDS16(reinterpret_cast<const uint4*>(p), (NBLK_B % NWAVE == 0 || blk < NBLK_B) ? db + blk * 64 : s_trash);
     }
     asm volatile("" ::: "memory");
@@ -1279,12 +1349,28 @@
       const uint4* sb = s_ring + rslot * BUFREC + bbase;
       rslot = rslot + 1 == D ? 0 : rslot + 1;
       half8 fa[2][MB], fb[2][NB];
+      constexpr bool MUL = NKS == 5 && c == 0 && RPW == 1 && DIL == 1;
+      half8 msc[MUL ? 2 : 1][MUL ? 2 : 1];
+      if constexpr (MUL) {
+        if (mul0) {
+#pragma unroll
+          for (int ty = 0; ty < 2; ++ty)
+#pragma unroll
+            for (int tx = 0; tx < 2; ++tx)
+              msc[ty][tx] = __builtin_bit_cast(half8, s_mul[cur.n * 4 * a.G0 + 4 * hh + 2 * ((wn + ty + 1) & 1) + ((jj + tx + 1) & 1)]);
+        }
+      }
       auto rd = [&](int tap, int buf) {
         const int dy = (tap / KS) * DIL, dx = (tap % KS) * DIL;
 #pragma unroll
         for (int i = 0; i < MB; ++i) fa[buf][i] = __builtin_bit_cast(half8, s_w[((i * NKS + c) * T + tap) * 64 + lane]);
 #pragma unroll
-        for (int b = 0; b < NB; ++b) fb[buf][b] = __builtin_bit_cast(half8, sb[((b >> 1) + dy) * LW + (b & 1) * 32 + dx]);
+        for (int b = 0; b < NB; ++b) {
+          fb[buf][b] = __builtin_bit_cast(half8, sb[((b >> 1) + dy) * LW + (b & 1) * 32 + dx]);
+          if constexpr (MUL) {
+            if (mul0) fb[buf][b] *= msc[(tap / KS) & 1][(tap % KS) & 1];
+          }
+        }
       };
       rd(0, 0);
 #pragma unroll
@@ -1344,9 +1430,15 @@
 int launch_ring3(const H8Args& h, const slu_conv_h8_desc* d, const SluEmit& e) {
   constexpr int TH = 8 * RPW, PAD = DIL;
   constexpr size_t nblk_b = (size_t)(2 * (TH + 2 * PAD) * (64 + 2 * PAD) + 63) / 64;
-  constexpr size_t lds = ((size_t)MB * NKS * 9 * 64 + (size_t)D * nblk_b * 64 + 64) * 16;
-  static_assert(lds + 3 * 32 * MB * 4 <= 160 * 1024, "ring does not fit in LDS");
+  constexpr size_t lds0 = ((size_t)MB * NKS * 9 * 64 + (size_t)D * nblk_b * 64 + 64) * 16;
+  static_assert(lds0 + 3 * 32 * MB * 4 <= 160 * 1024, "ring does not fit in LDS");
+  const bool shuf = h.src[0].shuf != 0;
+  if (shuf && (NKS != 5 || RPW != 1 || DIL != 1 || h.src[0].G != 2)) return SLU_EUNSUPPORTED;
+  const size_t lds = lds0 + ((shuf && h.src[0].scale) ? (size_t)h.N * 4 * h.src[0].G * 16 : 0);
+  if (lds + 3 * 32 * MB * 4 > 160 * 1024) return -1;
   RingArgs a{};
+  a.shuf = shuf ? 1 : 0;
+  a.sc0 = shuf ? h.src[0].scale : nullptr;
   a.x = h.src[0].ptr; a.G0 = h.src[0].G;
   a.x1 = h.nsrc > 1 ? h.src[1].ptr : h.src[0].ptr; a.G1 = h.nsrc > 1 ? h.src[1].G : 0;
   a.wpack = h.wpack; a.bias = h.bias; a.bn_a = h.bn_a; a.bn_b = h.bn_b;
@@ -1371,9 +1463,10 @@
   if (off || d->ksize != 3 || d->pad != d->dil || (d->dil != 1 && d->dil != 2) || a.nsrc < 1 || a.nsrc > 2) return false;
   int gsum = 0;
   for (int s = 0; s < a.nsrc; ++s) {
-    if (a.src[s].scale || a.src[s].nb) return false;
+    if ((a.src[s].scale && !a.src[s].shuf) || a.src[s].nb) return false;
     gsum += a.src[s].G;
   }
+  if (a.src[0].shuf && !(a.nsrc == 2 && a.Gin == 10 && a.src[0].G == 2)) return false;
   if (gsum != a.Gin || (a.nsrc == 2 && (a.src[0].G & 1)) || a.out_f32 || d->resid || (a.has_act & ~1)) return false;
   if ((a.has_act & 1) && !(a.slope >= 0.0f && a.slope <= 1.0f)) return false;
   return (a.Cout == 32 || a.Cout == 64) && ((a.Gin == 4 || a.Gin == 8) || (a.Gin == 10 && a.Cout == 32 && d->dil == 1));
@@ -1553,6 +1646,14 @@
   H8Args a{};
   const int rc = fill_h8(d, a);
   if (rc != SLU_OK) return rc;
+  if (a.src[0].shuf) {
+    if (ring3_ok(d, a)) {
+      const int rc2 = launch_ring3_any(a, d, e);
+      if (rc2 != -1) return rc2;
+    }
+    if (!any_scale(d) || d->ksize != 3 || d->dil != 1 || d->pad != 1 || a.out_f32) return SLU_EUNSUPPORTED;
+    return launch_h8_family<3, 1, 1>(a, d, choose_h8(a), true, e);
+  }
   if (gemm1x1_ok(d, a)) return a.Cout == 128 ? launch_gemm1x1<2, GEMM1X1_D128>(a, d, e) : launch_gemm1x1<4, GEMM1X1_D256>(a, d, e);
   if (stream_ok(d, a)) {
     if (a.nmblk <= 2) {
diff --git a/semanticlidarunc_amd/csrc/ctx_block_h8.hip b/semanticlidarunc_amd/csrc/ctx_block_h8.hip
--- a/semanticlidarunc_amd/csrc/ctx_block_h8.hip
+++ b/semanticlidarunc_amd/csrc/ctx_block_h8.hip
@@ -16,6 +16,7 @@
   float slope;
   uint2* out;
   int N, H, W, Gin;
+  int nb;
   int strips_x, nseg, seg_rows;
 };
 
@@ -125,7 +126,7 @@
   }
   const int i_w1 = opaque(OFF_W1 + lane), i_w2 = opaque(OFF_W2 + lane), i_w3 = opaque(OFF_W3 + lane), i_epi = opaque(OFF_EPI + hh);
 
-  struct Band { int x0, y0, n, j, r1; };
+  struct Band { int x0, y0, n, xn, j, r1; };
   auto decode = [&](int t) {
     Band p;
     const int tx = t % a.strips_x;
@@ -133,6 +134,7 @@
     p.x0 = tx * TW;
     p.y0 = (t % a.nseg) * a.seg_rows;
     p.n = t / a.nseg;
+    p.xn = a.nb > 0 ? p.n % a.nb : p.n;
     p.j = 0;
     p.r1 = min(a.H, p.y0 + a.seg_rows);
     return p;
@@ -151,7 +153,7 @@
       for (int k = 0; k < NKS1; ++k) {
         const int g = 2 * k + hh;
         const bool ok = in && g < a.Gin;
-        xr[i][k] = *(ok ? a.x + (long long)(((size_t)bd.n * a.Gin + g) * HW) + org + p1_goff[i] : &g_zero_rec_c);
+        xr[i][k] = *(ok ? a.x + (long long)(((size_t)bd.xn * a.Gin + g) * HW) + org + p1_goff[i] : &g_zero_rec_c);
       }
     }
   };
@@ -436,6 +438,7 @@
   if (!slu_ctx_block_h8_supported(d->Cin, d->C, d->H, d->W)) return SLU_EUNSUPPORTED;
   if (!(d->slope >= 0.0f && d->slope <= 1.0f)) return SLU_EINVAL;
   if (d->x == d->out) return SLU_EINVAL;
+  if (d->nbatch < 0 || (d->nbatch > 0 && d->N % d->nbatch)) return SLU_EINVAL;
   CtxArgs a{};
   a.x = reinterpret_cast<const uint4*>(d->x);
   a.w1 = reinterpret_cast<const uint4*>(d->w1);
@@ -445,6 +448,7 @@
   a.slope = d->slope;
   a.out = reinterpret_cast<uint2*>(d->out);
   a.N = d->N; a.H = d->H; a.W = d->W; a.Gin = (d->Cin + 7) / 8;
+  a.nb = d->nbatch;
   hipStream_t st = slu_stream(stream);
   return d->Cin <= 16 ? launch_ctx<1>(a, st) : launch_ctx<2>(a, st);
 }
diff --git a/semanticlidarunc_amd/csrc/dropout_draw.hip b/semanticlidarunc_amd/csrc/dropout_draw.hip
--- a/semanticlidarunc_amd/csrc/dropout_draw.hip
+++ b/semanticlidarunc_amd/csrc/dropout_draw.hip
@@ -36,8 +36,9 @@
     while (o + 1 < nout && e >= outs[o + 1].begin) ++o;
     const slu_dropout_out d = outs[o];
     const long long r = e - d.begin;
-    const int c = (int)(r % d.C);
+    int c = (int)(r % d.C);
     const long long n = r / d.C;
+    if (d.shuffled == 2) c = 32 * (c >> 5) + 4 * (c & 7) + ((c >> 3) & 3);
     float v = 1.0f;
     if (d.site_a >= 0) v *= site_mult(sites, d.site_a, n * sites[d.site_a].C + d.off_a + c, seed, offset);
     if (d.site_b >= 0) v *= site_mult(sites, d.site_b, n * sites[d.site_b].C + d.off_b + (d.shuffled ? c / 4 : c), seed, offset);
diff --git a/semanticlidarunc_amd/graph_infer.py b/semanticlidarunc_amd/graph_infer.py
--- a/semanticlidarunc_amd/graph_infer.py
+++ b/semanticlidarunc_amd/graph_infer.py
@@ -26,7 +26,7 @@
             torch.cuda.current_stream().wait_stream(side)
             self._scales = None
             self._plan = None
-            drawn = model._predraw_dropout(n, example.device)
+            drawn = model._predraw_dropout(n, example.device, sx_stored=model._in_place_blocks(n, example.shape[2], example.shape[3]))
             if drawn is not None:
                 plan = model.__dict__.get("_drop_plan")
                 if plan is None:
diff --git a/semanticlidarunc_amd/h8.py b/semanticlidarunc_amd/h8.py
--- a/semanticlidarunc_amd/h8.py
+++ b/semanticlidarunc_amd/h8.py
@@ -15,6 +15,51 @@
     tensor: torch.Tensor
     scale: Optional[torch.Tensor] = None
     nbatch: int = 0
+    shuffle: bool = False
+
+
+def shuffle_store_perm(channels: int, device=None) -> torch.Tensor:
+    if channels % 32:
+        raise RuntimeError(f"shuffle_store_perm: {channels} channels are not whole groups of 32")
+    key = (int(channels), None if device is None else str(device))
+    perm = _STORE_PERM.get(key)
+    if perm is None:
+        p = torch.arange(channels, device=device)
+        perm = _STORE_PERM[key] = 32 * (p // 32) + 4 * (p % 8) + (p // 8) % 4
+    return perm
+
+
+_STORE_PERM = {}
+
+
+_SHUFFLE_OK = {}
+
+
+def conv_shuffle_in_place_supported(*args, **kw) -> bool:
+    return conv_shuffle_in_place_kernel(*args, **kw) is not None
+
+
+def conv_shuffle_in_place_kernel(n: int, h: int, w: int, c_stored: int, c_skip: int, cout: int, ksize: int, dil: int, pad: int,
+                                 scaled: bool, skip_scaled: bool = False, skip_nbatch: int = 0) -> Optional[str]:
+    key = (n, h, w, c_stored, c_skip, cout, ksize, dil, pad, bool(scaled), bool(skip_scaled), int(skip_nbatch))
+    ok = _SHUFFLE_OK.get(key, 0)
+    if ok == 0:
+        ok = None
+        if c_stored % 64 == 0 and c_skip % 8 == 0 and h % 2 == 0 and w % 2 == 0:
+            d = ConvH8Desc()
+            fake = 1 << 20
+            d.src[0].ptr, d.src[0].scale, d.src[0].G, d.src[0].shuffle = fake, (fake if scaled else None), c_stored // 8, 1
+            d.nsrc = 1
+            if c_skip:
+                d.src[1].ptr, d.src[1].scale, d.src[1].G, d.src[1].nbatch = fake, (fake if skip_scaled else None), c_skip // 8, int(skip_nbatch)
+                d.nsrc = 2
+            d.N, d.H, d.W, d.Cout, d.ksize, d.dil, d.pad = n, h, w, cout, ksize, dil, pad
+            d.wpack, d.out, d.has_act, d.slope = fake, fake, 1, 0.01
+            buf = C.create_string_buffer(96)
+            if _lib.load().slu_conv2d_h8_kernel_name(C.byref(d), buf, 96) == 0:
+                ok = buf.value.decode()
+        _SHUFFLE_OK[key] = ok
+    return ok
 
 
 def _req_h8(t: torch.Tensor, name: str) -> torch.Tensor:
@@ -77,6 +122,11 @@
     for i, s in enumerate(srcs):
         t = _req_h8(s.tensor, f"src[{i}]")
         sn, sg, sh, sw, _ = t.shape
+        gstored = sg
+        if s.shuffle:
+            if i != 0 or sg % 8 or s.nbatch:
+                raise RuntimeError("src[0] only may be read through PixelShuffle in place, with whole groups of 64 stored channels")
+            sg, sh, sw = sg // 4, 2 * sh, 2 * sw
         if s.nbatch:
             if i == 0 or sn != s.nbatch or n % sn:
                 raise RuntimeError(f"src[{i}]: a batch-broadcast source must follow a full-batch source and divide N")
@@ -87,9 +137,10 @@
             raise RuntimeError(f"src[{i}]: spatial/batch size {(sn, sh, sw)} != {(n, h, w)}")
         if s.scale is not None:
             _req(s.scale, f"src[{i}].scale")
-            if tuple(s.scale.shape) != (n, 8 * sg):
-                raise RuntimeError(f"src[{i}].scale: expected {(n, 8 * sg)}, got {tuple(s.scale.shape)}")
-        d.src[i].ptr, d.src[i].scale, d.src[i].G, d.src[i].nbatch = t.data_ptr(), _ptr(s.scale), sg, int(s.nbatch)
+            if tuple(s.scale.shape) != (n, 8 * gstored):
+                raise RuntimeError(f"src[{i}].scale: expected {(n, 8 * gstored)}, got {tuple(s.scale.shape)}")
+        d.src[i].ptr, d.src[i].scale, d.src[i].G, d.src[i].nbatch = t.data_ptr(), _ptr(s.scale), gstored, int(s.nbatch)
+        d.src[i].shuffle = 1 if s.shuffle else 0
         gin += sg
         keep.append(t)
     if not 8 * (gin - 1) < cin <= 8 * gin:
@@ -223,10 +274,13 @@
 
 def ctx_block_h8(x: torch.Tensor, cin: int, w1: torch.Tensor, w2: torch.Tensor, w3: torch.Tensor, bias1: Optional[torch.Tensor],
                  bias2: Optional[torch.Tensor], bn1: Optional[tuple], bias3: Optional[torch.Tensor], bn2: Optional[tuple],
-                 slope: float) -> torch.Tensor:
-    lib = _lib.load()
-    _req_h8(x, "x")
-    n, g, h, w, _ = x.shape
+                 slope: float, n_out: Optional[int] = None) -> torch.Tensor:
+    lib = _lib.load()
+    _req_h8(x, "x")
+    nimg, g, h, w, _ = x.shape
+    n = nimg if n_out is None else int(n_out)
+    if n <= 0 or n % nimg:
+        raise RuntimeError(f"ctx_block_h8: n_out={n} is not a multiple of the {nimg} input images")
     if not 8 * (g - 1) < cin <= 8 * g or not ctx_block_supported(cin, 32, h, w):
         raise RuntimeError(f"ctx_block_h8: cin={cin} with {g} input blocks is not covered by the fused kernel")
     for t, nme, shape in ((w1, "w1", (32, cin, 1)), (w2, "w2", (32, 32, 3)), (w3, "w3", (32, 32, 3))):
@@ -248,6 +302,7 @@
     d.bn1_a, d.bn1_b = _ptr(None if bn1 is None else bn1[0]), _ptr(None if bn1 is None else bn1[1])
     d.bn2_a, d.bn2_b = _ptr(None if bn2 is None else bn2[0]), _ptr(None if bn2 is None else bn2[1])
     d.slope, d.out = float(slope), out.data_ptr()
+    d.nbatch = 0 if n == nimg else nimg
     if ops.TIMING is None:
         check(lib.slu_ctx_block_h8_fwd(C.byref(d), _stream()), "slu_ctx_block_h8_fwd")
         return out
@@ -258,7 +313,7 @@
     px = float(n * h * w)
     flops = 2.0 * (cin * 32 + 2 * 9 * 32 * 32) * px
     nbytes = px * 2.0 * ((8 * g + 32) + (32 + 32) + (32 + 32)) + 2.0 * (32 * cin + 2 * 9 * 32 * 32)
-    min_bytes = px * 2.0 * (8 * g + 32) + 2.0 * (32 * cin + 2 * 9 * 32 * 32)
+    min_bytes = float(h * w) * 2.0 * (nimg * 8 * g + n * 32) + 2.0 * (32 * cin + 2 * 9 * 32 * 32)
     ops.TIMING.append((f"ctx_h8_kernel<{1 if cin <= 16 else 2}>", flops, nbytes, e0, e1, min_bytes))
     ops.TIMING_TAGS.append(f"N{n} {cin}->32 k1 + 32->32 k3d1 + 32->32 k3d2 fused {h}x{w}")
     return out
diff --git a/semanticlidarunc_amd/ops.py b/semanticlidarunc_amd/ops.py
--- a/semanticlidarunc_amd/ops.py
+++ b/semanticlidarunc_amd/ops.py
@@ -1270,7 +1270,7 @@
         e, self.slices = 0, []
         for i, (key, c, refs, shuffled) in enumerate(outs):
             refs = list(refs) + [(-1, 0)] * (3 - len(refs))
-            ot[i] = (e, c, refs[0][0], refs[0][1], refs[1][0], refs[1][1], refs[2][0], refs[2][1], 1 if shuffled else 0)
+            ot[i] = (e, c, refs[0][0], refs[0][1], refs[1][0], refs[1][1], refs[2][0], refs[2][1], int(shuffled))
             self.slices.append((key, e, c))
             e += self.n * c
         self.total = e
diff --git a/semanticlidarunc_amd/salsanext.py b/semanticlidarunc_amd/salsanext.py
--- a/semanticlidarunc_amd/salsanext.py
+++ b/semanticlidarunc_amd/salsanext.py
@@ -22,6 +22,8 @@
 _FUSE_CTX = os.environ.get("SLU_FUSE_CTX", "1") != "0"
 _PACK_MULTI = os.environ.get("SLU_PACK_MULTI", "1") != "0"
 _FUSE_HEAD_MC = os.environ.get("SLU_FUSE_HEAD_MC", "1") != "0"
+_MC_BCAST_INPUT = os.environ.get("SLU_MC_BCAST_INPUT", "1") != "0"
+_SHUFFLE_IN_PLACE = os.environ.get("SLU_SHUFFLE_IN_PLACE", "1") != "0"
 
 
 def set_train_conv_precision(precision: str) -> None:
@@ -45,10 +47,11 @@
 
 class _Prepared:
 
-    __slots__ = ("key", "wpack", "bn_key", "bn_a", "bn_b", "dgrad", "key16", "wpack16", "key8", "wpack8")
+    __slots__ = ("key", "wpack", "bn_key", "bn_a", "bn_b", "dgrad", "key16", "wpack16", "key8", "wpack8", "key8p", "wpack8p", "vecp_key", "vecp")
 
     def __init__(self):
         self.key = self.bn_key = None
+        self.key8p = self.wpack8p = self.vecp_key = self.vecp = None
         self.wpack = self.bn_a = self.bn_b = None
         self.key16 = self.wpack16 = None
         self.key8 = self.wpack8 = None
@@ -77,16 +80,33 @@
             p.bn_key = bkey
         return p.bn_a, p.bn_b
 
-    def _run_h8(self, p: _Prepared, conv: nn.Conv2d, bn, srcs, resid, act, out_f32):
+    def _permuted_h8(self, p: _Prepared, conv: nn.Conv2d, bn):
         wkey = _tkey(conv.weight)
-        if p.key8 != wkey:
-            p.wpack8 = h8.pack_conv_weight_h8(conv.weight.detach().contiguous())
-            p.key8 = wkey
+        if p.key8p != wkey:
+            perm = h8.shuffle_store_perm(conv.out_channels, conv.weight.device)
+            p.wpack8p = h8.pack_conv_weight_h8(conv.weight.detach().index_select(0, perm).contiguous())
+            p.key8p = wkey
         bn_a, bn_b = self._folded_bn(p, bn)
-        return h8.conv2d_h8([h8.H8Source(s.tensor, s.scale, s.nbatch) for s in srcs], p.wpack8, conv.in_channels,
-                            conv.out_channels, conv.kernel_size[0], conv.dilation[0], conv.padding[0],
-                            bias=None if conv.bias is None else conv.bias.detach(), slope=_SLOPE if act else None,
-                            bn_a=bn_a, bn_b=bn_b, resid=resid, out_f32_nchw=out_f32)
+        vkey = (p.bn_key if bn is not None else None, None if conv.bias is None else _tkey(conv.bias))
+        if p.vecp_key != vkey:
+            perm = h8.shuffle_store_perm(conv.out_channels, conv.weight.device)
+            p.vecp = tuple(None if v is None else v.detach().index_select(0, perm).contiguous() for v in (conv.bias, bn_a, bn_b))
+            p.vecp_key = vkey
+        return (p.wpack8p,) + p.vecp
+
+    def _run_h8(self, p: _Prepared, conv: nn.Conv2d, bn, srcs, resid, act, out_f32, out_perm=False):
+        if out_perm:
+            wpack, bias, bn_a, bn_b = self._permuted_h8(p, conv, bn)
+        else:
+            wkey = _tkey(conv.weight)
+            if p.key8 != wkey:
+                p.wpack8 = h8.pack_conv_weight_h8(conv.weight.detach().contiguous())
+                p.key8 = wkey
+            wpack, bias = p.wpack8, None if conv.bias is None else conv.bias.detach()
+            bn_a, bn_b = self._folded_bn(p, bn)
+        return h8.conv2d_h8([h8.H8Source(s.tensor, s.scale, s.nbatch, bool(s.pixel_shuffle)) for s in srcs], wpack,
+                            conv.in_channels, conv.out_channels, conv.kernel_size[0], conv.dilation[0], conv.padding[0],
+                            bias=bias, slope=_SLOPE if act else None, bn_a=bn_a, bn_b=bn_b, resid=resid, out_f32_nchw=out_f32)
 
     def _prepared(self, conv: nn.Conv2d) -> _Prepared:
         cache: Dict[str, _Prepared] = self.__dict__.setdefault("_prep", {})
@@ -101,16 +121,27 @@
                     and conv_b.kernel_size == (1, 1) and conv_b.in_channels == 3 * c and conv_b.out_channels == c
                     and c <= _FUSE_TAIL_MAX_C and h8.conv_tail_supported(c, a1.shape[2], a1.shape[3]))
 
-    def _run_tail(self, conv_a: nn.Conv2d, bn_a, conv_b: nn.Conv2d, bn_b, a1, a2, resid=None, shortcut=None):
+    def _run_tail(self, conv_a: nn.Conv2d, bn_a, conv_b: nn.Conv2d, bn_b, a1, a2, resid=None, shortcut=None, out_perm=False):
+        if out_perm and a1.dtype != torch.float16:
+            raise RuntimeError("a block output in shuffle order exists on the half-precision inference path only")
+        if out_perm and shortcut is not None and self._tail_is_fused(conv_a, conv_b, a1):
+            raise RuntimeError("a block output in shuffle order: the shortcut computed inside the fused tail is not permuted")
         if self._tail_is_fused(conv_a, conv_b, a1):
-            packs, folded = [], []
-            for conv, bn in ((conv_a, bn_a), (conv_b, bn_b)):
+            packs, folded, biases = [], [], []
+            for conv, bn, perm in ((conv_a, bn_a, False), (conv_b, bn_b, out_perm)):
                 p = self._prepared(conv)
+                if perm:
+                    wp, bias, fa, fb = self._permuted_h8(p, conv, bn)
+                    packs.append(wp)
+                    biases.append(bias)
+                    folded.append(None if fa is None else (fa, fb))
+                    continue
                 wkey = _tkey(conv.weight)
                 if p.key8 != wkey:
                     p.wpack8 = h8.pack_conv_weight_h8(conv.weight.detach().contiguous())
                     p.key8 = wkey
                 packs.append(p.wpack8)
+                biases.append(None if conv.bias is None else conv.bias.detach())
                 fa, fb = self._folded_bn(p, bn)
                 folded.append(None if fa is None else (fa, fb))
             sc = None
@@ -122,21 +153,22 @@
                     p.wpack8 = h8.pack_conv_weight_h8(sconv.weight.detach().contiguous())
                     p.key8 = wkey
                 sc = (sx, p.wpack8, None if sconv.bias is None else sconv.bias.detach(), _SLOPE, sconv.in_channels)
-            return h8.conv_tail_h8(a1, a2, packs[0], packs[1], None if conv_a.bias is None else conv_a.bias.detach(), _SLOPE, folded[0],
-                                   None if conv_b.bias is None else conv_b.bias.detach(), _SLOPE, folded[1], resid=resid, shortcut=sc)
+            return h8.conv_tail_h8(a1, a2, packs[0], packs[1], biases[0], _SLOPE, folded[0], biases[1], _SLOPE, folded[1], resid=resid, shortcut=sc)
         if shortcut is not None:
-            resid = self._run(shortcut[1], None, [ConvSource(shortcut[0])])
+            resid = self._run(shortcut[1], None, [ConvSource(shortcut[0])], out_perm=out_perm)
         a3 = self._run(conv_a, bn_a, [ConvSource(a2)])
-        return self._run(conv_b, bn_b, [ConvSource(a1), ConvSource(a2), ConvSource(a3)], resid=resid)
-
-    def _run(self, conv: nn.Conv2d, bn: Optional[nn.BatchNorm2d], srcs, resid=None, act=True, out_f32=False):
+        return self._run(conv_b, bn_b, [ConvSource(a1), ConvSource(a2), ConvSource(a3)], resid=resid, out_perm=out_perm)
+
+    def _run(self, conv: nn.Conv2d, bn: Optional[nn.BatchNorm2d], srcs, resid=None, act=True, out_f32=False, out_perm=False):
         cache: Dict[str, _Prepared] = self.__dict__.setdefault("_prep", {})
         name = str(id(conv))
         p = cache.get(name)
         if p is None:
             p = cache[name] = _Prepared()
         if srcs[0].tensor.dtype == torch.float16:
-            return self._run_h8(p, conv, bn, srcs, resid, act, out_f32)
+            return self._run_h8(p, conv, bn, srcs, resid, act, out_f32, out_perm)
+        if out_perm:
+            raise RuntimeError("an output in shuffle order exists on the half-precision inference path only")
         wkey = _tkey(conv.weight)
         if p.key != wkey:
             p.wpack = ops.pack_conv_weight(conv.weight.detach().contiguous())
@@ -199,9 +231,11 @@
         self.conv3 = nn.Conv2d(out_filters, out_filters, 3, dilation=2, padding=2)
         self.bn2 = nn.BatchNorm2d(out_filters)
 
-    def forward(self, x):
-        if (_FUSE_CTX and x.dtype == torch.float16 and x.dim() == 5 and self.conv1.out_channels == 32
-                and h8.ctx_block_supported(self.conv1.in_channels, 32, x.shape[2], x.shape[3])):
+    def fused_for(self, h: int, w: int) -> bool:
+        return bool(_FUSE_CTX and self.conv1.out_channels == 32 and h8.ctx_block_supported(self.conv1.in_channels, 32, h, w))
+
+    def forward(self, x, n_out=None):
+        if x.dtype == torch.float16 and x.dim() == 5 and self.fused_for(x.shape[2], x.shape[3]):
             packs, folded = [], []
             for conv, bn in ((self.conv1, None), (self.conv2, self.bn1), (self.conv3, self.bn2)):
                 p = self._prepared(conv)
@@ -213,7 +247,10 @@
                 fa, fb = self._folded_bn(p, bn)
                 folded.append(None if fa is None else (fa, fb))
             b = [None if c.bias is None else c.bias.detach() for c in (self.conv1, self.conv2, self.conv3)]
-            return h8.ctx_block_h8(x, self.conv1.in_channels, packs[0], packs[1], packs[2], b[0], b[1], folded[1], b[2], folded[2], _SLOPE)
+            return h8.ctx_block_h8(x, self.conv1.in_channels, packs[0], packs[1], packs[2], b[0], b[1], folded[1], b[2], folded[2], _SLOPE,
+                                   n_out=n_out)
+        if n_out is not None and n_out != x.shape[0]:
+            raise RuntimeError("ResContextBlock: a broadcast input needs the fused half-precision launch")
         shortcut = self._run(self.conv1, None, [ConvSource(x)])
         a1 = self._run(self.conv2, self.bn1, [ConvSource(shortcut)])
         return self._run(self.conv3, self.bn2, [ConvSource(a1)], resid=shortcut)
@@ -236,21 +273,21 @@
         self.bn4 = nn.BatchNorm2d(out_filters)
         self.dropout = nn.Dropout2d(p=dropout_rate)
 
-    def features(self, x):
+    def features(self, x, out_perm=False):
         src = [ConvSource(x)]
         fuse_sc = (_FUSE_SHORTCUT and x.dtype == torch.float16 and x.dim() == 5 and x.shape[1] * 8 == self.conv1.in_channels
-                   and h8.conv_tail_shortcut_supported(self.conv1.out_channels, self.conv1.in_channels))
-        shortcut = None if fuse_sc else self._run(self.conv1, None, src)
+                   and h8.conv_tail_shortcut_supported(self.conv1.out_channels, self.conv1.in_channels) and not out_perm)
+        shortcut = None if fuse_sc else self._run(self.conv1, None, src, out_perm=out_perm)
         a1 = self._run(self.conv2, self.bn1, src)
         a2 = self._run(self.conv3, self.bn2, [ConvSource(a1)])
         if fuse_sc and self._tail_is_fused(self.conv4, self.conv5, a1):
             return self._run_tail(self.conv4, self.bn3, self.conv5, self.bn4, a1, a2, shortcut=(x, self.conv1))
         if shortcut is None:
-            shortcut = self._run(self.conv1, None, src)
-        return self._run_tail(self.conv4, self.bn3, self.conv5, self.bn4, a1, a2, resid=shortcut)
-
-    def forward(self, x, _scales=None, _name=""):
-        full = self.features(x)
+            shortcut = self._run(self.conv1, None, src, out_perm=out_perm)
+        return self._run_tail(self.conv4, self.bn3, self.conv5, self.bn4, a1, a2, resid=shortcut, out_perm=out_perm)
+
+    def forward(self, x, _scales=None, _name="", out_perm=False):
+        full = self.features(x, out_perm)
         s = None
         if self.drop_out:
             s = _draw(self.dropout, full.shape[0], self.conv5.out_channels, full.device, _scales, _name + ".dropout")
@@ -289,7 +326,22 @@
             sx = _mul(sx, up.repeat_interleave(4, dim=1))
         return sx, ss
 
-    def forward(self, x, skip, x_scale=None, _scales=None, _name="", skip_nbatch=0):
+    def reads_in_place(self, n: int, h: int, w: int, skip_nbatch: int = 0, scaled: bool = True) -> bool:
+        if not _SHUFFLE_IN_PLACE:
+            return False
+        ask = lambda sc, skip_sc: h8.conv_shuffle_in_place_kernel(n, 2 * h, 2 * w, self.in_filters, self.conv1.in_channels - self.in_filters // 4,
+                                                                  self.out_filters, 3, 1, 1, sc, skip_sc, skip_nbatch)
+        if self.drop_out:
+            return bool(scaled and ask(True, False) and ask(True, True))
+        return all((ask(sc, False) or "").startswith("ring3_h8_kernel") for sc in (True, False))
+
+    def _ones(self, n, c, dev):
+        t = self.__dict__.get("_ones_table")
+        if t is None or tuple(t.shape) != (n, c) or t.device != dev:
+            t = self.__dict__["_ones_table"] = torch.ones((n, c), dtype=torch.float32, device=dev)
+        return t
+
+    def forward(self, x, skip, x_scale=None, _scales=None, _name="", skip_nbatch=0, x_perm=False, out_perm=False):
         n, cx, dev = x.shape[0], self.in_filters, x.device
         cu, cs = cx // 4, self.conv1.in_channels - cx // 4
         if _scales is not None and _scales.get(_name + "._composed"):
@@ -299,7 +351,17 @@
                                           _draw(self.dropout2, n, cu + cs, dev, _scales, _name + ".dropout2"))
         else:
             sx, ss = x_scale, None
-        if x.dtype == torch.float16:
+        if x.dtype == torch.float16 and x_perm:
+            if sx is not None and not (_scales is not None and _scales.get(_name + "._sx_stored")):
+                sx = sx.index_select(1, h8.shuffle_store_perm(cx, dev))
+            if sx is None and not h8.conv_shuffle_in_place_supported(n, 2 * x.shape[2], 2 * x.shape[3], cx, cs, self.out_filters, 3, 1, 1, False,
+                                                                     ss is not None, skip_nbatch):
+                sx = self._ones(n, cx, dev)
+            e1 = self._run(self.conv1, self.bn1, [ConvSource(x, None if sx is None else sx.contiguous(), True),
+                                                  ConvSource(skip, ss, False, skip_nbatch)])
+        elif x.dtype == torch.float16:
+            if _scales is not None and _scales.get(_name + "._sx_stored"):
+                raise RuntimeError(f"{_name}: multipliers drawn in stored order for a block that does not read in place")
             xs = h8.pixel_shuffle_h8(x, None if sx is None else sx.contiguous())
             e1 = self._run(self.conv1, self.bn1, [ConvSource(xs), ConvSource(skip, ss, False, skip_nbatch)])
         else:
@@ -307,7 +369,7 @@
                 sx = sx.contiguous()
             e1 = self._run(self.conv1, self.bn1, [ConvSource(x, sx, True), ConvSource(skip, ss, False, skip_nbatch)])
         e2 = self._run(self.conv2, self.bn2, [ConvSource(e1)])
-        out = self._run_tail(self.conv3, self.bn3, self.conv4, self.bn4, e1, e2)
+        out = self._run_tail(self.conv3, self.bn3, self.conv4, self.bn4, e1, e2, out_perm=out_perm)
         s3 = None
         if self.drop_out:
             s3 = _draw(self.dropout3, n, self.out_filters, dev, _scales, _name + ".dropout3")
@@ -353,7 +415,12 @@
         b = x.shape[0]
         self.__dict__["_features_only"] = True
         try:
-            u1 = self.forward_mc(x, T, scales) if share_prefix else self._forward(x.repeat(int(T), 1, 1, 1), scales)
+            if share_prefix:
+                u1 = self.forward_mc(x, T, scales)
+            elif _MC_BCAST_INPUT and int(T) > 1 and x.dim() == 4 and self.downCntx.fused_for(x.shape[2], x.shape[3]):
+                u1 = self._forward(x, scales, passes=int(T))
+            else:
+                u1 = self._forward(x.repeat(int(T), 1, 1, 1), scales)
         finally:
             self.__dict__["_features_only"] = False
         p = self._prepared(self.logits)
@@ -405,12 +472,20 @@
                       ("upBlock2", "dropout1", 32), ("upBlock2", "dropout2", 288), ("upBlock2", "dropout3", 128),
                       ("upBlock3", "dropout1", 32), ("upBlock3", "dropout2", 160), ("upBlock3", "dropout3", 64))
 
-    def _predraw_dropout(self, n: int, device):
+    def _in_place_blocks(self, n: int, h: int, w: int, scaled=None):
+        if not (_CONV_PRECISION == "f16" and self._inference_only()):
+            return ()
+        if scaled is None:
+            scaled = any(m.training and m.p > 0.0 for m in self.modules() if isinstance(m, nn.Dropout2d))
+        return tuple(blk for blk, f in (("upBlock1", 16), ("upBlock2", 8), ("upBlock3", 4), ("upBlock4", 2))
+                     if getattr(self, blk).reads_in_place(n, h // f, w // f, scaled=scaled))
+
+    def _predraw_dropout(self, n: int, device, sx_stored=()):
         sites = [(f"{blk}.{name}", getattr(getattr(self, blk), name), c) for blk, name, c in self._DROPOUT_SITES]
         if not any(d.training and d.p > 0.0 for _, d, _ in sites):
             return None
         if _DROPOUT_KERNEL:
-            return self._predraw_dropout_kernel(n, device, sites)
+            return self._predraw_dropout_kernel(n, device, sites, tuple(sx_stored))
         main = torch.cuda.current_stream(device)
         side = self.__dict__.get("_drop_stream")
         if side is None or side.device != device:
@@ -434,8 +509,8 @@
         self.__dict__["_drop_event"] = side.record_event()
         return out
 
-    def _predraw_dropout_kernel(self, n: int, device, sites):
-        sig = (n, str(device), tuple((bool(d.training), float(d.p)) for _, d, _ in sites))
+    def _predraw_dropout_kernel(self, n: int, device, sites, sx_stored=()):
+        sig = (n, str(device), tuple((bool(d.training), float(d.p)) for _, d, _ in sites), sx_stored)
         plan = self.__dict__.get("_drop_plan")
         if plan is None or plan[0] != sig:
             index = {key: i for i, (key, _, _) in enumerate(sites)}
@@ -455,7 +530,7 @@
                 m = getattr(self, blk)
                 cu, cs = m.in_filters // 4, m.conv1.in_channels - m.in_filters // 4
                 d1, d2, d3 = (f"{blk}.dropout{k}" if f"{blk}.dropout{k}" in index else None for k in (1, 2, 3))
-                add(f"{blk}._sx", m.in_filters, [(prod, 0), (d1, 0), (d2, 0)], shuffled=True)
+                add(f"{blk}._sx", m.in_filters, [(prod, 0), (d1, 0), (d2, 0)], shuffled=2 if blk in sx_stored else 1)
                 add(f"{blk}._ss", cs, [(d2, cu)])
                 if d3 is not None:
                     add(f"{blk}.dropout3", chans[d3], [(d3, 0)])
@@ -466,7 +541,7 @@
                     refs = [(-1, 0)] + refs
                 fixed.append((key, c, refs[:3], shuffled))
             plan = (sig, ops.DropoutPlan(n, [(c, float(d.p), bool(d.training and d.p > 0.0)) for _, d, c in sites], fixed, device),
-                    [f"{blk}._composed" for blk in ("upBlock1", "upBlock2", "upBlock3", "upBlock4")])
+                    [f"{blk}._composed" for blk in ("upBlock1", "upBlock2", "upBlock3", "upBlock4")] + [f"{blk}._sx_stored" for blk in sx_stored])
             self.__dict__["_drop_plan"] = plan
         out = plan[1].run()
         for k in plan[2]:
@@ -503,7 +578,7 @@
         if ev is not None:
             torch.cuda.current_stream().wait_event(ev)
 
-    def _forward(self, x, scales):
+    def _forward(self, x, scales, passes: int = 1):
         if not isinstance(x, torch.Tensor) or x.dim() != 4:
             raise RuntimeError("SalsaNext expects a [B, C, H, W] tensor")
         if not x.is_cuda:
@@ -512,13 +587,19 @@
         if x.shape[2] % 16 or x.shape[3] % 16:
             raise RuntimeError("SalsaNext needs H and W divisible by 16")
         x = x.contiguous().float()
+        n = x.shape[0] * passes
+        if passes != 1 and not (_CONV_PRECISION == "f16" and self._inference_only()):
+            raise RuntimeError("SalsaNext: stacked passes over a shared input are a half-precision inference form")
         if not self._inference_only():
             self._pack_training_weights()
+        half = _CONV_PRECISION == "f16" and self._inference_only()
+        in_place = self._in_place_blocks(n, x.shape[2], x.shape[3], scaled=True if scales else None)
+        perm1, perm2, perm3, perm4 = (f"upBlock{k}" in in_place for k in (1, 2, 3, 4))
         if scales is None and (self._inference_only() or _DROPOUT_KERNEL) and not torch.cuda.is_current_stream_capturing():
-            scales = self._predraw_dropout(x.shape[0], x.device)
-        if _CONV_PRECISION == "f16" and self._inference_only():
+            scales = self._predraw_dropout(n, x.device, sx_stored=in_place)
+        if half:
             x = h8.to_h8(x)
-        d = self.downCntx(x)
+        d = self.downCntx(x) if passes == 1 else self.downCntx(x, n_out=n)
         d = self.downCntx2(d)
         d = self.downCntx3(d)
         d0c, d0b = self.resBlock1(d, scales, "resBlock1")
@@ -526,9 +607,9 @@
         d1c, d1b = self.resBlock2(d0c, scales, "resBlock2")
         d2c, d2b = self.resBlock3(d1c, scales, "resBlock3")
         d3c, d3b = self.resBlock4(d2c, scales, "resBlock4")
-        d5c, s5 = self.resBlock5(d3c, scales, "resBlock5")
-        u4, s = self.upBlock1(d5c, d3b, s5, scales, "upBlock1")
-        u3, s = self.upBlock2(u4, d2b, s, scales, "upBlock2")
-        u2, s = self.upBlock3(u3, d1b, s, scales, "upBlock3")
-        u1, _ = self.upBlock4(u2, d0b, s, scales, "upBlock4")
+        d5c, s5 = self.resBlock5(d3c, scales, "resBlock5", out_perm=perm1)
+        u4, s = self.upBlock1(d5c, d3b, s5, scales, "upBlock1", x_perm=perm1, out_perm=perm2)
+        u3, s = self.upBlock2(u4, d2b, s, scales, "upBlock2", x_perm=perm2, out_perm=perm3)
+        u2, s = self.upBlock3(u3, d1b, s, scales, "upBlock3", x_perm=perm3, out_perm=perm4)
+        u1, _ = self.upBlock4(u2, d0b, s, scales, "upBlock4", x_perm=perm4)
         return self._head(u1)
```

After: 723.0 scans/s, median of 6. 1.02x the previous value.
